# ManuelZ/image-search-engine

Hardware: AMD Instinct MI355X
Metric: queries/sec, exact brute-force L2 kNN (recall@10 vs exact CPU), 1Mx512 fp32 index, k=10 (higher is better)
Workload: dtype f32; 1 GPU; 1000000x512 fp32 uniform[0,1) index (default_rng 1234), L2, k=10, nq=16 queries per step, index resident in HBM, steps issued round-robin on 16 HIP streams; 400 untimed steps ahead of the warm-up bring the GPU out of its idle power state; n=1000000, d=512, k=10, nq=16

## Files before the change

### image-search-engine_amd/csrc/ise_knn.hip

```cpp

#include "ise_common.hpp"
#include "ise_scan_params.hpp"
#include "ise_assign.hpp"
#include "ise_exact.hpp"
#include "ise_merge.hpp"
#include "ise_exact_scan.hpp"
#include "ise_gemm_scan.hpp"
#include "ise_gemm_bf16.hpp"
#include "ise_rows.hpp"
#include "ise_short_scan.hpp"
#include "ise_range.hpp"
#include "ise_sel_scan.hpp"
#include "ise_stage.hpp"
#include "ise_remove.hpp"

static thread_local std::string g_err;
static int fail(int code, const std::string& msg) {
    g_err = msg;
    return code;
}
int ise_fail_(int code, const std::string& msg) { return fail(code, msg); }
#define HIP_TRY(expr)                                                                      \
    do {                                                                                   \
        hipError_t e_ = (expr);                                                            \
        if (e_ != hipSuccess)                                                              \
            return fail(e_ == hipErrorOutOfMemory ? ISE_E_NOMEM : ISE_E_HIP,               \
                        std::string(#expr) + ": " + hipGetErrorString(e_));                \
    } while (0)

struct ise_index {
    int d = 0, dp = 0, metric = ISE_METRIC_L2, device = 0;
    int storage = ISE_STORE_F32;
    long long n = 0, cap = 0;
    void* xb = nullptr;
    float* norms = nullptr;
    float* mu = nullptr;
    bool shift_pinned = false;
    long long mu_rows = 0;
    long long norms_rows = 0;
    void* xh = nullptr;
    float* hmeta = nullptr;
    int dph = 0;
    bool shadow_off = false;
    void* xq8 = nullptr;
    uint32_t* bmeta = nullptr;
    int dpb = 0;
    bool byte_off = false;
    double byte_rel = 0.0;
    double byte_rho = 1.0;
    unsigned long long half_batches = 0;
    unsigned long long byte_batches = 0;
    unsigned long long* stats_dev = nullptr;
    unsigned long long mu_updates = 0;
    unsigned long long gemm_chunks = 0;
    struct WorkSlot {
        u64* part = nullptr;
        size_t part_elems = 0;
        u64* keys_tmp = nullptr;
        size_t keys_tmp_elems = 0;
        u64* xchg = nullptr;
        size_t xchg_elems = 0;
        uint32_t xchg_seq = 0;
        char* gemm = nullptr;
        size_t gemm_bytes = 0;
        u64* fl_state = nullptr;
        int* fl_list = nullptr;
        size_t fl_elems = 0;
        uint32_t fl_seq = 0;
        hipEvent_t done = nullptr;
        bool used = false;
        hipStream_t last_stream = nullptr;
    };
    static constexpr int NWS = 6;
    WorkSlot ws[NWS];
    unsigned ws_next = 0;
    hipStream_t stream = nullptr;
    struct HostCtx {
        hipStream_t stream = nullptr;
        float* q_dev = nullptr;  size_t q_elems = 0;
        float* D_dev = nullptr;  long long* I_dev = nullptr;  size_t out_elems = 0;
        float* q_pin = nullptr;  size_t q_pin_elems = 0;
        float* D_pin = nullptr;  long long* I_pin = nullptr;  size_t out_pin_elems = 0;
        float* D_pin_dev = nullptr;  long long* I_pin_dev = nullptr;
        bool busy = false;
    };
    static constexpr int NHC = 4;
    HostCtx hc[NHC];
    std::mutex hc_mu;
    std::condition_variable hc_cv;
    struct HostReq {
        const float* q; long long nq; int k; float* D; long long* I;
        int rc = 0; std::string err; bool done = false;
        std::condition_variable cv;
    };
    static constexpr int CQ_LEADERS = 2;
    std::mutex cq_mu;
    std::deque<HostReq*> cq;
    int cq_leaders = 0;
    unsigned long long cq_batches = 0, cq_requests = 0;
    unsigned long long direct_queries = 0;
    unsigned long long short_batches = 0;
    int num_cu = 256;
    std::mutex mu_;
    template <class T>
    struct Buf {
        T* p = nullptr;
        size_t n = 0;
    };
    struct RangeWs {
        Buf<float> q;
        Buf<unsigned> cnt;
        Buf<long long> segoff;
        Buf<float> sD;
        Buf<uint32_t> sI;
        Buf<long long> tot, lims;
        Buf<unsigned> flag;
        Buf<float> D;
        Buf<long long> I;
        Buf<float> q_pin;
        Buf<long long> lims_pin;
        Buf<float> D_pin;
        Buf<long long> I_pin;
    };
    RangeWs rg;
    std::mutex rg_mu;
    unsigned long long range_batches = 0, range_overflows = 0;
    unsigned long long remove_calls = 0, remove_rows = 0, remove_moved = 0;
    float remove_last_ms = 0.f;
    unsigned long long remove_last_bytes = 0;
    unsigned long long row_epoch = 0;
    struct SelSlot {
        Buf<float> q;
        Buf<u64> part;
        Buf<u64> keys;
        hipEvent_t done = nullptr;
        bool used = false;
        hipStream_t last_stream = nullptr;
    };
    static constexpr int NSS = 4;
    SelSlot ss[NSS];
    unsigned ss_next = 0;
    unsigned long long sel_batches = 0, sel_passes = 0;
    unsigned long long sel_range_batches = 0;
};

static int elem_size(int storage) { return storage == ISE_STORE_BF16 ? 2 : 4; }
static int pad_dim(int d, int storage) {
    const int per_step = 64 / elem_size(storage);
    const int steps = (d + per_step - 1) / per_step;
    return (steps > 4 ? (steps + 3) / 4 * 4 : steps) * per_step;
}
static int pad_bytes(int d) {
    const int steps = (d + 63) / 64;
    return (steps > 4 ? (steps + 3) / 4 * 4 : steps) * 64;
}
static size_t row_bytes(const ise_index* h) { return (size_t)h->dp * elem_size(h->storage); }
static size_t shadow_row_bytes(const ise_index* h) { return (size_t)h->dph * 2; }
static size_t byte_row_bytes(const ise_index* h) { return (size_t)h->dpb; }
static int chunk_steps_rb(size_t rb) {
    const int steps = (int)(rb / 64);
    for (int ch = 8; ch > 1; ch >>= 1)
        if (steps % ch == 0) return ch;
    return 1;
}
static int chunk_steps(const ise_index* h) { return chunk_steps_rb(row_bytes(h)); }
static int qs_stride_units(int units) {
    const int pad = ((2 - (units / 4)) % 16 + 16) % 16 * 4;
    return units + pad;
}
static int qs_stride_for(const ise_index* h) { return qs_stride_units((int)(row_bytes(h) / 4)); }
static int qs_stride_half(const ise_index* h) { return qs_stride_units(h->dph); }
static int qs_stride_byte(const ise_index* h) { return qs_stride_units(h->dpb / 2); }
#define KPASS_MAX 36
#define XPASS_MAX 32
static size_t scan_lds_bytes(const ise_index* h, int waves, int T, int kb) {
    return scan_lds_layout(qs_stride_for(h), waves, T, kb);
}

extern "C" int ise_version(void) { return 100; }
extern "C" const char* ise_last_error(void) { return g_err.c_str(); }

extern "C" int ise_device_count(int* count) {
    if (!count) return fail(ISE_E_INVALID, "count is NULL");
    int n = 0;
    hipError_t e = hipGetDeviceCount(&n);
    if (e != hipSuccess) {
        *count = 0;
        return fail(ISE_E_NODEVICE, std::string("hipGetDeviceCount: ") + hipGetErrorString(e));
    }
    *count = n;
    return ISE_OK;
}

extern "C" int ise_device_arch(int device, char* buf, int buflen) {
    if (!buf || buflen <= 0) return fail(ISE_E_INVALID, "buf is NULL");
    hipDeviceProp_t prop;
    HIP_TRY(hipGetDeviceProperties(&prop, device));
    snprintf(buf, (size_t)buflen, "%s", prop.gcnArchName);
    return ISE_OK;
}

extern "C" int ise_index_create(ise_index_t** out, int d, int metric, int device) {
    return ise_index_create_ex(out, d, metric, device, ISE_STORE_F32);
}

extern "C" int ise_index_create_ex(ise_index_t** out, int d, int metric, int device, int storage) {
    if (!out) return fail(ISE_E_INVALID, "out is NULL");
    *out = nullptr;
    if (d <= 0) return fail(ISE_E_INVALID, "d must be positive");
    if (storage != ISE_STORE_F32 && storage != ISE_STORE_BF16)
        return fail(ISE_E_INVALID, "storage must be ISE_STORE_F32 or ISE_STORE_BF16");
    if (metric != ISE_METRIC_L2 && metric != ISE_METRIC_INNER_PRODUCT)
        return fail(ISE_E_INVALID, "metric must be ISE_METRIC_L2 or ISE_METRIC_INNER_PRODUCT");
    int ndev = 0;
    if (hipGetDeviceCount(&ndev) != hipSuccess || ndev <= 0)
        return fail(ISE_E_NODEVICE, "no HIP device visible: the kNN path needs an MI355X (gfx950) GPU");
    if (device < 0 || device >= ndev) return fail(ISE_E_INVALID, "device out of range");
    hipDeviceProp_t prop;
    HIP_TRY(hipGetDeviceProperties(&prop, device));
    if (strncmp(prop.gcnArchName, "gfx950", 6) != 0)
        return fail(ISE_E_NODEVICE, std::string("device is ") + prop.gcnArchName +
                                        ", this library is built for gfx950 only");
    ise_index* h = new (std::nothrow) ise_index();
    if (!h) return fail(ISE_E_NOMEM, "host allocation failed");
    h->d = d;
    h->storage = storage;
    h->dp = pad_dim(d, storage);
    h->dph = pad_dim(d, ISE_STORE_BF16);
    h->dpb = pad_bytes(d);
    h->metric = metric;
    h->device = device;
    h->num_cu = prop.multiProcessorCount > 0 ? prop.multiProcessorCount : 256;
    DeviceGuard gd(device);
    hipError_t e = hipStreamCreateWithFlags(&h->stream, hipStreamNonBlocking);
    if (e == hipSuccess) e = hipMalloc(&h->mu, (size_t)h->dp * sizeof(float));
    if (e == hipSuccess) e = hipMemset(h->mu, 0, (size_t)h->dp * sizeof(float));
    if (e == hipSuccess) e = hipMalloc(&h->stats_dev, 32 * sizeof(unsigned long long));
    if (e == hipSuccess) e = hipMemset(h->stats_dev, 0, 32 * sizeof(unsigned long long));
    if (e != hipSuccess) {
        if (h->stream) (void)hipStreamDestroy(h->stream);
        if (h->mu) (void)hipFree(h->mu);
        if (h->stats_dev) (void)hipFree(h->stats_dev);
        delete h;
        return fail(ISE_E_HIP, std::string("index setup: ") + hipGetErrorString(e));
    }
    *out = h;
    return ISE_OK;
}

static void free_byte_shadow(ise_index* h) {
    if (h->xq8) (void)hipFree(h->xq8);
    if (h->bmeta) (void)hipFree(h->bmeta);
    h->xq8 = nullptr;
    h->bmeta = nullptr;
}
static void free_shadow(ise_index* h) {
    if (h->xh) (void)hipFree(h->xh);
    if (h->hmeta) (void)hipFree(h->hmeta);
    h->xh = nullptr;
    h->hmeta = nullptr;
    free_byte_shadow(h);
}

static void free_all(ise_index* h) {
    if (h->xb) (void)hipFree(h->xb);
    if (h->norms) (void)hipFree(h->norms);
    free_shadow(h);
    for (auto& w : h->ws) {
        if (w.part) (void)hipFree(w.part);
        if (w.keys_tmp) (void)hipFree(w.keys_tmp);
        if (w.xchg) (void)hipFree(w.xchg);
        if (w.gemm) (void)hipFree(w.gemm);
        if (w.fl_state) (void)hipFree(w.fl_state);
        if (w.fl_list) (void)hipFree(w.fl_list);
        if (w.done) (void)hipEventDestroy(w.done);
        w = ise_index::WorkSlot();
    }
    for (auto& c : h->hc) {
        if (c.q_dev) (void)hipFree(c.q_dev);
        if (c.D_dev) (void)hipFree(c.D_dev);
        if (c.I_dev) (void)hipFree(c.I_dev);
        if (c.q_pin) (void)hipHostFree(c.q_pin);
        if (c.D_pin) (void)hipHostFree(c.D_pin);
        if (c.I_pin) (void)hipHostFree(c.I_pin);
        if (c.stream) (void)hipStreamDestroy(c.stream);
        c = ise_index::HostCtx();
    }
    {
        auto& r = h->rg;
        for (void* p : {(void*)r.q.p, (void*)r.cnt.p, (void*)r.segoff.p, (void*)r.sD.p, (void*)r.sI.p, (void*)r.tot.p,
                        (void*)r.lims.p, (void*)r.flag.p, (void*)r.D.p, (void*)r.I.p})
            if (p) (void)hipFree(p);
        for (void* p : {(void*)r.q_pin.p, (void*)r.lims_pin.p, (void*)r.D_pin.p, (void*)r.I_pin.p})
            if (p) (void)hipHostFree(p);
        r = ise_index::RangeWs();
    }
    for (auto& sl : h->ss) {
        for (void* p : {(void*)sl.q.p, (void*)sl.part.p, (void*)sl.keys.p})
            if (p) (void)hipFree(p);
        if (sl.done) (void)hipEventDestroy(sl.done);
        sl = ise_index::SelSlot();
    }
    h->xb = h->norms = nullptr;
    h->n = h->cap = 0;
}

extern "C" int ise_index_destroy(ise_index_t* h) {
    if (!h) return ISE_OK;
    {
        DeviceGuard gd(h->device);
        (void)hipDeviceSynchronize();
        free_all(h);
        if (h->mu) (void)hipFree(h->mu);
        if (h->stats_dev) (void)hipFree(h->stats_dev);
        if (h->stream) (void)hipStreamDestroy(h->stream);
    }
    delete h;
    return ISE_OK;
}

extern "C" int ise_index_reset(ise_index_t* h) {
    if (!h) return fail(ISE_E_INVALID, "handle is NULL");
    std::lock_guard<std::mutex> lk(h->mu_);
    DeviceGuard gd(h->device);
    HIP_TRY(hipDeviceSynchronize());
    if (h->xb) (void)hipFree(h->xb);
    if (h->norms) (void)hipFree(h->norms);
    free_shadow(h);
    h->shadow_off = false;
    h->byte_off = false;
    if (h->n > 0) h->row_epoch++;
    h->xb = h->norms = nullptr;
    h->n = h->cap = 0;
    h->shift_pinned = false;
    h->mu_rows = h->norms_rows = 0;
    HIP_TRY(hipMemset(h->mu, 0, (size_t)h->dp * sizeof(float)));
    return ISE_OK;
}

extern "C" int ise_index_info(const ise_index_t* h, int* d, int* metric, int64_t* ntotal, int* device) {
    if (!h) return fail(ISE_E_INVALID, "handle is NULL");
    if (d) *d = h->d;
    if (metric) *metric = h->metric;
    if (ntotal) *ntotal = h->n;
    if (device) *device = h->device;
    return ISE_OK;
}

static int reserve_rows(ise_index* h, long long need, hipStream_t st) {
    if (need <= h->cap) return ISE_OK;
    long long cap = h->cap ? h->cap : 0;
    long long want = need;
    if (cap > 0 && want < cap + cap / 2) want = cap + cap / 2;
    want = (want + 15) / 16 * 16;
    const size_t rb = row_bytes(h);
    char* nx = nullptr;
    float* nn = nullptr;
    HIP_TRY(hipMalloc(&nx, (size_t)want * rb));
    hipError_t e = hipMalloc(&nn, (size_t)want * sizeof(float));
    if (e != hipSuccess) {
        (void)hipFree(nx);
        return fail(ISE_E_NOMEM, std::string("hipMalloc(norms): ") + hipGetErrorString(e));
    }
    if (h->n > 0) {
        HIP_TRY(hipMemcpyAsync(nx, h->xb, (size_t)h->n * rb, hipMemcpyDeviceToDevice, st));
        HIP_TRY(hipMemcpyAsync(nn, h->norms, (size_t)h->n * sizeof(float), hipMemcpyDeviceToDevice, st));
    }
    HIP_TRY(hipMemsetAsync(nx + (size_t)h->n * rb, 0, (size_t)(want - h->n) * rb, st));
    HIP_TRY(hipMemsetAsync(nn + h->n, 0, (size_t)(want - h->n) * sizeof(float), st));
    char* nxh = nullptr;
    float* nmeta = nullptr;
    if (h->xh) {
        const size_t hb = shadow_row_bytes(h);
        if (hipMalloc(&nxh, (size_t)want * hb) != hipSuccess || hipMalloc(&nmeta, (size_t)want * 3 * sizeof(float)) != hipSuccess) {
            (void)hipGetLastError();
            if (nxh) (void)hipFree(nxh);
            nxh = nullptr;
        } else {
            HIP_TRY(hipMemcpyAsync(nxh, h->xh, (size_t)h->n * hb, hipMemcpyDeviceToDevice, st));
            HIP_TRY(hipMemsetAsync(nxh + (size_t)h->n * hb, 0, (size_t)(want - h->n) * hb, st));
            HIP_TRY(hipMemsetAsync(nmeta, 0, (size_t)want * 3 * sizeof(float), st));
            for (int i = 0; i < 3; i++)
                HIP_TRY(hipMemcpyAsync(nmeta + (size_t)i * want, h->hmeta + (size_t)i * h->cap, (size_t)h->n * sizeof(float),
                                       hipMemcpyDeviceToDevice, st));
        }
    }
    char* nxq = nullptr;
    uint32_t* nbm = nullptr;
    if (h->xq8 && nxh) {
        const size_t qb = byte_row_bytes(h);
        if (hipMalloc(&nxq, (size_t)want * qb) != hipSuccess || hipMalloc(&nbm, (size_t)want * sizeof(uint32_t)) != hipSuccess) {
            (void)hipGetLastError();
            if (nxq) (void)hipFree(nxq);
            nxq = nullptr;
        } else {
            HIP_TRY(hipMemcpyAsync(nxq, h->xq8, (size_t)h->n * qb, hipMemcpyDeviceToDevice, st));
            HIP_TRY(hipMemsetAsync(nxq + (size_t)h->n * qb, 0, (size_t)(want - h->n) * qb, st));
            HIP_TRY(hipMemsetAsync(nbm, 0, (size_t)want * sizeof(uint32_t), st));
            HIP_TRY(hipMemcpyAsync(nbm, h->bmeta, (size_t)h->n * sizeof(uint32_t), hipMemcpyDeviceToDevice, st));
        }
    }
    HIP_TRY(hipStreamSynchronize(st));
    if (h->xb) HIP_TRY(hipDeviceSynchronize());
    if (h->xb) (void)hipFree(h->xb);
    if (h->norms) (void)hipFree(h->norms);
    if (h->xh) {
        const bool had_byte = h->xq8 != nullptr;
        free_shadow(h);
        h->shadow_off = nxh == nullptr;
        h->byte_off = h->byte_off || (had_byte && nxh && !nxq);
        h->xh = nxh;
        h->hmeta = nmeta;
        h->xq8 = nxq;
        h->bmeta = nbm;
    }
    h->xb = nx;
    h->norms = nn;
    h->cap = want;
    return ISE_OK;
}

static bool rows_copy_verbatim(const ise_index* h) { return h->storage == ISE_STORE_F32 && h->dp == h->d; }

static bool uses_shift(const ise_index* h) { return h->storage == ISE_STORE_F32 && h->metric == ISE_METRIC_L2; }

static int prepare_shift_locked(ise_index* h, hipStream_t st);

static void launch_shadow(ise_index* h, long long row0, long long n, hipStream_t st) {
    const long long nblk = (n + 3) / 4;
    if (nblk > 0)
        hipLaunchKernelGGL(shadow_rows_kernel, dim3((unsigned)nblk), dim3(256), 0, st, (const float*)h->xb, row0, n, h->d,
                           h->dp, (const float*)h->mu, (_Float16*)h->xh, h->dph, h->hmeta, h->hmeta + h->cap,
                           h->hmeta + 2 * h->cap);
    if (nblk > 0 && h->xq8)
        hipLaunchKernelGGL(byte_rows_kernel, dim3((unsigned)nblk), dim3(256), 0, st, (const float*)h->xb, row0, n, h->d,
                           h->dp, (const float*)h->mu, (int8_t*)h->xq8, h->dpb, h->bmeta);
}

static void launch_norms(ise_index* h, long long row0, long long n, hipStream_t st) {
    const long long nblk = (n + 3) / 4;
    if (h->storage == ISE_STORE_BF16)
        hipLaunchKernelGGL(norms_bf16_kernel, dim3((unsigned)nblk), dim3(256), 0, st, (const __bf16*)h->xb, row0, n,
                           h->dp, h->norms);
    else
        hipLaunchKernelGGL(norms_kernel, dim3((unsigned)nblk), dim3(256), 0, st, (const float*)h->xb, row0, n, h->dp,
                           uses_shift(h) ? h->mu : (const float*)nullptr, h->norms);
    if (h->xh) launch_shadow(h, row0, n, st);
}

#define SHADOW_MIN_ROWS 262144
#define SHADOW_MAX_ROW_BYTES 2048
#define SHADOW_MAX_KC 16
#define BYTE_MAX_K 10
#define BYTE_MAX_NQ 16
#define BYTE_KC 32
#define BYTE_MAX_REL_ERR 0.005
#define BYTE_MIN_RHO 0.5
#define BYTE_SAMPLE 512
static bool byte_rel_ok(const ise_index* h) { return h->byte_rel <= BYTE_MAX_REL_ERR && h->byte_rho >= BYTE_MIN_RHO; }
static int measure_byte_rel(ise_index* h, hipStream_t st) {
    const int m = (int)std::min<long long>(BYTE_SAMPLE, h->n);
    double* dv = nullptr;
    float* dist = nullptr;
    HIP_TRY(hipMalloc(&dv, 2 * sizeof(double)));
    hipError_t e = hipMalloc(&dist, (size_t)m * m * sizeof(float));
    if (e == hipSuccess) {
        hipLaunchKernelGGL(byte_rel_kernel, dim3(1), dim3(1024), 0, st, (const float*)h->norms, (const uint32_t*)h->bmeta,
                           h->n, dv);
        hipLaunchKernelGGL(sample_dist_kernel, dim3((unsigned)(((long long)m * m + 255) / 256)), dim3(256), 0, st,
                           (const float*)h->xb, h->dp, h->d, h->n / m, m, dist);
        hipLaunchKernelGGL(rho_kernel, dim3(1), dim3(1024), 0, st, (const float*)dist, m, dv + 1);
        e = hipGetLastError();
    }
    double v[2] = {INFINITY, 0.0};
    if (e == hipSuccess) e = hipMemcpyAsync(v, dv, 2 * sizeof(double), hipMemcpyDeviceToHost, st);
    if (e == hipSuccess) e = hipStreamSynchronize(st);
    (void)hipFree(dv);
    if (dist) (void)hipFree(dist);
    if (e != hipSuccess) return fail(ISE_E_HIP, std::string("byte shadow statistics: ") + hipGetErrorString(e));
    h->byte_rel = v[0];
    h->byte_rho = v[1];
    return ISE_OK;
}
static bool shadow_wanted(const ise_index* h) {
    return uses_shift(h) && !h->xh && !h->shadow_off && h->n > SHADOW_MIN_ROWS &&
           shadow_row_bytes(h) <= SHADOW_MAX_ROW_BYTES;
}
static bool byte_alloc_refused();
static int alloc_shadow(ise_index* h) {
    hipError_t e = hipMalloc(&h->xh, (size_t)h->cap * shadow_row_bytes(h));
    if (e == hipSuccess) e = hipMalloc(&h->hmeta, (size_t)h->cap * 3 * sizeof(float));
    if (e == hipSuccess) e = hipMemset(h->xh, 0, (size_t)h->cap * shadow_row_bytes(h));
    if (e == hipSuccess) e = hipMemset(h->hmeta, 0, (size_t)h->cap * 3 * sizeof(float));
    if (e != hipSuccess) {
        (void)hipGetLastError();
        free_shadow(h);
        if (e != hipErrorOutOfMemory) return fail(ISE_E_HIP, std::string("shadow rows: ") + hipGetErrorString(e));
        h->shadow_off = true;
        return ISE_OK;
    }
    if (h->byte_off) return ISE_OK;
    e = byte_alloc_refused() ? hipErrorOutOfMemory : hipMalloc(&h->xq8, (size_t)h->cap * byte_row_bytes(h));
    if (e == hipSuccess) e = hipMalloc(&h->bmeta, (size_t)h->cap * sizeof(uint32_t));
    if (e == hipSuccess) e = hipMemset(h->xq8, 0, (size_t)h->cap * byte_row_bytes(h));
    if (e == hipSuccess) e = hipMemset(h->bmeta, 0, (size_t)h->cap * sizeof(uint32_t));
    if (e == hipSuccess) return ISE_OK;
    (void)hipGetLastError();
    if (e != hipErrorOutOfMemory) {
        free_shadow(h);
        return fail(ISE_E_HIP, std::string("byte shadow rows: ") + hipGetErrorString(e));
    }
    free_byte_shadow(h);
    h->byte_off = true;
    return ISE_OK;
}

static int prepare_shift_locked(ise_index* h, hipStream_t st) {
    if (!uses_shift(h) || h->n == 0) return ISE_OK;
    const bool need_mu = !h->shift_pinned && (h->mu_rows == 0 || h->n >= h->mu_rows + h->mu_rows / 4 + 1);
    const bool need_shadow = shadow_wanted(h);
    if (!need_mu && h->norms_rows == h->n && !need_shadow) return ISE_OK;
    HIP_TRY(hipDeviceSynchronize());
    if (need_mu) {
        const int groups = (int)std::max<long long>(1, std::min<long long>(COLMEAN_GROUPS_MAX, h->n / 64));
        float* partial = nullptr;
        HIP_TRY(hipMalloc(&partial, (size_t)groups * h->dp * sizeof(float)));
        hipLaunchKernelGGL(col_sum_kernel, dim3((h->dp + 255) / 256, groups), dim3(256), 0, st, (const float*)h->xb,
                           h->n, h->d, h->dp, groups, partial);
        hipLaunchKernelGGL(col_mean_kernel, dim3((h->dp + 255) / 256), dim3(256), 0, st, partial, h->n, h->d, h->dp,
                           groups, h->mu);
        hipError_t e = hipGetLastError();
        if (e == hipSuccess) e = hipStreamSynchronize(st);
        (void)hipFree(partial);
        if (e != hipSuccess) return fail(ISE_E_HIP, std::string("shift vector: ") + hipGetErrorString(e));
        h->mu_rows = h->n;
        h->norms_rows = 0;
        h->mu_updates++;
    }
    if (need_shadow) {
        int rc = alloc_shadow(h);
        if (rc) return rc;
        if (h->xh) launch_shadow(h, 0, h->norms_rows, st);
    }
    const bool full = h->norms_rows == 0 || need_shadow;
    if (h->n > h->norms_rows) launch_norms(h, h->norms_rows, h->n - h->norms_rows, st);
    HIP_TRY(hipGetLastError());
    HIP_TRY(hipStreamSynchronize(st));
    h->norms_rows = h->n;
    if (full && h->xq8) return measure_byte_rel(h, st);
    return ISE_OK;
}

static void norms_after_add(ise_index* h, long long n, hipStream_t st) {
    if (uses_shift(h) && !h->shift_pinned && h->mu_rows == 0) return;
    if (h->norms_rows != h->n) return;
    launch_norms(h, h->n, n, st);
    h->norms_rows = h->n + n;
}

static int add_device_locked(ise_index* h, const float* x_dev, long long n, hipStream_t st) {
    if (n == 0) return ISE_OK;
    if (h->n + n >= (1ll << 32)) return fail(ISE_E_INVALID, "index would exceed 2^32 - 1 rows");
    int rc = reserve_rows(h, h->n + n, st);
    if (rc) return rc;
    char* dst = static_cast<char*>(h->xb) + (size_t)h->n * row_bytes(h);
    if (rows_copy_verbatim(h)) {
        HIP_TRY(hipMemcpyAsync(dst, x_dev, (size_t)n * h->d * sizeof(float), hipMemcpyDeviceToDevice, st));
    } else {
        const long long total = n * h->dp;
        const int blocks = (int)std::min<long long>((total + 255) / 256, 8192);
        if (h->storage == ISE_STORE_BF16)
            hipLaunchKernelGGL(pad_rows_bf16_kernel, dim3(blocks), dim3(256), 0, st, x_dev, n, h->d, (__bf16*)dst, h->dp);
        else
            hipLaunchKernelGGL(pad_rows_kernel, dim3(blocks), dim3(256), 0, st, x_dev, n, h->d, (float*)dst, h->dp);
        HIP_TRY(hipGetLastError());
    }
    norms_after_add(h, n, st);
    HIP_TRY(hipGetLastError());
    h->n += n;
    return ISE_OK;
}

extern "C" int ise_index_set_shift(ise_index_t* h, const float* mu_host) {
    if (!h || !mu_host) return fail(ISE_E_INVALID, "NULL argument");
    std::lock_guard<std::mutex> lk(h->mu_);
    if (!uses_shift(h)) return ISE_OK;
    DeviceGuard gd(h->device);
    HIP_TRY(hipDeviceSynchronize());
    HIP_TRY(hipMemset(h->mu, 0, (size_t)h->dp * sizeof(float)));
    HIP_TRY(hipMemcpy(h->mu, mu_host, (size_t)h->d * sizeof(float), hipMemcpyHostToDevice));
    h->shift_pinned = true;
    h->norms_rows = 0;
    return ISE_OK;
}

extern "C" int ise_index_get_shift(ise_index_t* h, float* mu_host) {
    if (!h || !mu_host) return fail(ISE_E_INVALID, "NULL argument");
    std::lock_guard<std::mutex> lk(h->mu_);
    DeviceGuard gd(h->device);
    int rc = prepare_shift_locked(h, h->stream);
    if (rc) return rc;
    HIP_TRY(hipDeviceSynchronize());
    HIP_TRY(hipMemcpy(mu_host, h->mu, (size_t)h->d * sizeof(float), hipMemcpyDeviceToHost));
    return ISE_OK;
}

extern "C" int ise_index_add_device(ise_index_t* h, const float* x_dev, int64_t n, void* stream) {
    if (!h) return fail(ISE_E_INVALID, "handle is NULL");
    if (n < 0 || (n > 0 && !x_dev)) return fail(ISE_E_INVALID, "bad rows argument");
    std::lock_guard<std::mutex> lk(h->mu_);
    DeviceGuard gd(h->device);
    return add_device_locked(h, x_dev, n, (hipStream_t)stream);
}

extern "C" int ise_index_add_host(ise_index_t* h, const float* x, int64_t n) {
    if (!h) return fail(ISE_E_INVALID, "handle is NULL");
    if (n < 0 || (n > 0 && !x)) return fail(ISE_E_INVALID, "bad rows argument");
    if (n == 0) return ISE_OK;
    std::lock_guard<std::mutex> lk(h->mu_);
    DeviceGuard gd(h->device);
    if (h->n + n >= (1ll << 32)) return fail(ISE_E_INVALID, "index would exceed 2^32 - 1 rows");
    int rc = reserve_rows(h, h->n + n, h->stream);
    if (rc) return rc;
    const long long slab = std::max<long long>(1, (256ll << 20) / ((long long)h->d * 4));
    float* tmp = nullptr;
    if (!rows_copy_verbatim(h)) HIP_TRY(hipMalloc(&tmp, (size_t)std::min<long long>(slab, n) * h->d * sizeof(float)));
    for (long long i0 = 0; i0 < n; i0 += slab) {
        const long long m = std::min<long long>(slab, n - i0);
        if (rows_copy_verbatim(h)) {
            char* dst = static_cast<char*>(h->xb) + (size_t)h->n * row_bytes(h);
            hipError_t e = hipMemcpyAsync(dst, x + (size_t)i0 * h->d, (size_t)m * h->d * sizeof(float),
                                          hipMemcpyHostToDevice, h->stream);
            if (e != hipSuccess) return fail(ISE_E_HIP, std::string("H2D: ") + hipGetErrorString(e));
            norms_after_add(h, m, h->stream);
            h->n += m;
        } else {
            hipError_t e = hipMemcpyAsync(tmp, x + (size_t)i0 * h->d, (size_t)m * h->d * sizeof(float),
                                          hipMemcpyHostToDevice, h->stream);
            if (e != hipSuccess) {
                (void)hipFree(tmp);
                return fail(ISE_E_HIP, std::string("H2D: ") + hipGetErrorString(e));
            }
            rc = add_device_locked(h, tmp, m, h->stream);
            if (rc) {
                (void)hipFree(tmp);
                return rc;
            }
        }
        hipError_t e = hipStreamSynchronize(h->stream);
        if (e != hipSuccess) {
            if (tmp) (void)hipFree(tmp);
            return fail(ISE_E_HIP, std::string("add sync: ") + hipGetErrorString(e));
        }
    }
    if (tmp) (void)hipFree(tmp);
    return ISE_OK;
}

extern "C" int ise_index_reconstruct_host(ise_index_t* h, int64_t i0, int64_t n, float* out) {
    if (!h) return fail(ISE_E_INVALID, "handle is NULL");
    std::lock_guard<std::mutex> lk(h->mu_);
    if (i0 < 0 || n < 0 || i0 + n > h->n || (n > 0 && !out)) return fail(ISE_E_INVALID, "row range out of bounds");
    if (n == 0) return ISE_OK;
    DeviceGuard gd(h->device);
    const char* src = static_cast<const char*>(h->xb) + (size_t)i0 * row_bytes(h);
    if (h->storage == ISE_STORE_F32) {
        HIP_TRY(hipMemcpy2DAsync(out, (size_t)h->d * 4, src, row_bytes(h), (size_t)h->d * 4, (size_t)n,
                                 hipMemcpyDeviceToHost, h->stream));
        HIP_TRY(hipStreamSynchronize(h->stream));
        return ISE_OK;
    }
    const long long slab = std::max<long long>(1, (64ll << 20) / ((long long)h->d * 4));
    float* tmp = nullptr;
    HIP_TRY(hipMalloc(&tmp, (size_t)std::min<long long>(slab, n) * h->d * sizeof(float)));
    int rc = ISE_OK;
    for (long long r0 = 0; r0 < n && rc == ISE_OK; r0 += slab) {
        const long long m = std::min<long long>(slab, n - r0);
        const long long total = m * h->d;
        hipLaunchKernelGGL(unpack_rows_bf16_kernel, dim3((unsigned)std::min<long long>((total + 255) / 256, 8192)),
                           dim3(256), 0, h->stream, (const __bf16*)(src + (size_t)r0 * row_bytes(h)), m, h->d, h->dp, tmp);
        hipError_t e = hipMemcpyAsync(out + (size_t)r0 * h->d, tmp, (size_t)total * sizeof(float), hipMemcpyDeviceToHost,
                                      h->stream);
        if (e == hipSuccess) e = hipStreamSynchronize(h->stream);
        if (e != hipSuccess) rc = fail(ISE_E_HIP, std::string("reconstruct: ") + hipGetErrorString(e));
    }
    (void)hipFree(tmp);
    return rc;
}


static void launch_short(const ise_index* h, int ch, int waves, int bpc, int grid, size_t lds, hipStream_t st,
                         const ScanParams& sp, const ShortParams& tp) {
    if (h->storage == ISE_STORE_BF16) ise_launch_short_bf16(ch, waves, bpc, grid, lds, st, sp, tp);
    else if (uses_shift(h)) ise_launch_short_f32_shift(ch, waves, bpc, grid, lds, st, sp, tp);
    else ise_launch_short_f32_plain(ch, waves, bpc, grid, lds, st, sp, tp);
}

struct ScanPlan {
    int nblocks, tiles_total, tiles_per_block, nqt, ch, kpass, kb, waves, T;
    size_t lds;
    bool exact;
    int kc;
    bool gemm;
    size_t gemm_bytes;
    bool half;
    bool byte;
    bool short_;
    int short_bpc;
};

static void launch_scan(const ise_index* h, const ScanPlan& pl, dim3 grid, hipStream_t st, const ScanParams& sp) {
    const int ch = pl.ch, waves = pl.waves, T = pl.T;
    const size_t lds = pl.lds;
    if (pl.byte) ise_launch_scan_i8_shadow(ch, waves, T, grid, lds, st, sp);
    else if (pl.half) ise_launch_scan_f16_shadow(ch, waves, T, grid, lds, st, sp);
    else if (h->storage == ISE_STORE_BF16) ise_launch_scan_bf16(ch, waves, T, grid, lds, st, sp);
    else if (uses_shift(h)) ise_launch_scan_f32_shift(ch, waves, T, grid, lds, st, sp);
    else ise_launch_scan_f32_plain(ch, waves, T, grid, lds, st, sp);
}

static int exact_extra(int k) {
    static const int forced = [] { const char* e = getenv("ISE_EXACT_EXTRA"); return e ? atoi(e) : 0; }();
    (void)k;
    return forced > 0 && forced <= 16 ? forced : 4;
}
static float exact_beta(const ise_index* h) { return (0.5625f * h->dp + 256.f) * 5.9604645e-8f * 1.02f; }
static float half_beta(const ise_index* h) { return (5.f * h->dph + 128.f) * 5.9604645e-8f * 1.02f; }
static float half_lo_shrink(const ise_index* h) { return 1.f - ((float)h->dp / 16.f + 96.f) * 5.9604645e-8f; }
static float byte_beta(const ise_index* h) { return ((float)h->dp / 8.f + 64.f) * 5.9604645e-8f * 1.02f; }
struct EnvKnobs {
    std::atomic<int> force_exact{0};
    std::atomic<int> no_direct{0};
    std::atomic<int> no_short{0};
    std::atomic<int> short_tpb_max{0};
    std::atomic<int> direct_short_max_tiles{0};
    std::atomic<int> range_stage_cap{0};
    std::atomic<int> no_half{0};
    std::atomic<int> no_byte{0};
    std::atomic<int> fail_byte_alloc{0};
    std::atomic<int> remove_slab_rows{0};
    void refresh() {
        auto flag = [](const char* name) { const char* e = getenv(name); return (e && e[0] == '1') ? 1 : 0; };
        auto num = [](const char* name) { const char* e = getenv(name); return e ? atoi(e) : 0; };
        force_exact.store(flag("ISE_FORCE_EXACT"));
        no_direct.store(flag("ISE_NO_DIRECT"));
        no_short.store(flag("ISE_NO_SHORT"));
        short_tpb_max.store(num("ISE_SHORT_TPB_MAX"));
        direct_short_max_tiles.store(num("ISE_DIRECT_SHORT_MAX_TILES"));
        range_stage_cap.store(num("ISE_RANGE_STAGE_CAP"));
        no_half.store(flag("ISE_NO_HALF_FILTER"));
        no_byte.store(flag("ISE_NO_BYTE_FILTER"));
        fail_byte_alloc.store(flag("ISE_FAIL_BYTE_ALLOC"));
        remove_slab_rows.store(num("ISE_REMOVE_SLAB_ROWS"));
    }
};
static EnvKnobs& knobs() {
    static EnvKnobs k;
    static std::once_flag once;
    std::call_once(once, [] { k.refresh(); });
    return k;
}
extern "C" int ise_refresh_env_knobs(void) {
    knobs().refresh();
    return ISE_OK;
}
static bool force_exact() { return knobs().force_exact.load(std::memory_order_relaxed) != 0; }
static bool byte_alloc_refused() { return knobs().fail_byte_alloc.load(std::memory_order_relaxed) != 0; }

static bool xchg_enabled() {
    static const bool on = [] { const char* e = getenv("ISE_NO_XCHG"); return !(e && e[0] == '1'); }();
    return on;
}

static int make_plan(const ise_index* h, long long nq, int k, ScanPlan* pl, bool allow_short = true,
                     bool allow_half = true) {
    pl->exact = uses_shift(h);
    const bool shadow_ok = allow_half && pl->exact && h->xh != nullptr && !knobs().no_half.load(std::memory_order_relaxed);
    pl->byte = shadow_ok && h->xq8 != nullptr && byte_rel_ok(h) && !knobs().no_byte.load(std::memory_order_relaxed) &&
               k <= BYTE_MAX_K && nq <= BYTE_MAX_NQ;
    pl->kc = pl->exact ? (pl->byte ? BYTE_KC : k + exact_extra(k)) : k;
    pl->kpass = pl->kc < KPASS_MAX ? pl->kc : KPASS_MAX;
    pl->kb = pl->kpass <= 16 ? 16 : (pl->kpass <= 32 ? 32 : KB_MAX);
    pl->half = shadow_ok && (pl->byte || pl->kc <= SHADOW_MAX_KC);
    const size_t rb = pl->byte ? byte_row_bytes(h) : (pl->half ? shadow_row_bytes(h) : row_bytes(h));
    auto lds_bytes = [&](int waves, int T) {
        if (pl->byte) return scan_lds_layout(qs_stride_byte(h), waves, T, pl->kb, true);
        return pl->half ? scan_lds_layout(qs_stride_half(h), waves, T, pl->kb, true) : scan_lds_bytes(h, waves, T, pl->kb);
    };
    pl->ch = chunk_steps_rb(rb);
#ifdef ISE_ABLATE
    if (const char* e = getenv("ISE_CH")) {
        const int ch = atoi(e);
        if ((ch == 1 || ch == 2 || ch == 4 || ch == 8) && (int)(rb / 64) % ch == 0) pl->ch = ch;
    }
#endif
    static const double pass_cost_f32[5] = {0.0, 1.0, 1.11, 1.45, 0.0};
    static const double pass_cost_bf16[5] = {0.0, 1.0, 1.07, 1.16, 1.25};
    const bool bf16 = h->storage == ISE_STORE_BF16;
    const double* pass_cost = (bf16 || pl->half) ? pass_cost_bf16 : pass_cost_f32;
    int tmax = bf16 ? 4 : 3;
#ifdef ISE_ABLATE
    if (const char* e = getenv("ISE_TMAX")) tmax = std::min(tmax, std::max(1, atoi(e)));
#endif
    pl->T = 0;
    double best = 0;
    for (int t = 1; t <= tmax; t++) {
        int wv = 0;
        size_t lds = 0;
        const bool xchg_pays = !bf16 && xchg_enabled() && (h->n + 15) / 16 >= 6ll * 8 * h->num_cu;
        if (t == 2 && !xchg_pays && lds_bytes(16, 2) <= LDS_LIMIT) {
            wv = 16;
            lds = lds_bytes(16, 2);
        }
        for (int cand_w = 8; cand_w >= (t == 1 ? 4 : 8) && !wv; cand_w -= 4) {
            lds = lds_bytes(cand_w, t);
            if (lds <= LDS_LIMIT) wv = cand_w;
        }
        if (!wv) break;
        const double cost = (double)((nq + 16 * t - 1) / (16 * t)) * pass_cost[t];
        if (!pl->T || cost < best - 1e-9) {
            pl->T = t;
            pl->waves = wv;
            pl->lds = lds;
            best = cost;
        }
    }
    if (!pl->T) return fail(ISE_E_INVALID, "d too large: a 16-query tile must fit the 160 KiB LDS "
                                              "(float32 rows: d <= 2240, bf16 rows: d <= 4480)");
    if ((pl->T == 1 || pl->waves == 16) && pl->ch > 4) pl->ch = 4;
    pl->tiles_total = (int)((h->n + 15) / 16);
    int blocks_per_cu = (pl->T == 1 && pl->waves <= 8 && pl->lds <= LDS_LIMIT / 2) ? 2 : 1;
#ifdef ISE_ABLATE
    if (const char* e = getenv("ISE_PLAN")) {
        int wv = 8, bpc = 2;
        if (pl->T == 1 && sscanf(e, "%d,%d", &wv, &bpc) == 2 && (wv == 4 || wv == 8) && bpc >= 1) {
            pl->waves = wv;
            pl->lds = lds_bytes(wv, 1);
            blocks_per_cu = bpc;
        }
    }
#endif
    const bool long_rows = rb > 2048;
    const int nqt_plan = (int)((nq + 16 * pl->T - 1) / (16 * pl->T));
    const int min_tiles = (int)std::max<size_t>(1, 65536 / (16 * rb));
    const int slots = h->num_cu * blocks_per_cu;
    const int nb_packed = std::min(slots, (pl->tiles_total + pl->waves - 1) / pl->waves);
    const int nb_spread = std::min(std::max(1, slots / nqt_plan), (pl->tiles_total + min_tiles - 1) / min_tiles);
    int nb = std::max(nb_packed, nb_spread);
    if (nb < 1) nb = 1;
    if (nb > MERGE_LISTS_MAX) nb = MERGE_LISTS_MAX;
    pl->tiles_per_block = (pl->tiles_total + nb - 1) / nb;
    if (pl->tiles_per_block < 1) pl->tiles_per_block = 1;
    pl->nblocks = (pl->tiles_total + pl->tiles_per_block - 1) / pl->tiles_per_block;
    if (pl->nblocks < 1) pl->nblocks = 1;
    if (long_rows && pl->T == 1 && pl->waves <= 8 && pl->tiles_per_block <= pl->waves && chunk_steps_rb(rb) == 8) pl->ch = 8;
    pl->nqt = (int)((nq + 16 * pl->T - 1) / (16 * pl->T));
    pl->gemm = false;
    pl->gemm_bytes = 0;
    pl->short_ = false;
    pl->short_bpc = 0;
    static const bool short_t2 = [] { const char* e = getenv("ISE_SHORT_T2"); return !(e && e[0] == '0'); }();
    const int short_T = nq <= 16 ? 1 : 2;
    if (allow_short && !pl->byte && (nq <= 16 || (short_t2 && nq <= 64)) && pl->kc <= pl->kpass && h->n > 0 &&
        !knobs().no_short.load(std::memory_order_relaxed)) {
        int tpb_max = knobs().short_tpb_max.load(std::memory_order_relaxed);
        if (tpb_max <= 0 || tpb_max > SHORT_TPB_MAX) tpb_max = SHORT_TPB_MAX;
        const int S = qs_stride_for(h);
        static const int shapes[2][3] = {{16, 1, 1}, {8, 2, 1}};
        int first = row_bytes(h) <= 2048 ? 0 : 2;
#ifdef ISE_ABLATE
        if (const char* e = getenv("ISE_SHORT_SHAPE")) first = std::max(first, std::min(1, atoi(e)));
#endif
        for (int si = first; si < 2 && !pl->short_; si++) {
            const int wv = shapes[si][0], bpc = shapes[si][1];
            const int short_nqt = (int)((nq + 16 * short_T - 1) / (16 * short_T));
            const int packed = (pl->tiles_total + wv - 1) / wv;
            const int spread = std::min(std::max(1, h->num_cu * bpc / short_nqt), (pl->tiles_total + min_tiles - 1) / min_tiles);
            int nbs = std::max(1, std::min(h->num_cu * bpc * shapes[si][2], std::max(packed, spread)));
            nbs = std::min(nbs, MERGE_LISTS_MAX);
            const int tpb = (pl->tiles_total + nbs - 1) / nbs;
            const size_t lds = short_lds_layout(S, tpb, wv, short_T);
            if (tpb <= tpb_max && lds <= (size_t)LDS_LIMIT / bpc) {
                pl->short_ = true;
                pl->nblocks = nbs;
                pl->tiles_per_block = tpb;
                pl->lds = lds;
                pl->waves = wv;
                pl->short_bpc = bpc;
                pl->T = short_T;
                pl->nqt = short_nqt;
                pl->ch = std::min(chunk_steps(h), 4);
                pl->half = false;
                pl->byte = false;
            }
        }
    }
    return ISE_OK;
}

static int ensure_workspace(ise_index::WorkSlot* w, const ScanPlan& pl, long long nq, bool* changed) {
    if (!w->done) HIP_TRY(hipEventCreateWithFlags(&w->done, hipEventDisableTiming));
    const size_t need = std::max<size_t>((size_t)pl.nqt * pl.nblocks * (16 * pl.T) * pl.kpass, (size_t)MERGE_LISTS_MAX * XPASS_MAX);
    if (need > w->part_elems) {
        if (w->part) (void)hipFree(w->part);
        w->part = nullptr;
        w->part_elems = 0;
        HIP_TRY(hipMalloc(&w->part, need * sizeof(u64)));
        w->part_elems = need;
        *changed = true;
    }
    const size_t needx = (size_t)pl.nqt * (16 * pl.T) * pl.nblocks;
    if (needx > w->xchg_elems) {
        if (w->xchg) (void)hipFree(w->xchg);
        w->xchg = nullptr;
        w->xchg_elems = 0;
        HIP_TRY(hipMalloc(&w->xchg, needx * sizeof(u64)));
        HIP_TRY(hipMemset(w->xchg, 0xFF, needx * sizeof(u64)));
        w->xchg_elems = needx;
        w->xchg_seq = 0;
        if (const char* e = getenv("ISE_XCHG_SEQ_START"))
            w->xchg_seq = (uint32_t)strtoul(e, nullptr, 0);
        *changed = true;
    }
    if (pl.kc > pl.kpass) {
        const size_t need2 = (size_t)nq * ((size_t)pl.kc + 2 + pl.kpass + XPASS_MAX);
        if (need2 > w->keys_tmp_elems) {
            if (w->keys_tmp) (void)hipFree(w->keys_tmp);
            w->keys_tmp = nullptr;
            w->keys_tmp_elems = 0;
            HIP_TRY(hipMalloc(&w->keys_tmp, need2 * sizeof(u64)));
            w->keys_tmp_elems = need2;
            *changed = true;
        }
    }
    if (pl.gemm) {
        const size_t needg = pl.gemm_bytes;
        if (needg > w->gemm_bytes) {
            if (w->gemm) (void)hipFree(w->gemm);
            w->gemm = nullptr;
            w->gemm_bytes = 0;
            HIP_TRY(hipMalloc(&w->gemm, needg));
            w->gemm_bytes = needg;
            *changed = true;
        }
    }
    if (pl.exact) {
        if (!w->fl_state) {
            HIP_TRY(hipMalloc(&w->fl_state, 2 * sizeof(u64)));
            HIP_TRY(hipMemset(w->fl_state, 0, 2 * sizeof(u64)));
            w->fl_seq = 0;
            if (const char* e = getenv("ISE_XCHG_SEQ_START")) w->fl_seq = (uint32_t)strtoul(e, nullptr, 0);
            *changed = true;
        }
        if ((size_t)nq > w->fl_elems) {
            if (w->fl_list) (void)hipFree(w->fl_list);
            w->fl_list = nullptr;
            w->fl_elems = 0;
            HIP_TRY(hipMalloc(&w->fl_list, (size_t)nq * sizeof(int)));
            w->fl_elems = (size_t)nq;
            *changed = true;
        }
    }
    return ISE_OK;
}

static int ensure_workspaces(ise_index* h, const ScanPlan& pl, long long nq) {
    bool changed = false;
    for (auto& w : h->ws) {
        int rc = ensure_workspace(&w, pl, nq, &changed);
        if (rc) return rc;
    }
    if (changed) HIP_TRY(hipDeviceSynchronize());
    return ISE_OK;
}

__global__ void floor_from_keys_kernel(const u64* pass_keys, int nq, int kp, u64* floor_out) {
    const int q = blockIdx.x * blockDim.x + threadIdx.x;
    if (q < nq) floor_out[q] = pass_keys[(size_t)q * kp + kp - 1];
}
__global__ void scatter_pass_kernel(const u64* pass_keys, int nq, int kp, u64* keys_all, int k, int off) {
    const int i = blockIdx.x * blockDim.x + threadIdx.x;
    if (i < nq * kp) {
        const int q = i / kp, r = i - q * kp;
        if (off + r < k) keys_all[(size_t)q * k + off + r] = pass_keys[i];
    }
}
__global__ void decode_keys_kernel(const u64* keys, long long total, int metric, float* D, long long* I) {
    const long long i = (long long)blockIdx.x * blockDim.x + threadIdx.x;
    if (i < total) {
        const u64 key = keys[i];
        const bool pad = key == KEY_PAD;
        const float sc = unord_f32((uint32_t)(key >> 32));
        D[i] = pad ? (metric == ISE_METRIC_L2 ? FLT_MAX : -FLT_MAX) : (metric == ISE_METRIC_L2 ? sc : -sc);
        I[i] = pad ? -1ll : (long long)(uint32_t)key;
    }
}

struct TimedOut {
    hipEvent_t e0, e1, e2;
    bool on = false;
};

static int next_xchg_seq(ise_index::WorkSlot* w, hipStream_t st, uint32_t* seq) {
    if (w->xchg_seq >= 0xFFFFFFF0u) {
        HIP_TRY(hipMemsetAsync(w->xchg, 0xFF, w->xchg_elems * sizeof(u64), st));
        w->xchg_seq = 0;
    }
    *seq = ++w->xchg_seq;
    return ISE_OK;
}
static int next_fl_seq(ise_index::WorkSlot* w, hipStream_t st, uint32_t* seq) {
    if (w->fl_seq >= 0xFFFFFFF0u) {
        HIP_TRY(hipMemsetAsync(w->fl_state, 0, sizeof(u64), st));
        w->fl_seq = 0;
    }
    *seq = ++w->fl_seq;
    return ISE_OK;
}

template <bool RERANK>
static void launch_merge(unsigned grid, size_t lds, hipStream_t st, const MergeParams& mp, const ExactParams& xp) {
    hipLaunchKernelGGL((merge_kernel<RERANK>), dim3(grid), dim3(MERGE_THREADS), lds, st, mp, xp);
}

static int enqueue_exact_fallback(ise_index* h, ise_index::WorkSlot* w, const ScanPlan& pl, const ExactParams& xp,
                                  long long nq, hipStream_t st) {
    ExactScanParams xs;
    xs.xb = (const float*)h->xb; xs.q = xp.q; xs.n = h->n; xs.d = h->d; xs.dp = h->dp;
    xs.id_base = xp.id_base; xs.fl_state = w->fl_state; xs.fl_list = w->fl_list; xs.seq = xp.seq;
    xs.part = w->part;
    xs.rows_per_block = (long long)pl.tiles_per_block * 16;
    xs.arrive = reinterpret_cast<unsigned int*>(w->fl_state + 1);
    xs.direct_n = 0;
    const size_t lds = (size_t)XQ * h->dp * 4 + (size_t)XQ * 4 * 32 * 8;
    MergeParams mp;
    mp.lists = w->part; mp.qt = 1; mp.n_lists = pl.nblocks; mp.nq = (int)nq; mp.metric = h->metric;
    mp.fl_state = w->fl_state; mp.fl_list = w->fl_list; mp.seq = xp.seq; mp.dbg = nullptr; mp.gate = nullptr;
    const int k = xp.k;
    if (k <= XPASS_MAX) {
        xs.kpass = k; xs.floor_keys = nullptr;
        mp.k = k; mp.stride_list = k; mp.stride_qtile = (long long)pl.nblocks * k;
        mp.D = xp.D; mp.I = xp.I; mp.keys_out = xp.keys_out; mp.out_by_pos = 0;
        hipLaunchKernelGGL(exact_scan_kernel<XQ>, dim3((unsigned)pl.nblocks), dim3(256), lds, st, xs, mp);
        HIP_TRY(hipGetLastError());
        return ISE_OK;
    }
    u64* fb_floor = w->keys_tmp + (size_t)nq * ((size_t)pl.kc + 1 + pl.kpass);
    u64* fb_pass = fb_floor + nq;
    const int kp = XPASS_MAX;
    for (int off = 0; off < k; off += kp) {
        xs.kpass = kp; xs.floor_keys = off ? fb_floor : nullptr;
        mp.k = kp; mp.stride_list = kp; mp.stride_qtile = (long long)pl.nblocks * kp;
        mp.D = nullptr; mp.I = nullptr; mp.keys_out = fb_pass; mp.out_by_pos = 1;
        hipLaunchKernelGGL(exact_scan_kernel<XQ>, dim3((unsigned)pl.nblocks), dim3(256), lds, st, xs, mp);
        const long long tot = nq * kp;
        hipLaunchKernelGGL(exact_scatter_kernel, dim3((unsigned)((tot + 255) / 256)), dim3(256), 0, st, xp,
                           (const u64*)fb_pass, kp, off, fb_floor);
        HIP_TRY(hipGetLastError());
    }
    return ISE_OK;
}

static bool no_direct() { return knobs().no_direct.load(std::memory_order_relaxed) != 0; }
static bool direct_applies(const ise_index* h, const ise_index::WorkSlot* w, const ScanPlan& pl, long long nq, int k,
                           int* blocks_out) {
    if (!pl.exact || nq != 1 || k > XPASS_MAX || h->n <= 0 || !w->fl_state || no_direct() || force_exact()) return false;
    int max_tiles = knobs().direct_short_max_tiles.load(std::memory_order_relaxed);
    if (max_tiles <= 0) max_tiles = 128;
    if (pl.short_ && pl.tiles_total > max_tiles) return false;
    long long min_rows = std::max<long long>(16, std::min<long long>(64, (32 * 1024) / ((long long)h->dp * 4)));
    if (h->n < min_rows * 64) min_rows = std::max<long long>(16, h->n / 64);
    long long blocks = std::min<long long>(MERGE_LISTS_MAX, (h->n + min_rows - 1) / min_rows);
    static const long long per_cu = [] { const char* e = getenv("ISE_DIRECT_BLOCKS_PER_CU"); const int v = e ? atoi(e) : 0; return (long long)(v > 0 ? v : 2); }();
    blocks = std::min<long long>(blocks, (long long)h->num_cu * per_cu);
    if ((size_t)nq * blocks * k > w->part_elems) return false;
    *blocks_out = (int)blocks;
    return true;
}
static int direct_small_enqueue(ise_index* h, ise_index::WorkSlot* w, int blocks, const float* q_dev, long long nq, int k,
                                uint32_t id_base, float* D_dev, long long* I_dev, u64* keys_out, hipStream_t st,
                                TimedOut* tm) {
    ExactScanParams xs;
    xs.xb = (const float*)h->xb; xs.q = q_dev; xs.n = h->n; xs.d = h->d; xs.dp = h->dp;
    xs.kpass = k; xs.id_base = id_base; xs.fl_state = w->fl_state; xs.fl_list = w->fl_list; xs.seq = 0;
    xs.floor_keys = nullptr; xs.part = w->part;
    xs.rows_per_block = (h->n + blocks - 1) / blocks;
    xs.arrive = reinterpret_cast<unsigned int*>(w->fl_state + 1);
    xs.direct_n = (int)nq;
    MergeParams mp;
    mp.lists = w->part; mp.qt = 1; mp.n_lists = blocks; mp.nq = (int)nq; mp.metric = h->metric;
    mp.fl_state = w->fl_state; mp.fl_list = w->fl_list; mp.seq = 0; mp.dbg = nullptr; mp.gate = nullptr;
    mp.k = k; mp.stride_list = k; mp.stride_qtile = (long long)blocks * k;
    mp.D = D_dev; mp.I = I_dev; mp.keys_out = keys_out; mp.out_by_pos = 0;
    if (tm && tm->on) HIP_TRY(hipEventRecord(tm->e0, st));
    const int qn = 1;
    const size_t lds = (size_t)qn * h->dp * 4 + (size_t)qn * 4 * 32 * 8;
    hipLaunchKernelGGL((exact_scan_kernel<1, true>), dim3((unsigned)blocks), dim3(256), lds, st, xs, mp);
    HIP_TRY(hipGetLastError());
    if (tm && tm->on) {
        HIP_TRY(hipEventRecord(tm->e1, st));
        HIP_TRY(hipEventRecord(tm->e2, st));
    }
    h->direct_queries += (unsigned long long)nq;
    return ISE_OK;
}

#define GEMM_MIN_NQ 256
#define GEMM_CAPQ 4096
#define GEMM_SAMPLE_SLABS 128
static bool gemm_applies(const ise_index* h, long long nq, int k) {
    static const bool off = [] { const char* e = getenv("ISE_NO_GEMM"); return e && e[0] == '1'; }();
    static const long long min_nq = [] { const char* e = getenv("ISE_GEMM_MIN_NQ"); const int v = e ? atoi(e) : 0; return (long long)(v >= 17 ? v : GEMM_MIN_NQ); }();
    const long long need = h->storage == ISE_STORE_BF16 ? std::min<long long>(min_nq, 128) : min_nq;
    if (off || nq < need || h->n < 128ll * 1024) return false;
    if (h->dp > 512 || h->dp % 128 != 0) return false;
    if (h->storage == ISE_STORE_BF16) return k <= XPASS_MAX;
    if (!uses_shift(h)) return k <= XPASS_MAX;
    return k + exact_extra(k) <= XPASS_MAX;
}
#define GEMM_CAPW 2048
struct GemmLayout {
    size_t qprep, xn, tau, ccnt, dump, cand, wbuf, wcnt, total;
};
static GemmLayout gemm_layout(const ise_index* h) {
    GemmLayout g;
    size_t o = 0;
    auto take = [&](size_t bytes) { const size_t at = o; o += (bytes + 255) / 256 * 256; return at; };
    g.qprep = take((size_t)GEMM_NQ_MAX * qs_stride_for(h) * 4);
    g.xn = take((size_t)GEMM_NQ_MAX * 4);
    g.tau = take((size_t)GEMM_NQ_MAX * 4);
    g.ccnt = take((size_t)(GEMM_NQ_MAX * GEMM_SUBS + 64) * 4);
    g.dump = take((size_t)GEMM_NQ_MAX * GEMM_SAMPLE_SLABS * 128 * 4);
    g.cand = take((size_t)GEMM_NQ_MAX * GEMM_CAPQ * 8);
    g.wbuf = take((size_t)h->num_cu * 8 * GEMM_CAPW * 16);
    g.wcnt = take((size_t)h->num_cu * 8 * 4);
    g.total = o;
    return g;
}

static int plan_for_batch(const ise_index* h, long long nq, int k, ScanPlan* pl) {
    const bool big = gemm_applies(h, nq, k);
    int rc = make_plan(h, big ? std::min<long long>(nq, GEMM_NQ_MAX) : nq, k, pl);
    if (rc) return rc;
    pl->gemm = big;
    pl->gemm_bytes = big ? gemm_layout(h).total : 0;
    return ISE_OK;
}

template <int NS, bool DUMP, bool IPM>
static void launch_gemm_metric(int grid, size_t lds, hipStream_t st, const GemmScanParams& gp) {
    static LdsAttrOnce attr;
    attr.ensure(reinterpret_cast<const void*>(&gemm_scan_kernel<NS, DUMP, IPM>), LDS_LIMIT);
    hipLaunchKernelGGL((gemm_scan_kernel<NS, DUMP, IPM>), dim3(grid), dim3(512), lds, st, gp);
}
template <int NS, bool DUMP>
static void launch_gemm_one(int grid, size_t lds, hipStream_t st, const GemmScanParams& gp) {
    if (gp.metric == ISE_METRIC_INNER_PRODUCT) launch_gemm_metric<NS, DUMP, true>(grid, lds, st, gp);
    else launch_gemm_metric<NS, DUMP, false>(grid, lds, st, gp);
}
template <bool DUMP>
static int launch_gemm(int ns, int grid, size_t lds, hipStream_t st, const GemmScanParams& gp) {
    switch (ns) {
        case 8: launch_gemm_one<8, DUMP>(grid, lds, st, gp); break;
        case 16: launch_gemm_one<16, DUMP>(grid, lds, st, gp); break;
        case 24: launch_gemm_one<24, DUMP>(grid, lds, st, gp); break;
        case 32: launch_gemm_one<32, DUMP>(grid, lds, st, gp); break;
        default: return fail(ISE_E_INVALID, "large-batch path: unsupported padded dimension");
    }
    return ISE_OK;
}

static int search_large_chunk(ise_index* h, ise_index::WorkSlot* w, const float* q_dev, long long nq, int k,
                              uint32_t id_base, float* D_dev, long long* I_dev, u64* keys_out, hipStream_t st,
                              TimedOut* tm) {
    const int kc = k + exact_extra(k);
    const int S = qs_stride_for(h);
    const GemmLayout gl = gemm_layout(h);
    h->gemm_chunks++;
    float* qprep = reinterpret_cast<float*>(w->gemm + gl.qprep);
    float* xn = reinterpret_cast<float*>(w->gemm + gl.xn);
    float* tau = reinterpret_cast<float*>(w->gemm + gl.tau);
    unsigned int* ccnt = reinterpret_cast<unsigned int*>(w->gemm + gl.ccnt);
    float* dump = reinterpret_cast<float*>(w->gemm + gl.dump);
    u64* cand = reinterpret_cast<u64*>(w->gemm + gl.cand);
    const int nq_pad = (int)((nq + GQ - 1) / GQ * GQ);
    int rc;

    if (tm && tm->on) HIP_TRY(hipEventRecord(tm->e0, st));
    hipLaunchKernelGGL(qprep_kernel, dim3((unsigned)((nq_pad + 3) / 4)), dim3(256), 0, st, q_dev, (int)nq, nq_pad, h->d, S,
                       (const float*)h->mu, qprep, xn);
    HIP_TRY(hipGetLastError());

    GemmScanParams gp;
    gp.xb = (const float*)h->xb; gp.norms = h->norms; gp.mu = h->mu; gp.n = h->n; gp.rows16 = (h->n + 15) / 16 * 16;
    gp.dp = h->dp; gp.S = S; gp.qprep = qprep; gp.xn = xn; gp.tau = tau; gp.nq = (int)nq; gp.nq_pad = nq_pad;
    gp.beta = exact_beta(h); gp.id_base = id_base; gp.metric = ISE_METRIC_L2;
    gp.wbuf = reinterpret_cast<u32x4*>(w->gemm + gl.wbuf); gp.wcnt = reinterpret_cast<unsigned int*>(w->gemm + gl.wcnt);
    gp.capw = GEMM_CAPW;
    gp.ablate = 0;
    const int slabs_all = (int)((h->n + 127) / 128);
    const size_t lds = gemm_lds_bytes(S);
    const int ns = h->dp / 16;

    gp.slabs = std::min(slabs_all, GEMM_SAMPLE_SLABS);
    gp.slab_stride = slabs_all / gp.slabs;
    const int nstages = nq_pad / GQ;
    gp.qparts = std::max(1, std::min(nstages, (2 * h->num_cu) / gp.slabs));
    gp.dump = dump;
    if ((rc = launch_gemm<true>(ns, gp.slabs * gp.qparts, lds, st, gp))) return rc;
    hipLaunchKernelGGL(kth_select_kernel, dim3((unsigned)nq_pad), dim3(256), 0, st, (const float*)dump, gp.slabs * 128, kc,
                       (int)nq, tau);
    HIP_TRY(hipGetLastError());
    HIP_TRY(hipMemsetAsync(ccnt, 0, (size_t)(GEMM_NQ_MAX * GEMM_SUBS + 64) * 4, st));

    gp.slabs = slabs_all; gp.slab_stride = 1; gp.qparts = 1; gp.dump = nullptr;
    const int grid = std::min(slabs_all, h->num_cu);
    if ((rc = launch_gemm<false>(ns, grid, lds, st, gp))) return rc;
    unsigned int* overflow = ccnt + GEMM_NQ_MAX * GEMM_SUBS;
    hipLaunchKernelGGL(regroup_kernel, dim3((unsigned)grid * 8), dim3(256), 0, st, (const u32x4*)gp.wbuf,
                       (const unsigned int*)gp.wcnt, GEMM_CAPW, cand, ccnt, GEMM_CAPQ, overflow);
    HIP_TRY(hipGetLastError());
    if (tm && tm->on) HIP_TRY(hipEventRecord(tm->e1, st));

    ScanPlan pl;
    rc = make_plan(h, nq, k, &pl);
    if (rc) return rc;
    ExactParams xp;
    xp.xb = (const float*)h->xb; xp.q = q_dev; xp.n = h->n; xp.d = h->d; xp.dp = h->dp; xp.nq = (int)nq;
    xp.k = k; xp.kc = kc; xp.id_base = id_base; xp.D = D_dev; xp.I = I_dev; xp.keys_out = keys_out;
    xp.fl_state = w->fl_state; xp.fl_list = w->fl_list; xp.seq = 0; xp.stats = h->stats_dev;
    xp.force_fail = force_exact() ? 1 : 0;
    xp.tau_bound = tau;
    if ((rc = next_fl_seq(w, st, &xp.seq))) return rc;
    hipLaunchKernelGGL(gemm_select_kernel, dim3((unsigned)nq), dim3(256),
                       rerank_lds_bytes(h->dp, kc) + (size_t)(GEMM_CAPQ + 256) * 8, st, xp, (const u64*)cand,
                       (const unsigned int*)ccnt, GEMM_CAPQ, (const unsigned int*)overflow);
    HIP_TRY(hipGetLastError());
    if ((rc = enqueue_exact_fallback(h, w, pl, xp, nq, st))) return rc;
    if (tm && tm->on) HIP_TRY(hipEventRecord(tm->e2, st));
    return ISE_OK;
}

static int scan_path_enqueue(ise_index* h, ise_index::WorkSlot* w, const ScanPlan& pl, const float* q_dev, long long nq,
                             int k, uint32_t id_base, float* D_dev, long long* I_dev, u64* keys_out, hipStream_t st,
                             TimedOut* tm, const unsigned int* gate) {
    int rc;
    ScanParams sp;
    sp.xb = h->xb; sp.norms = h->norms; sp.q = q_dev; sp.mu = h->mu; sp.floor_keys = nullptr; sp.part = w->part;
    sp.n = h->n; sp.d = h->d; sp.dp = h->dp; sp.qs_stride = qs_stride_for(h);
    sp.row_slots = (int)(row_bytes(h) / 16);
    sp.nq = (int)nq; sp.k = pl.kpass; sp.kb = pl.kb; sp.metric = h->metric; sp.id_base = id_base;
    sp.beta = pl.exact ? exact_beta(h) : 0.f;
    if (pl.byte) {
        sp.xb = h->xq8; sp.bmeta = h->bmeta;
        sp.qs_stride = qs_stride_byte(h); sp.row_slots = (int)(byte_row_bytes(h) / 16);
        sp.beta = byte_beta(h); sp.lo_shrink = half_lo_shrink(h);
        h->half_batches++;
        h->byte_batches++;
    } else if (pl.half) {
        sp.xb = h->xh; sp.norms = h->hmeta; sp.herr = h->hmeta + h->cap; sp.hexp = h->hmeta + 2 * h->cap;
        sp.qs_stride = qs_stride_half(h); sp.row_slots = (int)(shadow_row_bytes(h) / 16);
        sp.beta = half_beta(h); sp.lo_shrink = half_lo_shrink(h);
        h->half_batches++;
    }
    sp.tiles_total = pl.tiles_total; sp.tiles_per_block = pl.tiles_per_block;
    sp.xchg = xchg_enabled() ? w->xchg : nullptr;
    sp.xchg_seq = 0;
    sp.gate = gate;
    sp.ablate = 0;
    sp.stamps = nullptr;
#ifdef ISE_ABLATE
    if (const char* e = getenv("ISE_ABLATE")) sp.ablate = atoi(e);
    if (const char* e = getenv("ISE_STAMPS")) sp.stamps = (unsigned long long*)strtoull(e, nullptr, 0);
#endif

    MergeParams mp;
    const int NQ = 16 * pl.T;
    mp.lists = w->part; mp.stride_list = (long long)NQ * pl.kpass;
    mp.stride_qtile = (long long)pl.nblocks * NQ * pl.kpass; mp.qt = NQ;
    mp.n_lists = pl.nblocks; mp.nq = (int)nq; mp.k = pl.kpass; mp.metric = h->metric;
    mp.fl_state = nullptr; mp.fl_list = nullptr; mp.seq = 0; mp.out_by_pos = 0;
    mp.dbg = h->stats_dev + 8;
    mp.gate = gate;

    ExactParams xp;
    xp.xb = (const float*)h->xb; xp.q = q_dev; xp.n = h->n; xp.d = h->d; xp.dp = h->dp; xp.nq = (int)nq;
    xp.k = k; xp.kc = pl.kc; xp.id_base = id_base; xp.D = D_dev; xp.I = I_dev; xp.keys_out = keys_out;
    xp.fl_state = w->fl_state; xp.fl_list = w->fl_list; xp.seq = 0; xp.stats = h->stats_dev;
    xp.force_fail = force_exact() ? 1 : 0;
    xp.tau_bound = nullptr;

    if (pl.short_) {
        if (gate) return fail(ISE_E_INVALID, "internal: a gated rerun was planned for the short-index kernel");
        ShortParams shp;
        shp.even_split = 1;
        shp.T = pl.T;
        shp.nqt = pl.nqt;
        h->short_batches++;
        if (tm && tm->on) HIP_TRY(hipEventRecord(tm->e0, st));
        launch_short(h, pl.ch, pl.waves, pl.short_bpc, pl.nblocks, pl.lds, st, sp, shp);
        HIP_TRY(hipGetLastError());
        if (tm && tm->on) HIP_TRY(hipEventRecord(tm->e1, st));
        if (pl.exact) {
            if ((rc = next_fl_seq(w, st, &xp.seq))) return rc;
            mp.D = nullptr; mp.I = nullptr; mp.keys_out = nullptr;
            launch_merge<true>((unsigned)nq, rerank_lds_bytes(h->dp, pl.kc), st, mp, xp);
            HIP_TRY(hipGetLastError());
            if ((rc = enqueue_exact_fallback(h, w, pl, xp, nq, st))) return rc;
        } else {
            mp.D = D_dev; mp.I = I_dev; mp.keys_out = keys_out;
            launch_merge<false>((unsigned)nq, 0, st, mp, xp);
            HIP_TRY(hipGetLastError());
        }
        if (tm && tm->on) HIP_TRY(hipEventRecord(tm->e2, st));
        return ISE_OK;
    }
    const dim3 grid((unsigned)pl.nblocks, (unsigned)pl.nqt);
    if (pl.kc <= pl.kpass) {
        if ((rc = next_xchg_seq(w, st, &sp.xchg_seq))) return rc;
        if (tm && tm->on) HIP_TRY(hipEventRecord(tm->e0, st));
        launch_scan(h, pl, grid, st, sp);
        HIP_TRY(hipGetLastError());
        if (tm && tm->on) HIP_TRY(hipEventRecord(tm->e1, st));
        if (pl.exact) {
            if ((rc = next_fl_seq(w, st, &xp.seq))) return rc;
            mp.D = nullptr; mp.I = nullptr; mp.keys_out = nullptr;
            launch_merge<true>((unsigned)nq, rerank_lds_bytes(h->dp, pl.kc), st, mp, xp);
            HIP_TRY(hipGetLastError());
            if ((rc = enqueue_exact_fallback(h, w, pl, xp, nq, st))) return rc;
        } else {
            mp.D = D_dev; mp.I = I_dev; mp.keys_out = keys_out;
            launch_merge<false>((unsigned)nq, 0, st, mp, xp);
            HIP_TRY(hipGetLastError());
        }
        if (tm && tm->on) HIP_TRY(hipEventRecord(tm->e2, st));
        return ISE_OK;
    }
    const int kc = pl.kc;
    u64* keys_all = (!pl.exact && keys_out) ? keys_out : w->keys_tmp;
    u64* floor_dev = w->keys_tmp + (size_t)nq * kc;
    u64* pass_keys = floor_dev + nq;
    if (tm && tm->on) HIP_TRY(hipEventRecord(tm->e0, st));
    for (int off = 0; off < kc; off += pl.kpass) {
        sp.floor_keys = off ? floor_dev : nullptr;
        mp.D = nullptr; mp.I = nullptr; mp.keys_out = pass_keys;
        if ((rc = next_xchg_seq(w, st, &sp.xchg_seq))) return rc;
        launch_scan(h, pl, grid, st, sp);
        HIP_TRY(hipGetLastError());
        launch_merge<false>((unsigned)nq, 0, st, mp, xp);
        HIP_TRY(hipGetLastError());
        const int tot = (int)nq * pl.kpass;
        hipLaunchKernelGGL(scatter_pass_kernel, dim3((tot + 255) / 256), dim3(256), 0, st, pass_keys, (int)nq,
                           pl.kpass, keys_all, kc, off);
        hipLaunchKernelGGL(floor_from_keys_kernel, dim3(((int)nq + 255) / 256), dim3(256), 0, st, pass_keys, (int)nq,
                           pl.kpass, floor_dev);
        HIP_TRY(hipGetLastError());
    }
    if (tm && tm->on) HIP_TRY(hipEventRecord(tm->e1, st));
    if (pl.exact) {
        if ((rc = next_fl_seq(w, st, &xp.seq))) return rc;
        hipLaunchKernelGGL(rerank_kernel, dim3((unsigned)nq), dim3(256), rerank_lds_bytes(h->dp, kc), st, xp,
                           (const u64*)keys_all);
        HIP_TRY(hipGetLastError());
        if ((rc = enqueue_exact_fallback(h, w, pl, xp, nq, st))) return rc;
    } else if (D_dev) {
        const long long total = nq * k;
        hipLaunchKernelGGL(decode_keys_kernel, dim3((unsigned)((total + 255) / 256)), dim3(256), 0, st, keys_all, total,
                           h->metric, D_dev, I_dev);
        HIP_TRY(hipGetLastError());
    }
    if (tm && tm->on) HIP_TRY(hipEventRecord(tm->e2, st));
    return ISE_OK;
}


template <int NS, bool DUMP, bool L2>
static void launch_gemm_bf16_metric(int grid, size_t lds, hipStream_t st, const GemmScanParams& gp) {
    static LdsAttrOnce attr;
    attr.ensure(reinterpret_cast<const void*>(&gemm_scan_bf16_kernel<NS, DUMP, L2>), LDS_LIMIT);
    hipLaunchKernelGGL((gemm_scan_bf16_kernel<NS, DUMP, L2>), dim3(grid), dim3(512), lds, st, gp);
}
template <int NS, bool DUMP>
static void launch_gemm_bf16_one(int grid, size_t lds, hipStream_t st, const GemmScanParams& gp) {
    if (gp.metric == ISE_METRIC_L2) launch_gemm_bf16_metric<NS, DUMP, true>(grid, lds, st, gp);
    else launch_gemm_bf16_metric<NS, DUMP, false>(grid, lds, st, gp);
}
template <bool DUMP>
static int launch_gemm_bf16(int ns, int grid, size_t lds, hipStream_t st, const GemmScanParams& gp) {
    switch (ns) {
        case 4: launch_gemm_bf16_one<4, DUMP>(grid, lds, st, gp); break;
        case 8: launch_gemm_bf16_one<8, DUMP>(grid, lds, st, gp); break;
        case 12: launch_gemm_bf16_one<12, DUMP>(grid, lds, st, gp); break;
        case 16: launch_gemm_bf16_one<16, DUMP>(grid, lds, st, gp); break;
        default: return fail(ISE_E_INVALID, "large-batch path: unsupported padded dimension");
    }
    return ISE_OK;
}

static int search_large_chunk_bf16(ise_index* h, ise_index::WorkSlot* w, const float* q_dev, long long nq, int k,
                                   uint32_t id_base, float* D_dev, long long* I_dev, u64* keys_out, hipStream_t st,
                                   TimedOut* tm) {
    const int S = qs_stride_for(h);
    const GemmLayout gl = gemm_layout(h);
    h->gemm_chunks++;
    uint32_t* qprep = reinterpret_cast<uint32_t*>(w->gemm + gl.qprep);
    float* xn = reinterpret_cast<float*>(w->gemm + gl.xn);
    float* tau = reinterpret_cast<float*>(w->gemm + gl.tau);
    unsigned int* ccnt = reinterpret_cast<unsigned int*>(w->gemm + gl.ccnt);
    float* dump = reinterpret_cast<float*>(w->gemm + gl.dump);
    u64* cand = reinterpret_cast<u64*>(w->gemm + gl.cand);
    const int nq_pad = (int)((nq + GB_GQ - 1) / GB_GQ * GB_GQ);
    int rc;

    if (tm && tm->on) HIP_TRY(hipEventRecord(tm->e0, st));
    hipLaunchKernelGGL(qprep_bf16_kernel, dim3((unsigned)((nq_pad + 3) / 4)), dim3(256), 0, st, q_dev, (int)nq, nq_pad, h->d, S,
                       qprep, xn);
    HIP_TRY(hipGetLastError());

    constexpr int ROWS = 8 * GB_XT * 16;
    GemmScanParams gp;
    gp.xb = (const float*)h->xb; gp.norms = h->norms; gp.mu = nullptr; gp.n = h->n; gp.rows16 = (h->n + 15) / 16 * 16;
    gp.dp = h->dp; gp.S = S; gp.qprep = reinterpret_cast<const float*>(qprep); gp.xn = xn; gp.tau = tau; gp.nq = (int)nq;
    gp.nq_pad = nq_pad; gp.beta = 0.f; gp.metric = h->metric; gp.id_base = id_base;
    gp.wbuf = reinterpret_cast<u32x4*>(w->gemm + gl.wbuf); gp.wcnt = reinterpret_cast<unsigned int*>(w->gemm + gl.wcnt);
    gp.capw = GEMM_CAPW;
    gp.ablate = 0;
#ifdef ISE_ABLATE
    if (const char* e = getenv("ISE_GEMM_ABLATE")) gp.ablate = atoi(e);
#endif
    const int slabs_all = (int)((h->n + ROWS - 1) / ROWS);
    const size_t lds = (size_t)2 * GB_GQ * S * 4 + (size_t)2 * GEMM_NQ_MAX * 4;
    const int ns = h->dp / 32;

    gp.slabs = std::min(slabs_all, GEMM_SAMPLE_SLABS * 128 / ROWS);
    gp.slab_stride = slabs_all / gp.slabs;
    const int nstages = nq_pad / GB_GQ;
    gp.qparts = std::max(1, std::min(nstages, (2 * h->num_cu) / gp.slabs));
    gp.dump = dump;
    if ((rc = launch_gemm_bf16<true>(ns, gp.slabs * gp.qparts, lds, st, gp))) return rc;
    hipLaunchKernelGGL(kth_select_kernel, dim3((unsigned)nq_pad), dim3(256), 0, st, (const float*)dump, gp.slabs * ROWS, k,
                       (int)nq, tau);
    HIP_TRY(hipGetLastError());
    HIP_TRY(hipMemsetAsync(ccnt, 0, (size_t)(GEMM_NQ_MAX * GEMM_SUBS + 64) * 4, st));

    gp.slabs = slabs_all; gp.slab_stride = 1; gp.qparts = 1; gp.dump = nullptr;
    const int grid = std::min(slabs_all, h->num_cu);
    if ((rc = launch_gemm_bf16<false>(ns, grid, lds, st, gp))) return rc;
    unsigned int* overflow = ccnt + GEMM_NQ_MAX * GEMM_SUBS;
    unsigned int* rerun = overflow + 1;
    hipLaunchKernelGGL(regroup_kernel, dim3((unsigned)grid * 8), dim3(256), 0, st, (const u32x4*)gp.wbuf,
                       (const unsigned int*)gp.wcnt, GEMM_CAPW, cand, ccnt, GEMM_CAPQ, overflow);
    HIP_TRY(hipGetLastError());
    if (tm && tm->on) HIP_TRY(hipEventRecord(tm->e1, st));
    hipLaunchKernelGGL(gemm_select_plain_kernel, dim3((unsigned)nq), dim3(256), (size_t)(GEMM_CAPQ + 320) * 8, st, (const u64*)cand,
                       (const unsigned int*)ccnt, GEMM_CAPQ, (const unsigned int*)overflow, rerun, k, h->metric, D_dev, I_dev,
                       keys_out);
    HIP_TRY(hipGetLastError());
    ScanPlan pl;
    rc = make_plan(h, nq, k, &pl, false);
    if (rc) return rc;
    rc = scan_path_enqueue(h, w, pl, q_dev, nq, k, id_base, D_dev, I_dev, keys_out, st, nullptr, rerun);
    if (rc) return rc;
    if (tm && tm->on) HIP_TRY(hipEventRecord(tm->e2, st));
    return ISE_OK;
}

static int search_large_chunk_ip(ise_index* h, ise_index::WorkSlot* w, const float* q_dev, long long nq, int k,
                                 uint32_t id_base, float* D_dev, long long* I_dev, u64* keys_out, hipStream_t st,
                                 TimedOut* tm) {
    const int S = qs_stride_for(h);
    const GemmLayout gl = gemm_layout(h);
    h->gemm_chunks++;
    float* qprep = reinterpret_cast<float*>(w->gemm + gl.qprep);
    float* xn = reinterpret_cast<float*>(w->gemm + gl.xn);
    float* tau = reinterpret_cast<float*>(w->gemm + gl.tau);
    unsigned int* ccnt = reinterpret_cast<unsigned int*>(w->gemm + gl.ccnt);
    float* dump = reinterpret_cast<float*>(w->gemm + gl.dump);
    u64* cand = reinterpret_cast<u64*>(w->gemm + gl.cand);
    const int nq_pad = (int)((nq + GQ - 1) / GQ * GQ);
    int rc;

    if (tm && tm->on) HIP_TRY(hipEventRecord(tm->e0, st));
    hipLaunchKernelGGL(qprep_kernel, dim3((unsigned)((nq_pad + 3) / 4)), dim3(256), 0, st, q_dev, (int)nq, nq_pad, h->d, S,
                       (const float*)nullptr, qprep, xn);
    HIP_TRY(hipGetLastError());

    GemmScanParams gp;
    gp.xb = (const float*)h->xb; gp.norms = h->norms; gp.mu = nullptr; gp.n = h->n; gp.rows16 = (h->n + 15) / 16 * 16;
    gp.dp = h->dp; gp.S = S; gp.qprep = qprep; gp.xn = xn; gp.tau = tau; gp.nq = (int)nq; gp.nq_pad = nq_pad;
    gp.beta = 0.f; gp.id_base = id_base; gp.metric = ISE_METRIC_INNER_PRODUCT;
    gp.wbuf = reinterpret_cast<u32x4*>(w->gemm + gl.wbuf); gp.wcnt = reinterpret_cast<unsigned int*>(w->gemm + gl.wcnt);
    gp.capw = GEMM_CAPW;
    gp.ablate = 0;
    const int slabs_all = (int)((h->n + 127) / 128);
    const size_t lds = gemm_lds_bytes(S);
    const int ns = h->dp / 16;

    gp.slabs = std::min(slabs_all, GEMM_SAMPLE_SLABS);
    gp.slab_stride = slabs_all / gp.slabs;
    const int nstages = nq_pad / GQ;
    gp.qparts = std::max(1, std::min(nstages, (2 * h->num_cu) / gp.slabs));
    gp.dump = dump;
    if ((rc = launch_gemm<true>(ns, gp.slabs * gp.qparts, lds, st, gp))) return rc;
    hipLaunchKernelGGL(kth_select_kernel, dim3((unsigned)nq_pad), dim3(256), 0, st, (const float*)dump, gp.slabs * 128, k,
                       (int)nq, tau);
    HIP_TRY(hipGetLastError());
    HIP_TRY(hipMemsetAsync(ccnt, 0, (size_t)(GEMM_NQ_MAX * GEMM_SUBS + 64) * 4, st));

    gp.slabs = slabs_all; gp.slab_stride = 1; gp.qparts = 1; gp.dump = nullptr;
    const int grid = std::min(slabs_all, h->num_cu);
    if ((rc = launch_gemm<false>(ns, grid, lds, st, gp))) return rc;
    unsigned int* overflow = ccnt + GEMM_NQ_MAX * GEMM_SUBS;
    unsigned int* rerun = overflow + 1;
    hipLaunchKernelGGL(regroup_kernel, dim3((unsigned)grid * 8), dim3(256), 0, st, (const u32x4*)gp.wbuf,
                       (const unsigned int*)gp.wcnt, GEMM_CAPW, cand, ccnt, GEMM_CAPQ, overflow);
    HIP_TRY(hipGetLastError());
    if (tm && tm->on) HIP_TRY(hipEventRecord(tm->e1, st));
    hipLaunchKernelGGL(gemm_select_plain_kernel, dim3((unsigned)nq), dim3(256), (size_t)(GEMM_CAPQ + 320) * 8, st, (const u64*)cand,
                       (const unsigned int*)ccnt, GEMM_CAPQ, (const unsigned int*)overflow, rerun, k, h->metric, D_dev, I_dev,
                       keys_out);
    HIP_TRY(hipGetLastError());
    ScanPlan pl;
    rc = make_plan(h, nq, k, &pl, false);
    if (rc) return rc;
    rc = scan_path_enqueue(h, w, pl, q_dev, nq, k, id_base, D_dev, I_dev, keys_out, st, nullptr, rerun);
    if (rc) return rc;
    if (tm && tm->on) HIP_TRY(hipEventRecord(tm->e2, st));
    return ISE_OK;
}

static int search_enqueue(ise_index* h, const float* q_dev, long long nq, int k, uint32_t id_base, float* D_dev,
                          long long* I_dev, u64* keys_out, hipStream_t st, TimedOut* tm) {
    int rc = prepare_shift_locked(h, st);
    if (rc) return rc;
    ScanPlan pl;
    rc = plan_for_batch(h, nq, k, &pl);
    if (rc) return rc;
    rc = ensure_workspaces(h, pl, pl.gemm ? std::min<long long>(nq, GEMM_NQ_MAX) : nq);
    if (rc) return rc;
    ise_index::WorkSlot* w = nullptr;
    bool same_stream = false;
    for (auto& s : h->ws)
        if (s.used && s.last_stream == st) { w = &s; same_stream = true; break; }
    if (!w)
        for (auto& s : h->ws)
            if (!s.used) { w = &s; break; }
    if (!w) w = &h->ws[h->ws_next++ % ise_index::NWS];
    if (w->used && !same_stream) HIP_TRY(hipStreamWaitEvent(st, w->done, 0));
    struct Release {
        ise_index::WorkSlot* w;
        hipStream_t st;
        ~Release() {
            if (hipEventRecord(w->done, st) == hipSuccess) { w->used = true; w->last_stream = st; }
        }
    } release{w, st};

    if (pl.gemm) {
        for (long long q0 = 0; q0 < nq; q0 += GEMM_NQ_MAX) {
            const long long m = std::min<long long>(GEMM_NQ_MAX, nq - q0);
            rc = (h->storage == ISE_STORE_BF16 ? search_large_chunk_bf16
                  : uses_shift(h)               ? search_large_chunk
                                                : search_large_chunk_ip)(
                h, w, q_dev + (size_t)q0 * h->d, m, k, id_base, D_dev ? D_dev + (size_t)q0 * k : nullptr,
                I_dev ? I_dev + (size_t)q0 * k : nullptr, keys_out ? keys_out + (size_t)q0 * k : nullptr, st, tm);
            if (rc) return rc;
        }
        return ISE_OK;
    }

    int dblocks = 0;
    if (direct_applies(h, w, pl, nq, k, &dblocks))
        return direct_small_enqueue(h, w, dblocks, q_dev, nq, k, id_base, D_dev, I_dev, keys_out, st, tm);
    return scan_path_enqueue(h, w, pl, q_dev, nq, k, id_base, D_dev, I_dev, keys_out, st, tm, nullptr);
}

static int check_search_args(const ise_index* h, const void* q, long long nq, int k) {
    if (!h) return fail(ISE_E_INVALID, "handle is NULL");
    if (nq < 0 || (nq > 0 && !q)) return fail(ISE_E_INVALID, "bad query argument");
    if (k <= 0 || k > ISE_MAX_K) return fail(ISE_E_INVALID, "k must be in [1, 2048]");
    if (nq > (1ll << 20)) return fail(ISE_E_INVALID, "at most 2^20 queries per call");
    return ISE_OK;
}

extern "C" int ise_index_search_device(ise_index_t* h, const float* q_dev, int64_t nq, int k, float* D_dev,
                                       int64_t* I_dev, void* stream) {
    int rc = check_search_args(h, q_dev, nq, k);
    if (rc) return rc;
    if (nq == 0) return ISE_OK;
    if (!D_dev || !I_dev) return fail(ISE_E_INVALID, "output pointer is NULL");
    std::lock_guard<std::mutex> lk(h->mu_);
    DeviceGuard gd(h->device);
    return search_enqueue(h, q_dev, nq, k, 0u, D_dev, (long long*)I_dev, nullptr, (hipStream_t)stream, nullptr);
}

extern "C" int ise_index_search_keys_device(ise_index_t* h, const float* q_dev, int64_t nq, int k, uint32_t id_base,
                                            uint64_t* keys_dev, void* stream) {
    int rc = check_search_args(h, q_dev, nq, k);
    if (rc) return rc;
    if (nq == 0) return ISE_OK;
    if (!keys_dev) return fail(ISE_E_INVALID, "output pointer is NULL");
    if ((long long)id_base + h->n > (1ll << 32)) return fail(ISE_E_INVALID, "id_base + ntotal exceeds 2^32");
    std::lock_guard<std::mutex> lk(h->mu_);
    DeviceGuard gd(h->device);
    return search_enqueue(h, q_dev, nq, k, id_base, nullptr, nullptr, (u64*)keys_dev, (hipStream_t)stream, nullptr);
}

extern "C" int ise_index_search_timed_device(ise_index_t* h, const float* q_dev, int64_t nq, int k, float* D_dev,
                                             int64_t* I_dev, void* stream, int iters, float* scan_ms_avg,
                                             float* merge_ms_avg) {
    int rc = check_search_args(h, q_dev, nq, k);
    if (rc) return rc;
    if (nq == 0 || iters <= 0) return fail(ISE_E_INVALID, "timed search needs nq > 0, iters > 0");
    if (!D_dev || !I_dev) return fail(ISE_E_INVALID, "output pointer is NULL");
    std::lock_guard<std::mutex> lk(h->mu_);
    DeviceGuard gd(h->device);
    hipStream_t st = (hipStream_t)stream;
    TimedOut tm;
    tm.on = true;
    HIP_TRY(hipEventCreate(&tm.e0));
    HIP_TRY(hipEventCreate(&tm.e1));
    HIP_TRY(hipEventCreate(&tm.e2));
    double s_scan = 0, s_merge = 0;
    for (int it = 0; it < iters; it++) {
// ... 694 lines not shown
    struct Release {
        ise_index::SelSlot* sl;
        hipStream_t st;
        ~Release() {
            if (hipEventRecord(sl->done, st) == hipSuccess) { sl->used = true; sl->last_stream = st; }
        }
    } release{sl, st};
    for (long long i0 = 0; i0 < nq; i0 += SEL_NQ_CHUNK) {
        const long long m = std::min<long long>(SEL_NQ_CHUNK, nq - i0);
        rc = sel_chunk_enqueue(h, sl, sel, q_dev + (size_t)i0 * h->d, m, k, D_dev + (size_t)i0 * k, I_dev + (size_t)i0 * k, st);
        if (rc) return rc;
    }
    return ISE_OK;
}

extern "C" int ise_index_search_sel_device(ise_index_t* h, const float* q_dev, int64_t nq, int k, const ise_selector_t* sel,
                                           float* D_dev, int64_t* I_dev, void* stream) {
    int rc = check_search_args(h, q_dev, nq, k);
    if (rc) return rc;
    if (!sel) return fail(ISE_E_INVALID, "selector is NULL");
    if (nq > 0 && (!D_dev || !I_dev)) return fail(ISE_E_INVALID, "output pointer is NULL");
    std::lock_guard<std::mutex> lk(h->mu_);
    if (nq == 0) return selector_check_locked(h, sel);
    DeviceGuard gd(h->device);
    return search_sel_enqueue(h, sel, q_dev, nq, k, D_dev, (long long*)I_dev, (hipStream_t)stream);
}

extern "C" int ise_index_search_sel_host(ise_index_t* h, const float* q, int64_t nq, int k, const ise_selector_t* sel,
                                         float* D, int64_t* I) {
    int rc = check_search_args(h, q, nq, k);
    if (rc) return rc;
    if (!sel) return fail(ISE_E_INVALID, "selector is NULL");
    if (nq > 0 && (!D || !I)) return fail(ISE_E_INVALID, "output pointer is NULL");
    if (nq == 0) {
        std::lock_guard<std::mutex> lk(h->mu_);
        return selector_check_locked(h, sel);
    }
    DeviceGuard gd(h->device);
    ise_index::HostCtx* c = acquire_ctx(h);
    struct Rel { ise_index* h; ise_index::HostCtx* c; ~Rel() { release_ctx(h, c); } } rel{h, c};
    if (!c->stream) HIP_TRY(hipStreamCreateWithFlags(&c->stream, hipStreamNonBlocking));
    const long long batch = 1024;
    const size_t qe = (size_t)std::min<long long>(nq, batch) * h->d;
    const size_t oe = (size_t)std::min<long long>(nq, batch) * k;
    if (qe > c->q_elems) {
        if (c->q_dev) (void)hipFree(c->q_dev);
        c->q_dev = nullptr; c->q_elems = 0;
        HIP_TRY(hipMalloc(&c->q_dev, qe * sizeof(float)));
        c->q_elems = qe;
    }
    if (oe > c->out_elems) {
        if (c->D_dev) (void)hipFree(c->D_dev);
        if (c->I_dev) (void)hipFree(c->I_dev);
        c->D_dev = nullptr; c->I_dev = nullptr; c->out_elems = 0;
        HIP_TRY(hipMalloc(&c->D_dev, oe * sizeof(float)));
        HIP_TRY(hipMalloc(&c->I_dev, oe * sizeof(long long)));
        c->out_elems = oe;
    }
    for (long long i0 = 0; i0 < nq; i0 += batch) {
        const long long m = std::min<long long>(batch, nq - i0);
        HIP_TRY(hipMemcpyAsync(c->q_dev, q + (size_t)i0 * h->d, (size_t)m * h->d * sizeof(float), hipMemcpyHostToDevice,
                               c->stream));
        {
            std::lock_guard<std::mutex> lk(h->mu_);
            rc = search_sel_enqueue(h, sel, c->q_dev, m, k, c->D_dev, c->I_dev, c->stream);
        }
        if (rc) return rc;
        HIP_TRY(hipMemcpyAsync(D + (size_t)i0 * k, c->D_dev, (size_t)m * k * sizeof(float), hipMemcpyDeviceToHost, c->stream));
        HIP_TRY(hipMemcpyAsync(I + (size_t)i0 * k, c->I_dev, (size_t)m * k * sizeof(long long), hipMemcpyDeviceToHost,
                               c->stream));
        HIP_TRY(hipStreamSynchronize(c->stream));
    }
    return ISE_OK;
}

extern "C" int ise_index_sel_stats(ise_index_t* h, uint64_t* out3) {
    if (!h || !out3) return fail(ISE_E_INVALID, "NULL argument");
    {
        std::lock_guard<std::mutex> lk(h->mu_);
        out3[0] = h->sel_batches;
        out3[1] = h->sel_passes;
    }
    std::lock_guard<std::mutex> lk(h->rg_mu);
    out3[2] = h->sel_range_batches;
    return ISE_OK;
}

struct RemoveRun {
    long long start, len;
};

struct RemoveScratch {
    uint32_t* g = nullptr;
    uint32_t* cend = nullptr;
    uint32_t* src_idx = nullptr;
    char* bounce = nullptr;
    hipEvent_t ev0 = nullptr, ev1 = nullptr;
    ~RemoveScratch() {
        for (void* p : {(void*)g, (void*)cend, (void*)src_idx, (void*)bounce})
            if (p) (void)hipFree(p);
        if (ev0) (void)hipEventDestroy(ev0);
        if (ev1) (void)hipEventDestroy(ev1);
    }
};

static void remove_move_rows(const ise_index* h, void* base, size_t stride, long long a, long long m, const RemoveScratch& sc,
                             hipStream_t st) {
    const uint32_t upr = (uint32_t)(stride / 16);
    const uint32_t total = (uint32_t)(m * upr);
    const uint32_t pieces = (total + 64 * REMOVE_UNROLL - 1) / (64 * REMOVE_UNROLL);
    const unsigned grid = std::max(1u, std::min((pieces + 3) / 4, (unsigned)h->num_cu * 4u));
    hipLaunchKernelGGL(remove_rows_kernel<true>, dim3(grid), dim3(256), 0, st, (const u32x4*)base,
                       (const uint32_t*)sc.src_idx, (u32x4*)sc.bounce, total, upr);
    hipLaunchKernelGGL(remove_rows_kernel<false>, dim3(grid), dim3(256), 0, st, (const u32x4*)sc.bounce,
                       (const uint32_t*)nullptr, (u32x4*)(static_cast<char*>(base) + (size_t)a * stride), total, upr);
}

static int remove_runs_locked(ise_index* h, const std::vector<RemoveRun>& runs, long long removed) {
    const long long n_old = h->n, n_new = n_old - removed, first = runs[0].start;
    const long long moved = n_new - first;
    hipStream_t st = h->stream;
    HIP_TRY(hipDeviceSynchronize());
    if (n_new <= SHADOW_MIN_ROWS) free_shadow(h);
    const bool meta = h->norms_rows == n_old;
    const size_t rb = row_bytes(h), hb = shadow_row_bytes(h), qb = byte_row_bytes(h);
    const bool mv_h = meta && h->xh, mv_q = meta && h->xq8;
    RemoveScratch sc;
    if (moved > 0) {
        const long long T = (long long)runs.size();
        std::vector<uint32_t> g((size_t)T), cend((size_t)T);
        long long c = 0;
        for (long long t = 0; t < T; t++) {
            g[(size_t)t] = (uint32_t)(runs[(size_t)t].start - c);
            c += runs[(size_t)t].len;
            cend[(size_t)t] = (uint32_t)c;
        }
        long long slab = knobs().remove_slab_rows.load(std::memory_order_relaxed);
        if (slab <= 0) slab = std::max<long long>(1, (256ll << 20) / (long long)rb);
        slab = std::min(slab, std::max<long long>(1, (1ll << 31) / (long long)(rb / 16)));
        slab = std::min(slab, moved);
        HIP_TRY(hipMalloc(&sc.g, (size_t)T * sizeof(uint32_t)));
        HIP_TRY(hipMalloc(&sc.cend, (size_t)T * sizeof(uint32_t)));
        HIP_TRY(hipMalloc(&sc.src_idx, (size_t)slab * sizeof(uint32_t)));
        HIP_TRY(hipMalloc(&sc.bounce, (size_t)slab * rb));
        HIP_TRY(hipEventCreate(&sc.ev0));
        HIP_TRY(hipEventCreate(&sc.ev1));
        HIP_TRY(hipMemcpyAsync(sc.g, g.data(), (size_t)T * sizeof(uint32_t), hipMemcpyHostToDevice, st));
        HIP_TRY(hipMemcpyAsync(sc.cend, cend.data(), (size_t)T * sizeof(uint32_t), hipMemcpyHostToDevice, st));
        HIP_TRY(hipStreamSynchronize(st));
        HIP_TRY(hipEventRecord(sc.ev0, st));
        for (long long a = first; a < n_new; a += slab) {
            const long long m = std::min(slab, n_new - a);
            const unsigned gw = (unsigned)std::min<long long>((m + 255) / 256, (long long)h->num_cu * 8);
            hipLaunchKernelGGL(remove_src_kernel, dim3(gw), dim3(256), 0, st, (const uint32_t*)sc.g,
                               (const uint32_t*)sc.cend, (int)T, (uint32_t)a, (uint32_t)m, sc.src_idx);
            remove_move_rows(h, h->xb, rb, a, m, sc, st);
            if (mv_h) remove_move_rows(h, h->xh, hb, a, m, sc, st);
            if (mv_q) remove_move_rows(h, h->xq8, qb, a, m, sc, st);
            if (meta) {
                RemovePlanes gp{}, cp{};
                int np = 0;
                auto plane = [&](void* arr) {
                    uint32_t* w = static_cast<uint32_t*>(arr);
                    uint32_t* b = reinterpret_cast<uint32_t*>(sc.bounce) + (size_t)np * m;
                    gp.src[np] = w;
                    gp.dst[np] = b;
                    cp.src[np] = b;
                    cp.dst[np] = w + a;
                    np++;
                };
                plane(h->norms);
                if (mv_h)
                    for (int i = 0; i < 3; i++) plane(h->hmeta + (size_t)i * h->cap);
                if (mv_q) plane(h->bmeta);
                hipLaunchKernelGGL(remove_words_kernel<true>, dim3(gw, np), dim3(256), 0, st, gp,
                                   (const uint32_t*)sc.src_idx, (uint32_t)m);
                hipLaunchKernelGGL(remove_words_kernel<false>, dim3(gw, np), dim3(256), 0, st, cp,
                                   (const uint32_t*)nullptr, (uint32_t)m);
            }
            HIP_TRY(hipGetLastError());
        }
        HIP_TRY(hipEventRecord(sc.ev1, st));
    }
    HIP_TRY(hipMemsetAsync(static_cast<char*>(h->xb) + (size_t)n_new * rb, 0, (size_t)removed * rb, st));
    HIP_TRY(hipMemsetAsync(h->norms + n_new, 0, (size_t)removed * sizeof(float), st));
    if (h->xh) {
        HIP_TRY(hipMemsetAsync(static_cast<char*>(h->xh) + (size_t)n_new * hb, 0, (size_t)removed * hb, st));
        for (int i = 0; i < 3; i++)
            HIP_TRY(hipMemsetAsync(h->hmeta + (size_t)i * h->cap + n_new, 0, (size_t)removed * sizeof(float), st));
    }
    if (h->xq8) {
        HIP_TRY(hipMemsetAsync(static_cast<char*>(h->xq8) + (size_t)n_new * qb, 0, (size_t)removed * qb, st));
        HIP_TRY(hipMemsetAsync(h->bmeta + n_new, 0, (size_t)removed * sizeof(uint32_t), st));
    }
    h->n = n_new;
    h->row_epoch++;
    h->norms_rows = meta ? n_new : 0;
    const long long mu_rows_old = h->mu_rows;
    h->mu_rows = std::min(h->mu_rows, n_new);
    if (uses_shift(h) && !h->shift_pinned && n_new * 4 < mu_rows_old * 3) h->mu_rows = 0;
    HIP_TRY(hipGetLastError());
    HIP_TRY(hipStreamSynchronize(st));
    h->remove_last_ms = 0.f;
    h->remove_last_bytes = 0;
    if (moved > 0) {
        (void)hipEventElapsedTime(&h->remove_last_ms, sc.ev0, sc.ev1);
        const size_t per_row = rb + (mv_h ? hb + 12 : 0) + (mv_q ? qb + 4 : 0) + (meta ? 4 : 0);
        h->remove_last_bytes = (unsigned long long)moved * per_row;
    }
    h->remove_calls++;
    h->remove_rows += (unsigned long long)removed;
    h->remove_moved += (unsigned long long)moved;
    return ISE_OK;
}

extern "C" int ise_index_remove_range(ise_index_t* h, int64_t i0, int64_t i1, int64_t* n_removed) {
    if (!h) return fail(ISE_E_INVALID, "handle is NULL");
    if (n_removed) *n_removed = 0;
    std::lock_guard<std::mutex> lr(h->rg_mu);
    std::lock_guard<std::mutex> lk(h->mu_);
    const long long a = std::max<long long>(i0, 0), b = std::min<long long>(i1, h->n);
    if (a >= b) return ISE_OK;
    DeviceGuard gd(h->device);
    const int rc = remove_runs_locked(h, {RemoveRun{a, b - a}}, b - a);
    if (rc == ISE_OK && n_removed) *n_removed = b - a;
    return rc;
}

extern "C" int ise_index_remove_ids_host(ise_index_t* h, const int64_t* ids, int64_t n_ids, int64_t* n_removed) {
    if (!h) return fail(ISE_E_INVALID, "handle is NULL");
    if (n_removed) *n_removed = 0;
    if (n_ids < 0 || (n_ids > 0 && !ids)) return fail(ISE_E_INVALID, "ids is NULL");
    if (n_ids == 0) return ISE_OK;
    std::vector<long long> v;
    std::vector<RemoveRun> runs;
    try {
        v.reserve((size_t)n_ids);
        for (int64_t i = 0; i < n_ids; i++)
            if (ids[i] >= 0) v.push_back(ids[i]);
        std::sort(v.begin(), v.end());
        v.erase(std::unique(v.begin(), v.end()), v.end());
    } catch (const std::bad_alloc&) {
        return fail(ISE_E_NOMEM, "remove_ids: host allocation failed");
    }
    std::lock_guard<std::mutex> lr(h->rg_mu);
    std::lock_guard<std::mutex> lk(h->mu_);
    long long removed = 0;
    try {
        for (long long id : v) {
            if (id >= h->n) break;
            if (!runs.empty() && runs.back().start + runs.back().len == id) runs.back().len++;
            else runs.push_back(RemoveRun{id, 1});
            removed++;
        }
    } catch (const std::bad_alloc&) {
        return fail(ISE_E_NOMEM, "remove_ids: host allocation failed");
    }
    if (removed == 0) return ISE_OK;
    DeviceGuard gd(h->device);
    const int rc = remove_runs_locked(h, runs, removed);
    if (rc == ISE_OK && n_removed) *n_removed = removed;
    return rc;
}

extern "C" int ise_index_remove_stats(ise_index_t* h, uint64_t* out3) {
    if (!h || !out3) return fail(ISE_E_INVALID, "NULL argument");
    std::lock_guard<std::mutex> lk(h->mu_);
    out3[0] = h->remove_calls;
    out3[1] = h->remove_rows;
    out3[2] = h->remove_moved;
    return ISE_OK;
}

extern "C" int ise_index_remove_last_timing(ise_index_t* h, float* ms, uint64_t* bytes) {
    if (!h || !ms || !bytes) return fail(ISE_E_INVALID, "NULL argument");
    std::lock_guard<std::mutex> lk(h->mu_);
    *ms = h->remove_last_ms;
    *bytes = h->remove_last_bytes;
    return ISE_OK;
}

extern "C" int ise_index_range_stats(ise_index_t* h, uint64_t* out2) {
    if (!h || !out2) return fail(ISE_E_INVALID, "NULL argument");
    std::lock_guard<std::mutex> lk(h->rg_mu);
    out2[0] = h->range_batches;
    out2[1] = h->range_overflows;
    return ISE_OK;
}

extern "C" int ise_index_short_stats(ise_index_t* h, uint64_t* out1) {
    if (!h || !out1) return fail(ISE_E_INVALID, "NULL argument");
    std::lock_guard<std::mutex> lk(h->mu_);
    out1[0] = h->short_batches;
    return ISE_OK;
}

extern "C" int ise_index_half_stats(ise_index_t* h, uint64_t* out1) {
    if (!h || !out1) return fail(ISE_E_INVALID, "NULL argument");
    std::lock_guard<std::mutex> lk(h->mu_);
    out1[0] = h->half_batches;
    return ISE_OK;
}

extern "C" int ise_index_byte_stats(ise_index_t* h, uint64_t* out2) {
    if (!h || !out2) return fail(ISE_E_INVALID, "NULL argument");
    std::lock_guard<std::mutex> lk(h->mu_);
    out2[0] = h->byte_batches;
    out2[1] = (h->xq8 && byte_rel_ok(h)) ? 1 : 0;
    return ISE_OK;
}

extern "C" int ise_index_byte_row(ise_index_t* h, int64_t i, float* out2) {
    if (!h || !out2) return fail(ISE_E_INVALID, "NULL argument");
    std::lock_guard<std::mutex> lk(h->mu_);
    if (i < 0 || i >= h->n) return fail(ISE_E_INVALID, "row out of range");
    DeviceGuard gd(h->device);
    int rc = prepare_shift_locked(h, h->stream);
    if (rc) return rc;
    if (!h->xq8) return fail(ISE_E_INVALID, "this index has no byte shadow rows");
    HIP_TRY(hipDeviceSynchronize());
    uint32_t m = 0;
    HIP_TRY(hipMemcpy(&m, h->bmeta + i, sizeof(uint32_t), hipMemcpyDeviceToHost));
    uint32_t cb = m << 16, eb = m >> 16;
    float cr;
    memcpy(&cr, &cb, sizeof(float));
    const _Float16 eh = __builtin_bit_cast(_Float16, (unsigned short)eb);
    out2[0] = cr;
    out2[1] = cr * (float)eh;
    return ISE_OK;
}

extern "C" int ise_index_shadow_row(ise_index_t* h, int64_t i, float* out3) {
    if (!h || !out3) return fail(ISE_E_INVALID, "NULL argument");
    std::lock_guard<std::mutex> lk(h->mu_);
    if (i < 0 || i >= h->n) return fail(ISE_E_INVALID, "row out of range");
    DeviceGuard gd(h->device);
    int rc = prepare_shift_locked(h, h->stream);
    if (rc) return rc;
    if (!h->xh) return fail(ISE_E_INVALID, "this index has no shadow rows");
    HIP_TRY(hipDeviceSynchronize());
    for (int j = 0; j < 3; j++)
        HIP_TRY(hipMemcpy(out3 + j, h->hmeta + (size_t)j * h->cap + i, sizeof(float), hipMemcpyDeviceToHost));
    return ISE_OK;
}

extern "C" int ise_index_stage_query_debug(ise_index_t* h, const void* q_dev, int route, void* limbs, int64_t limbs_bytes,
                                           float* out2, int32_t* info3) {
    if (!h || !q_dev || !limbs || !out2 || !info3) return fail(ISE_E_INVALID, "NULL argument");
    if (route != 0 && route != 1) return fail(ISE_E_INVALID, "route: 0 = fp16 shadow, 1 = byte shadow");
    std::lock_guard<std::mutex> lk(h->mu_);
    DeviceGuard gd(h->device);
    int rc = prepare_shift_locked(h, h->stream);
    if (rc) return rc;
    if (route == 1 ? !h->xq8 : !h->xh) return fail(ISE_E_INVALID, "this index has no such shadow rows");
    const int P = route == 1 ? h->dpb : h->dph, es = route == 1 ? 1 : 2;
    const size_t need = (size_t)2 * P * es;
    if (P > 1024 || limbs_bytes < (int64_t)need) return fail(ISE_E_INVALID, "limbs: room for hi and lo of the padded row needed");
    unsigned char* dev = nullptr;
    HIP_TRY(hipMalloc(&dev, need + 16));
    float* out_f = reinterpret_cast<float*>(dev + need);
    int* out_i = reinterpret_cast<int*>(dev + need + 8);
    if (route == 1)
        hipLaunchKernelGGL(stage_debug_kernel<true>, dim3(1), dim3(32), 0, h->stream, (const float*)q_dev, h->mu, h->d, P, dev, out_f, out_i);
    else
        hipLaunchKernelGGL(stage_debug_kernel<false>, dim3(1), dim3(32), 0, h->stream, (const float*)q_dev, h->mu, h->d, P, dev, out_f, out_i);
    hipError_t e = hipGetLastError();
    if (e == hipSuccess) e = hipStreamSynchronize(h->stream);
    std::vector<unsigned char> host(need + 16);
    if (e == hipSuccess) e = hipMemcpy(host.data(), dev, need + 16, hipMemcpyDeviceToHost);
    (void)hipFree(dev);
    HIP_TRY(e);
    memcpy(limbs, host.data(), need);
    memcpy(out2, host.data() + need, 8);
    memcpy(info3, host.data() + need + 8, 8);
    info3[2] = P;
    return ISE_OK;
}

extern "C" int ise_index_host_stats(ise_index_t* h, uint64_t* out3) {
    if (!h || !out3) return fail(ISE_E_INVALID, "NULL argument");
    {
        std::lock_guard<std::mutex> lk(h->cq_mu);
        out3[0] = h->cq_batches;
        out3[1] = h->cq_requests;
    }
    std::lock_guard<std::mutex> lk(h->mu_);
    out3[2] = h->direct_queries;
    return ISE_OK;
}

extern "C" int ise_index_reserve_workspaces(ise_index_t* h, int64_t nq, int k) {
    int rc = check_search_args(h, h, nq, k);
    if (rc) return rc;
    if (nq == 0) return ISE_OK;
    std::lock_guard<std::mutex> lk(h->mu_);
    DeviceGuard gd(h->device);
    rc = prepare_shift_locked(h, h->stream);
    if (rc) return rc;
    ScanPlan pl;
    rc = plan_for_batch(h, nq, k, &pl);
    if (rc) return rc;
    return ensure_workspaces(h, pl, pl.gemm ? std::min<long long>(nq, GEMM_NQ_MAX) : nq);
}

extern "C" int ise_index_stats(ise_index_t* h, uint64_t* out4) {
    if (!h || !out4) return fail(ISE_E_INVALID, "NULL argument");
    std::lock_guard<std::mutex> lk(h->mu_);
    DeviceGuard gd(h->device);
    HIP_TRY(hipDeviceSynchronize());
    unsigned long long tmp[4];
    HIP_TRY(hipMemcpy(tmp, h->stats_dev, sizeof(tmp), hipMemcpyDeviceToHost));
#ifdef ISE_ABLATE
    if (getenv("ISE_DEBUG_STAMPS")) {
        unsigned long long st[16];
        if (hipMemcpy(st, h->stats_dev + 8, sizeof(st), hipMemcpyDeviceToHost) == hipSuccess) {
            fprintf(stderr, "merge/rerank stamps (us since kernel entry):");
            for (int i = 1; i < 8; i++) fprintf(stderr, " [%d] %.2f", i, (double)(long long)(st[i] - st[0]) / 100.0);
            fprintf(stderr, "\n");
        }
    }
#endif
    out4[0] = tmp[0];
    out4[1] = tmp[1];
    out4[2] = h->mu_updates;
    out4[3] = h->gemm_chunks;
    return ISE_OK;
}

static int assign_stage_rows(const ise_index* h) {
    const size_t per = (size_t)(qs_stride_for(h) + 1) * 4;
    int cs = (int)std::min<size_t>(ASSIGN_CS_MAX, (150 * 1024) / per) / 16 * 16;
    return cs;
}
static size_t assign_lds_bytes(const ise_index* h) {
    return (size_t)assign_stage_rows(h) * (qs_stride_for(h) + 1) * 4;
}

template <int NS, int XT>
static void launch_assign(int grid, size_t lds, hipStream_t st, const AssignParams& ap) {
    static LdsAttrOnce attr;
    attr.ensure(reinterpret_cast<const void*>(&assign_kernel<NS, XT>), LDS_LIMIT);
    hipLaunchKernelGGL((assign_kernel<NS, XT>), dim3(grid), dim3(512), lds, st, ap);
}

static bool assign_supported(const ise_index* h) {
    return h->storage == ISE_STORE_F32 && h->dp <= 512 && h->n > 0 && assign_stage_rows(h) >= 16;
}

extern "C" int ise_index_assign_device(ise_index_t* h, const float* x_dev, int64_t n, float* D_dev, int64_t* I_dev,
                                       void* stream) {
    if (!h) return fail(ISE_E_INVALID, "handle is NULL");
    if (n < 0 || (n > 0 && (!x_dev || !I_dev))) return fail(ISE_E_INVALID, "bad argument");
    if (n == 0) return ISE_OK;
    std::lock_guard<std::mutex> lk(h->mu_);
    DeviceGuard gd(h->device);
    if (!assign_supported(h))
        return fail(ISE_E_INVALID, "assignment kernel needs a non-empty float32 index with d <= 512");
    {
        int rc = prepare_shift_locked(h, (hipStream_t)stream);
        if (rc) return rc;
    }
    AssignParams ap;
    ap.x = x_dev; ap.cb = (const float*)h->xb; ap.cnorm = h->norms; ap.mu = uses_shift(h) ? h->mu : nullptr; ap.n = n; ap.d = h->d; ap.dp = h->dp;
    ap.cs_stride = qs_stride_for(h); ap.K = (int)h->n; ap.metric = h->metric; ap.cs = assign_stage_rows(h);
    ap.I = (long long*)I_dev; ap.D = D_dev;
    const size_t lds = assign_lds_bytes(h);
    const int ns = h->dp / 16;
    const int xt = ns <= 8 ? 4 : (ns <= 16 ? 2 : 1);
    const long long rows_per_block = 8ll * xt * 16;
    const long long nslabs = (n + rows_per_block - 1) / rows_per_block;
    const int grid = (int)std::min<long long>(nslabs, (long long)h->num_cu);
    hipStream_t st = (hipStream_t)stream;
    switch (ns) {
        case 1: launch_assign<1, 4>(grid, lds, st, ap); break;
        case 2: launch_assign<2, 4>(grid, lds, st, ap); break;
        case 3: launch_assign<3, 4>(grid, lds, st, ap); break;
        case 4: launch_assign<4, 4>(grid, lds, st, ap); break;
        case 8: launch_assign<8, 4>(grid, lds, st, ap); break;
        case 12: launch_assign<12, 2>(grid, lds, st, ap); break;
        case 16: launch_assign<16, 2>(grid, lds, st, ap); break;
        case 20: launch_assign<20, 1>(grid, lds, st, ap); break;
        case 24: launch_assign<24, 1>(grid, lds, st, ap); break;
        case 28: launch_assign<28, 1>(grid, lds, st, ap); break;
        case 32: launch_assign<32, 1>(grid, lds, st, ap); break;
        default: return fail(ISE_E_INVALID, "unsupported padded dimension for the assignment kernel");
    }
    HIP_TRY(hipGetLastError());
    return ISE_OK;
}

extern "C" int ise_merge_keys_device(const uint64_t* keys_dev, int n_lists, int64_t nq, int k, int metric, float* D_dev,
                                     int64_t* I_dev, int device, void* stream) {
    if (!keys_dev || !D_dev || !I_dev) return fail(ISE_E_INVALID, "NULL pointer");
    if (n_lists <= 0 || n_lists > MERGE_LISTS_MAX) return fail(ISE_E_INVALID, "n_lists must be in [1, 1024]");
    if (k <= 0 || k > ISE_MAX_K || nq < 0 || nq > (1ll << 20)) return fail(ISE_E_INVALID, "bad nq / k");
    if (metric != ISE_METRIC_L2 && metric != ISE_METRIC_INNER_PRODUCT) return fail(ISE_E_INVALID, "bad metric");
    if (nq == 0) return ISE_OK;
    DeviceGuard gd(device);
    MergeParams mp;
    mp.lists = (const u64*)keys_dev;
    mp.stride_list = (long long)nq * k;
    mp.stride_qtile = (long long)k; mp.qt = 1;
    mp.n_lists = n_lists; mp.nq = (int)nq; mp.k = k; mp.metric = metric;
    mp.D = D_dev; mp.I = (long long*)I_dev; mp.keys_out = nullptr;
    mp.fl_state = nullptr; mp.fl_list = nullptr; mp.seq = 0; mp.out_by_pos = 0; mp.dbg = nullptr; mp.gate = nullptr;
    if (n_lists <= 64)
        hipLaunchKernelGGL(merge_small_kernel, dim3((unsigned)((nq + 3) / 4)), dim3(256), 0, (hipStream_t)stream, mp);
    else
        launch_merge<false>((unsigned)nq, 0, (hipStream_t)stream, mp, ExactParams());
    HIP_TRY(hipGetLastError());
    return ISE_OK;
}

extern "C" int ise_normalize_rows_device(float* x_dev, int64_t n, int d, int device, void* stream) {
    if (n < 0 || d <= 0 || (n > 0 && !x_dev)) return fail(ISE_E_INVALID, "bad argument");
    if (n == 0) return ISE_OK;
    if (n >= (1ll << 32)) return fail(ISE_E_INVALID, "too many rows");
    DeviceGuard gd(device);
    hipLaunchKernelGGL(normalize_kernel, dim3((unsigned)((n + 3) / 4)), dim3(256), 0, (hipStream_t)stream, x_dev,
                       (long long)n, d);
    HIP_TRY(hipGetLastError());
    return ISE_OK;
}

extern "C" int ise_bovw_histogram_device(const int64_t* labels_dev, const int64_t* offsets_dev, int64_t n_images, int K,
                                         double* out_dev, int device, void* stream) {
    if (n_images < 0 || K <= 0 || (n_images > 0 && (!offsets_dev || !out_dev)))
        return fail(ISE_E_INVALID, "bad argument");
    if (K > HIST_K_MAX) return fail(ISE_E_INVALID, "histogram: at most 16384 bins");
    if (n_images == 0) return ISE_OK;
    if (n_images >= (1ll << 31)) return fail(ISE_E_INVALID, "too many images");
    DeviceGuard gd(device);
    hipLaunchKernelGGL(bovw_histogram_kernel, dim3((unsigned)n_images), dim3(256), (size_t)K * sizeof(unsigned int),
                       (hipStream_t)stream, (const long long*)labels_dev, (const long long*)offsets_dev, K, out_dev);
    HIP_TRY(hipGetLastError());
    return ISE_OK;
}

extern "C" int ise_normalize_rows_host(float* x, int64_t n, int d, int device) {
    if (n < 0 || d <= 0 || (n > 0 && !x)) return fail(ISE_E_INVALID, "bad argument");
    if (n == 0) return ISE_OK;
    int ndev = 0;
    if (hipGetDeviceCount(&ndev) != hipSuccess || ndev <= 0)
        return fail(ISE_E_NODEVICE, "no HIP device visible: normalize_L2 runs on the GPU");
    DeviceGuard gd(device);
    const long long slab = std::max<long long>(1, (256ll << 20) / ((long long)d * 4));
    float* tmp = nullptr;
    HIP_TRY(hipMalloc(&tmp, (size_t)std::min<long long>(slab, n) * d * sizeof(float)));
    int rc = ISE_OK;
    for (long long i0 = 0; i0 < n && rc == ISE_OK; i0 += slab) {
        const long long m = std::min<long long>(slab, n - i0);
        hipError_t e = hipMemcpy(tmp, x + (size_t)i0 * d, (size_t)m * d * sizeof(float), hipMemcpyHostToDevice);
        if (e == hipSuccess) {
            hipLaunchKernelGGL(normalize_kernel, dim3((unsigned)((m + 3) / 4)), dim3(256), 0, 0, tmp, m, d);
            e = hipGetLastError();
        }
        if (e == hipSuccess)
            e = hipMemcpy(x + (size_t)i0 * d, tmp, (size_t)m * d * sizeof(float), hipMemcpyDeviceToHost);
        if (e != hipSuccess) rc = fail(ISE_E_HIP, std::string("normalize: ") + hipGetErrorString(e));
    }
    (void)hipFree(tmp);
    return rc;
}
```

### image-search-engine_amd/csrc/ise_scan.hpp

```cpp
#pragma once
#include "ise_common.hpp"
#include "ise_scan_params.hpp"
#include "ise_select.hpp"
#include "ise_stage.hpp"

#ifndef ISE_FINAL_FILTER
#define ISE_FINAL_FILTER 1
#endif

#ifdef ISE_ABLATE
#define ABL(bit) (p.ablate & (bit))
#define STAMP(i)                                                                                   \
    do {                                                                                           \
        if (p.stamps && lane == 0)                                                                 \
            p.stamps[((size_t)blockIdx.x * W + w) * 16 + (i)] = __builtin_amdgcn_s_memrealtime();  \
    } while (0)
#define CSTAMP(i)                                                                                  \
    do {                                                                                           \
        if (p.stamps && lane == 0)                                                                 \
            p.stamps[((size_t)blockIdx.x * W + w) * 16 + (i)] = __builtin_amdgcn_s_memtime();      \
    } while (0)
#else
#define ABL(bit) 0
#define STAMP(i) do {} while (0)
#define CSTAMP(i) do {} while (0)
#endif

template <int CH, int W, int T, bool BF16, bool SHIFT, int RM = ROWS_OWN>
__global__ __launch_bounds__(W * 64, T == 1 ? W / 2 : (W / 4 > 0 ? W / 4 : 1)) void scan_kernel(const ScanParams p) {
    constexpr bool HALF = RM == ROWS_F16, BYTE = RM == ROWS_I8, SHADOW = HALF || BYTE;
    static_assert(!(BF16 && SHIFT), "the shift is applied to fp32 rows only");
    static_assert(!SHADOW || SHIFT, "shadow rows belong to float32 L2 indexes");
    constexpr bool F32S = SHIFT && !SHADOW;
    if (p.gate && *p.gate == 0u) return;
    constexpr int BLOCK_THREADS = W * 64;
    constexpr bool XCHG = T >= 3 || (T == 2 && W == 8) || (RM == ROWS_I8 && T == 1 && W == 8);
    constexpr bool FFILT = XCHG && ISE_FINAL_FILTER;
    constexpr int NQ = 16 * T;
    constexpr int TPR = W >= 16 ? 32 : BLOCK_THREADS / 16;
    constexpr int KPLB = (W * 16 + 63) / 64;
    constexpr int KPLF = (KB_MAX + W * CAP + 63) / 64;
    static_assert(KB_MAX + CAP <= 64 && MERGE_TRIG + 4 <= CAP, "list sizes");
    extern __shared__ __align__(16) unsigned char smem[];
    const int S = p.qs_stride;
    const int kb = p.kb;
    float* mus = reinterpret_cast<float*>(smem);
    float* qs = mus + S;
    float* xn = qs + NQ * S;
    float* xe = xn + NQ;
    int* xsh = reinterpret_cast<int*>(xe + NQ);
    u64* tauS = reinterpret_cast<u64*>(xn + (SHADOW ? 3 : 1) * NQ);
    int* bwc = reinterpret_cast<int*>(tauS + NQ);
    int* lockS = bwc + NQ;
    int* cntS = lockS + NQ;
    u64* bootw = reinterpret_cast<u64*>(cntS + W * NQ);
    u64* cand = bootw + NQ * kb;
    u64* boot = cand;

    const int tid = threadIdx.x, lane = tid & 63, w = __builtin_amdgcn_readfirstlane(tid >> 6);
    const int c = lane & 15, g = lane >> 4;
    const int q0 = blockIdx.y * NQ;
    const int nqt = min(NQ, p.nq - q0);
    const int k = p.k;
    const int nsteps = p.row_slots >> 2;
    const int t0 = blockIdx.x * p.tiles_per_block;
    const int t1 = min(t0 + p.tiles_per_block, p.tiles_total);
    const bool l2 = p.metric == ISE_METRIC_L2;
    STAMP(0);

    auto load_chunk = [&](f32x4(&a)[CH], int tile, int s0) {
        const char* base = static_cast<const char*>(p.xb) +
                           ((((size_t)tile * 16 + c) * p.row_slots + 4 * s0 + g) << 4);
        if (ABL(32)) base = static_cast<const char*>(p.xb) + (((size_t)c * p.row_slots + g) << 4);
        if (ABL(128)) return;
#pragma unroll
        for (int s = 0; s < CH; s++) a[s] = *reinterpret_cast<const f32x4*>(base + 64 * s);
    };
    auto load_norms = [&](int tile) -> f32x4 {
        return *reinterpret_cast<const f32x4*>(p.norms + (size_t)tile * 16 + 4 * g);
    };
    auto load_meta = [&](const void* m, int tile) -> f32x4 {
        if constexpr (!SHADOW) return (f32x4){0.f, 0.f, 0.f, 0.f};
        return *reinterpret_cast<const f32x4*>(static_cast<const float*>(m) + (size_t)tile * 16 + 4 * g);
    };

    constexpr int FPS = BF16 ? 2 : 1;
    constexpr int QV = 8;
    constexpr int QVS = QV / FPS;
    const int S4 = S >> 2;
    const int dslots = BF16 ? (p.d >> 3) : (p.d >> 2);
    const bool vec_q = !SHADOW && (p.d & (BF16 ? 7 : 3)) == 0 && ((reinterpret_cast<uintptr_t>(p.q) & 15) == 0) &&
                       S4 <= TPR * QVS;
    f32x4 qv[T][QV];
    f32x4 muv[F32S ? QVS : 1];
    const bool stager = tid < 16 * TPR;
    if (F32S && vec_q && stager) {
#pragma unroll
        for (int i = 0; i < QVS; i++) {
            const int j4 = tid % TPR + i * TPR;
            muv[i] = (f32x4){0.f, 0.f, 0.f, 0.f};
            if (j4 < dslots) muv[i] = *reinterpret_cast<const f32x4*>(p.mu + 4 * j4);
        }
    }
    if (vec_q && stager) {
#pragma unroll
        for (int tq = 0; tq < T; tq++) {
            const int cc = tq * 16 + tid / TPR, t = tid % TPR;
            const bool rowok = cc < nqt && !ABL(1);
            const float* src = p.q + (size_t)(q0 + (rowok ? cc : 0)) * p.d;
#pragma unroll
            for (int i = 0; i < QVS; i++) {
                const int j4 = t + i * TPR;
#pragma unroll
                for (int f = 0; f < FPS; f++) {
                    qv[tq][i * FPS + f] = (f32x4){0.f, 0.f, 0.f, 0.f};
                    if (rowok && j4 < dslots)
                        qv[tq][i * FPS + f] = *reinterpret_cast<const f32x4*>(src + 4 * (j4 * FPS + f));
                }
            }
        }
    }
    const int PS = p.row_slots * (BYTE ? 16 : 8);
    const bool vec_s = SHADOW && W < 16 && shadow_vec_ok(p.d, PS, p.q, TPR);
    f32x4 sqv[SHADOW ? T : 1][SHADOW_QV], smuv[SHADOW_QV];
    auto shadow_src = [&](int tq) -> const float* {
        const int cc = tq * 16 + tid / TPR;
        return p.q + (size_t)(q0 + ((cc < nqt && !ABL(1)) ? cc : 0)) * p.d;
    };
    if constexpr (SHADOW) {
        if (vec_s && stager) {
            stage_request_row(smuv, p.mu, tid % TPR, TPR, p.d >> 2);
#pragma unroll
            for (int tq = 0; tq < T; tq++) stage_request_row(sqv[tq], shadow_src(tq), tid % TPR, TPR, p.d >> 2);
        }
    }
    __builtin_amdgcn_sched_barrier(0);

    constexpr int R = (T == 1 || W >= 16) ? 2 : (T == 2 ? 4 : (T == 3 ? 3 : 2));
    const bool has_work = (t0 + w) < t1 && !ABL(16);
    f32x4 A[R][CH];
    int ltile = t0 + w, ls0 = 0;
    auto advance_load = [&]() {
        int ns = ls0 + CH, nt = ltile;
        if (ns >= nsteps) { ns = 0; nt = ltile + W; }
        if (nt < t1) { ltile = nt; ls0 = ns; }
    };
    if (has_work) {
#pragma unroll
        for (int j = 0; j < R - 1; j++) {
            load_chunk(A[j], ltile, ls0);
            advance_load();
        }
    }
    __builtin_amdgcn_sched_barrier(0);

    auto to_bf16_pair = [](float lo, float hi) -> uint32_t {
        const __bf16 a = (__bf16)lo, b = (__bf16)hi;
        return (uint32_t)__builtin_bit_cast(unsigned short, a) | ((uint32_t)__builtin_bit_cast(unsigned short, b) << 16);
    };
    auto bf16_round = [](float v) -> float { return (float)(__bf16)v; };
#pragma unroll
    for (int tq = 0; tq < T; tq++) {
        if (!stager) continue;
        const int cc = tq * 16 + tid / TPR, t = tid % TPR;
        float sn = 0.f;
        if (vec_q) {
#pragma unroll
            for (int i = 0; i < QVS; i++) {
                const int j4 = t + i * TPR;
                if (j4 < S4) {
                    if (BF16) {
                        const f32x4 v0 = qv[tq][i * FPS], v1 = qv[tq][i * FPS + FPS - 1];
                        u32x4 o;
                        o[0] = to_bf16_pair(v0[0], v0[1]);
                        o[1] = to_bf16_pair(v0[2], v0[3]);
                        o[2] = to_bf16_pair(v1[0], v1[1]);
                        o[3] = to_bf16_pair(v1[2], v1[3]);
                        *reinterpret_cast<u32x4*>(qs + cc * S + 4 * j4) = o;
#pragma unroll
                        for (int e = 0; e < 4; e++) {
                            const float r0 = bf16_round(v0[e]), r1 = bf16_round(v1[e]);
                            sn = fmaf(r0, r0, sn);
                            sn = fmaf(r1, r1, sn);
                        }
                    } else {
                        f32x4 v = qv[tq][i];
                        if (F32S) {
                            if (cc < nqt) v = v - muv[i];
                            if (cc == 0) *reinterpret_cast<f32x4*>(mus + 4 * j4) = muv[i];
                        }
                        *reinterpret_cast<f32x4*>(qs + cc * S + 4 * j4) = v;
                        sn = fmaf(v[0], v[0], sn);
                        sn = fmaf(v[1], v[1], sn);
                        sn = fmaf(v[2], v[2], sn);
                        sn = fmaf(v[3], v[3], sn);
                        if (F32S) sn += nonfinite_mark(qv[tq][i]);
                    }
                }
            }
        } else if (SHADOW) {
            if constexpr (SHADOW) {
                const bool rowok = cc < nqt && !ABL(1);
                unsigned char* hi = reinterpret_cast<unsigned char*>(qs + cc * S);
                unsigned char* lo = hi + 16 * p.row_slots;
                if (vec_s) {
                    float amax, mark;
                    stage_shadow_vec_scale<TPR>(sqv[tq], smuv, shadow_src(tq), p.mu, p.d >> 2, rowok, t, PS >> 2, tq > 0,
                                                amax, mark);
                    stage_shadow_vec_limbs<BYTE, TPR>(sqv[tq], smuv, shadow_src(tq), p.mu, p.d >> 2, rowok, t, PS >> 2,
                                                      amax, mark, hi, lo, xn + cc, xe + cc, xsh + cc);
                } else {
                    stage_shadow_scalar<BYTE, TPR>(shadow_src(tq), p.mu, p.d, PS, rowok, t, hi, lo, xn + cc, xe + cc,
                                                   xsh + cc);
                }
            }
        } else {
            const bool rowok = cc < nqt && !ABL(1);
            const float* src = p.q + (size_t)(q0 + (rowok ? cc : 0)) * p.d;
            constexpr int SB = 8;
            for (int j0 = t; j0 < S; j0 += SB * TPR) {
                float lo[SB], hi[SB], m[SB];
#pragma unroll
                for (int b = 0; b < SB; b++) {
                    const int j = j0 + b * TPR;
                    lo[b] = hi[b] = m[b] = 0.f;
                    if (BF16) {
                        if (rowok && j < S && 2 * j < p.d) lo[b] = src[2 * j];
                        if (rowok && j < S && 2 * j + 1 < p.d) hi[b] = src[2 * j + 1];
                    } else {
                        if (SHIFT && j < S && j < p.d) m[b] = p.mu[j];
                        if (rowok && j < S && j < p.d) lo[b] = src[j];
                    }
                }
#pragma unroll
                for (int b = 0; b < SB; b++) {
                    const int j = j0 + b * TPR;
                    if (j < S) {
                        if (BF16) {
                            reinterpret_cast<uint32_t*>(qs)[cc * S + j] = to_bf16_pair(lo[b], hi[b]);
                            const float r0 = bf16_round(lo[b]), r1 = bf16_round(hi[b]);
                            sn = fmaf(r0, r0, sn);
                            sn = fmaf(r1, r1, sn);
                        } else {
                            const float v = (rowok && j < p.d) ? lo[b] - m[b] : 0.f;
                            qs[cc * S + j] = v;
                            if (SHIFT && cc == 0) mus[j] = m[b];
                            sn = fmaf(v, v, sn);
                            if (SHIFT) sn += nonfinite_mark(lo[b]);
                        }
                    }
                }
            }
        }
        if (!SHADOW) {
#pragma unroll
            for (int o = TPR / 2; o > 0; o >>= 1) sn += __shfl_xor(sn, o);
            if (t == 0) xn[cc] = sn;
        }
    }
    for (int i = tid; i < NQ; i += BLOCK_THREADS) {
        tauS[i] = TAU0;
        bwc[i] = 0;
        lockS[i] = 0;
    }
    __syncthreads();
    STAMP(1);
    CSTAMP(8);

    const float* qrow = qs + c * S + 4 * g;
    const bool use_floor = p.floor_keys != nullptr;

    float xq_n[T], xq_e[T], xq_r[T];
    int xq_sh[T];
    u64 tau[T];
    int cnt[T];
    f32x4 acc0[T], acc1[T];
#pragma unroll
    for (int t = 0; t < T; t++) {
        xq_n[t] = xn[t * 16 + c];
        xq_e[t] = SHADOW ? xe[t * 16 + c] : 0.f;
        xq_sh[t] = SHADOW ? xsh[t * 16 + c] : 0;
        xq_r[t] = BYTE ? sqrtf(xq_n[t]) + 0x1p-60f : 0.f;
        tau[t] = TAU0;
        cnt[t] = 0;
        acc0[t] = (f32x4){0.f, 0.f, 0.f, 0.f};
        acc1[t] = (f32x4){0.f, 0.f, 0.f, 0.f};
    }
    u64 xbound = KEY_PAD;
    bool booted = false;

    auto merge_out = [&](int t, int cq) {
        const int qq = t * 16 + cq;
        const int n_ = __builtin_amdgcn_readlane(cnt[t], cq);
        const u64* buf = cand + (size_t)(w * NQ + qq) * CAP;
        if (lane == 0)
            while (atomicCAS(&lockS[qq], 0, 1) != 0) __builtin_amdgcn_s_sleep(1);
        wave_lds_fence();
        const int nb = bwc[qq];
        u64 kk[1];
        kk[0] = lane < nb ? bootw[qq * kb + lane] : (lane - nb < n_ ? buf[lane - nb] : KEY_PAD);
        wave_lds_fence();
        u64 ktau = KEY_PAD;
        const int nw = wave_select<1>(kk, nb + n_, k, bootw + qq * kb, &ktau);
        if (lane == 0) {
            bwc[qq] = nw;
            if (nw == k) tauS[qq] = min_u64(tauS[qq], ktau);
        }
        wave_lds_fence();
        if (lane == 0) atomicExch(&lockS[qq], 0);
        if (c == cq) {
            cnt[t] = 0;
            if (nw == k) tau[t] = min_u64(tau[t], ktau);
        }
    };

    auto boot_phase = [&](const u64(&key)[T][4]) {
        STAMP(2);
#pragma unroll
        for (int t = 0; t < T; t++)
#pragma unroll
            for (int j = 0; j < 4; j++) boot[(size_t)(t * 16 + c) * (W * 16) + w * 16 + 4 * g + j] = key[t][j];
        __syncthreads();
        STAMP(7);
        for (int qq = w; qq < NQ; qq += W) {
            u64 kk[KPLB];
#pragma unroll
            for (int e = 0; e < KPLB; e++)
                kk[e] = (lane + 64 * e) < W * 16 ? boot[(size_t)qq * (W * 16) + lane + 64 * e] : KEY_PAD;
            u64 ktau = TAU0;
            const int nw = wave_cut<KPLB>(kk, W * 16, k, kb, bootw + qq * kb, &ktau);
            u64 best = kk[0];
#pragma unroll
            for (int e = 1; e < KPLB; e++) best = min_u64(best, kk[e]);
            best = wave_min_u64(best);
            if (lane == 0) {
                bwc[qq] = nw;
                tauS[qq] = ktau;
                if (XCHG && p.xchg)
                    __hip_atomic_store(p.xchg + ((size_t)blockIdx.y * NQ + qq) * gridDim.x + blockIdx.x,
                                       ((u64)p.xchg_seq << 32) | (best >> 32), __ATOMIC_RELAXED,
                                       __HIP_MEMORY_SCOPE_AGENT);
            }
        }
        __syncthreads();
#pragma unroll
        for (int t = 0; t < T; t++) tau[t] = tauS[t * 16 + c];
        booted = true;
        STAMP(3);
    };

    auto score = [&](int t, float dotj, float ynj, float yej, float ysj) -> float {
        if constexpr (HALF) return half_lower_bound(p.beta, p.lo_shrink, xq_n[t] + ynj,
                                                    ldexpf(dotj, -((int)ysj + xq_sh[t])), yej + xq_e[t]);
        if constexpr (BYTE) {
            const uint32_t m = __float_as_uint(yej);
            const float cr = __uint_as_float(m << 16);
            const float er = cr * (float)__builtin_bit_cast(_Float16, (unsigned short)(m >> 16));
            return byte_lower_bound(p.beta, p.lo_shrink, xq_n[t], ynj, ldexpf(dotj * cr, -xq_sh[t]), xq_r[t],
                                    sqrtf(ynj) + 0x1p-60f, er, xq_e[t]);
        }
        if (l2) {
            const float tt = xq_n[t] + ynj;
            const float sc = tt - 2.f * dotj;
            if (SHIFT) return l2_lower_bound(p.beta, tt, sc);
            return sc < 0.f ? 0.f : sc;
        }
        return -dotj;
    };
    auto make_keys = [&](int etile, const f32x4(&sc)[T], u64(&key)[T][4]) {
        const long long row0 = (long long)etile * 16 + 4 * g;
#pragma unroll
        for (int t = 0; t < T; t++)
#pragma unroll
            for (int j = 0; j < 4; j++) {
                bool ok = (row0 + j < p.n) && (sc[t][j] < FLT_MAX) && (t * 16 + c < nqt);
                const u64 kj = ((u64)ord_f32(sc[t][j]) << 32) | (uint32_t)((uint32_t)(row0 + j) + p.id_base);
                if (use_floor) ok = ok && (kj > p.floor_keys[q0 + min(t * 16 + c, nqt - 1)]);
                key[t][j] = ok ? kj : KEY_PAD;
            }
    };

    float tau_sc[T];
#pragma unroll
    for (int t = 0; t < T; t++) tau_sc[t] = FLT_MAX;

    auto epilogue = [&](int etile, f32x4 yn, f32x4 ye, f32x4 ys) {
        f32x4 sc[T];
#pragma unroll
        for (int t = 0; t < T; t++) {
            f32x4 dot = acc0[t] + acc1[t];
            if constexpr (BYTE) {
                const i32x4 ah = __builtin_bit_cast(i32x4, acc0[t]), al = __builtin_bit_cast(i32x4, acc1[t]);
#pragma unroll
                for (int j = 0; j < 4; j++) dot[j] = fmaf(256.f, (float)ah[j], (float)al[j]);
            }
            acc0[t] = (f32x4){0.f, 0.f, 0.f, 0.f};
            acc1[t] = (f32x4){0.f, 0.f, 0.f, 0.f};
#pragma unroll
            for (int j = 0; j < 4; j++) sc[t][j] = score(t, dot[j], yn[j], ye[j], ys[j]);
        }
        if (!booted) {
            u64 key[T][4];
            make_keys(etile, sc, key);
            boot_phase(key);
#pragma unroll
            for (int t = 0; t < T; t++) tau_sc[t] = unord_f32((uint32_t)(tau[t] >> 32));
            return;
        }
#pragma unroll
        for (int t = 0; t < T; t++) {
            tau[t] = min_u64(tau[t], tauS[t * 16 + c]);
            tau_sc[t] = unord_f32((uint32_t)(tau[t] >> 32));
        }
        u64 hit[T][4];
        u64 any_hit = 0;
#pragma unroll
        for (int t = 0; t < T; t++)
#pragma unroll
            for (int j = 0; j < 4; j++) {
                hit[t][j] = __ballot(sc[t][j] <= tau_sc[t]);
                any_hit |= hit[t][j];
            }
        if (any_hit && !ABL(2)) {
            const long long row0 = (long long)etile * 16 + 4 * g;
            const u64 qmask = 0x0001000100010001ull << c;
            const u64 lt_mask = (1ull << lane) - 1ull;
#pragma unroll
            for (int t = 0; t < T; t++) {
                u64* mybuf = cand + (size_t)(w * NQ + t * 16 + c) * CAP;
#pragma unroll
                for (int j = 0; j < 4; j++) {
                    if (hit[t][j]) {
                        const float s_ = sc[t][j];
                        bool ok = (row0 + j < p.n) && (s_ < FLT_MAX) && (t * 16 + c < nqt);
                        const u64 kj = ((u64)ord_f32(s_) << 32) | (uint32_t)((uint32_t)(row0 + j) + p.id_base);
                        if (use_floor) ok = ok && (kj > p.floor_keys[q0 + min(t * 16 + c, nqt - 1)]);
                        const bool v = ok && kj < tau[t];
                        const u64 m = __ballot(v);
                        if (m) {
                            const u64 mq = m & qmask;
                            if (v) mybuf[cnt[t] + __popcll(mq & lt_mask)] = kj;
                            cnt[t] += __popcll(mq);
                            u64 nm = __ballot(cnt[t] >= MERGE_TRIG) & 0xFFFFull;
                            while (nm) {
                                const int cq = __ffsll((long long)nm) - 1;
                                nm &= nm - 1;
                                merge_out(t, cq);
                            }
                        }
                    }
                }
                tau_sc[t] = unord_f32((uint32_t)(tau[t] >> 32));
            }
        }
    };

    auto exchange = [&]() {
        const int nb = (int)gridDim.x;
        const int G = (nb + 255) >> 8;
        for (int qq = w; qq < NQ; qq += W) {
            const u64* src = p.xchg + ((size_t)blockIdx.y * NQ + qq) * nb;
            auto slot_value = [&](int slot) -> uint32_t {
                uint32_t best = 0xFFFFFFFFu;
                for (int j = 0; j < G; j++) {
                    const int i = slot * G + j;
                    if (i < nb) {
                        const u64 v = __hip_atomic_load(src + i, __ATOMIC_RELAXED, __HIP_MEMORY_SCOPE_AGENT);
                        if ((uint32_t)(v >> 32) == p.xchg_seq) best = min(best, (uint32_t)v);
                    }
                }
                return best;
            };
            const uint32_t v0 = slot_value(lane), v1 = slot_value(lane + 64), v2 = slot_value(lane + 128),
                           v3 = slot_value(lane + 192);
            uint32_t prefix = 0;
            int rank = k;
            for (int b = 31; b >= 0; b--) {
                const uint32_t hm = b == 31 ? 0u : 0xFFFFFFFFu << (b + 1);
                auto zero_here = [&](uint32_t v) { return ((v ^ prefix) & hm) == 0u && ((v >> b) & 1u) == 0u; };
                const int c0 = __popcll(__ballot(zero_here(v0))) + __popcll(__ballot(zero_here(v1))) +
                               __popcll(__ballot(zero_here(v2))) + __popcll(__ballot(zero_here(v3)));
                if (rank > c0) {
                    rank -= c0;
                    prefix |= 1u << b;
                }
            }
            if (prefix != 0xFFFFFFFFu) {
                const u64 bound = ((u64)prefix << 32) | 0xFFFFFFFFull;
                if (FFILT && lane == (qq - w) / W) xbound = bound;
                if (lane == 0) {
                    while (atomicCAS(&lockS[qq], 0, 1) != 0) __builtin_amdgcn_s_sleep(1);
                }
                wave_lds_fence();
                if (lane == 0 && bound < tauS[qq]) tauS[qq] = bound;
                wave_lds_fence();
                if (lane == 0) atomicExch(&lockS[qq], 0);
            }
        }
    };

    f32x4 bcur[T], bcur_lo[SHADOW ? T : 1];
    auto load_b = [&](f32x4(&b)[T], f32x4(&blo)[SHADOW ? T : 1], int step) {
        if (ABL(512)) return;
#pragma unroll
        for (int t = 0; t < T; t++) {
            b[t] = *reinterpret_cast<const f32x4*>(qrow + (size_t)t * 16 * S + 16 * step);
            if constexpr (SHADOW) blo[t] = *reinterpret_cast<const f32x4*>(qrow + (size_t)t * 16 * S + 4 * p.row_slots + 16 * step);
        }
    };
    auto compute_chunk = [&](const f32x4(&a)[CH], int s0, int next_first_step) {
#pragma unroll
        for (int s = 0; s < CH; s++) {
            f32x4 bnext[T], bnext_lo[SHADOW ? T : 1];
            if (ABL(64)) {
#pragma unroll
                for (int t = 0; t < T; t++) acc0[t] += a[s];
                continue;
            }
            load_b(bnext, bnext_lo, s + 1 < CH ? s0 + s + 1 : next_first_step);
            f32x4 as = a[s];
            if (F32S && !ABL(1024)) as = as - *reinterpret_cast<const f32x4*>(mus + 4 * g + 16 * (s0 + s));
#pragma unroll
            for (int t = 0; t < T; t++) {
                if (BYTE) {
                    const i32x4 av = __builtin_bit_cast(i32x4, a[s]);
                    acc0[t] = __builtin_bit_cast(f32x4, __builtin_amdgcn_mfma_i32_16x16x64_i8(
                                                            av, __builtin_bit_cast(i32x4, bcur[t]),
                                                            __builtin_bit_cast(i32x4, acc0[t]), 0, 0, 0));
                    acc1[t] = __builtin_bit_cast(f32x4, __builtin_amdgcn_mfma_i32_16x16x64_i8(
                                                            av, __builtin_bit_cast(i32x4, bcur_lo[t]),
                                                            __builtin_bit_cast(i32x4, acc1[t]), 0, 0, 0));
                } else if (HALF) {
                    const f16x8 av = __builtin_bit_cast(f16x8, a[s]);
                    acc0[t] = __builtin_amdgcn_mfma_f32_16x16x32_f16(av, __builtin_bit_cast(f16x8, bcur[t]), acc0[t], 0, 0, 0);
                    acc1[t] = __builtin_amdgcn_mfma_f32_16x16x32_f16(av, __builtin_bit_cast(f16x8, bcur_lo[t]), acc1[t], 0, 0, 0);
                } else if (BF16) {
                    const bf16x8 av = __builtin_bit_cast(bf16x8, a[s]), bv = __builtin_bit_cast(bf16x8, bcur[t]);
                    if (s & 1) acc1[t] = __builtin_amdgcn_mfma_f32_16x16x32_bf16(av, bv, acc1[t], 0, 0, 0);
                    else acc0[t] = __builtin_amdgcn_mfma_f32_16x16x32_bf16(av, bv, acc0[t], 0, 0, 0);
                } else {
                    acc0[t] = __builtin_amdgcn_mfma_f32_16x16x4f32(as[0], bcur[t][0], acc0[t], 0, 0, 0);
                    acc1[t] = __builtin_amdgcn_mfma_f32_16x16x4f32(as[1], bcur[t][1], acc1[t], 0, 0, 0);
                    acc0[t] = __builtin_amdgcn_mfma_f32_16x16x4f32(as[2], bcur[t][2], acc0[t], 0, 0, 0);
                    acc1[t] = __builtin_amdgcn_mfma_f32_16x16x4f32(as[3], bcur[t][3], acc1[t], 0, 0, 0);
                }
            }
#pragma unroll
            for (int t = 0; t < T; t++) {
                bcur[t] = bnext[t];
                if constexpr (SHADOW) bcur_lo[t] = bnext_lo[t];
            }
        }
    };

    if (has_work) {
        int tile = t0 + w, s0 = 0;
        int tiles_done = 0;
        bool exchanged = !XCHG || p.xchg == nullptr || ABL(256);
        load_b(bcur, bcur_lo, 0);
        bool done = false;
        while (!done) {
#pragma unroll
            for (int j = 0; j < R; j++) {
                if (!done) {
                    const f32x4 yn = load_norms(tile);
                    const f32x4 ye = load_meta(BYTE ? (const void*)p.bmeta : p.herr, tile);
                    const f32x4 ys = HALF ? load_meta(p.hexp, tile) : (f32x4){0.f, 0.f, 0.f, 0.f};
                    load_chunk(A[(j + R - 1) % R], ltile, ls0);
                    advance_load();
                    __builtin_amdgcn_sched_barrier(0);
                    int ns0 = s0 + CH, ntile = tile;
                    if (ns0 >= nsteps) { ns0 = 0; ntile = tile + W; }
                    compute_chunk(A[j], s0, ns0);
                    if (ns0 == 0 && !ABL(8) && !(ABL(2048) && booted)) epilogue(tile, yn, ye, ys);
                    if (ns0 == 0) tiles_done++;
                    done = ntile >= t1;
                    tile = ntile; s0 = ns0;
                }
            }
            if constexpr (XCHG) {
                if (!exchanged && tiles_done >= 1) {
                    if (t1 - tile >= 4 * W) exchange();
                    exchanged = true;
                }
            }
        }
    }
    if (!booted) {
        u64 none[T][4];
#pragma unroll
        for (int t = 0; t < T; t++)
#pragma unroll
            for (int j = 0; j < 4; j++) none[t][j] = KEY_PAD;
        boot_phase(none);
    }

    STAMP(4);
    CSTAMP(9);
#pragma unroll
    for (int t = 0; t < T; t++)
        if (g == 0) cntS[w * NQ + t * 16 + c] = cnt[t];
    __syncthreads();
    STAMP(5);
    for (int qq = w; qq < NQ && !ABL(4); qq += W) {
        int P[W + 2];
        P[0] = 0;
        P[1] = bwc[qq];
#pragma unroll
        for (int i = 0; i < W; i++) P[i + 2] = P[i + 1] + cntS[i * NQ + qq];
        const int n = P[W + 1];
        u64 bnd = KEY_PAD;
        if constexpr (FFILT) {
            if (!use_floor && !ABL(8192)) bnd = readlane_u64(xbound, (qq - w) / W);
        }
        u64 kk[KPLF];
#pragma unroll
        for (int e = 0; e < KPLF; e++) {
            kk[e] = KEY_PAD;
            const int idx = lane + 64 * e;
            if (64 * e < n) {
                if (idx < P[1]) kk[e] = bootw[qq * kb + idx];
#pragma unroll
                for (int i = 0; i < W; i++)
                    if (idx >= P[i + 1] && idx < P[i + 2])
                        kk[e] = cand[(size_t)(i * NQ + qq) * CAP + idx - P[i + 1]];
                if (FFILT && kk[e] > bnd) kk[e] = KEY_PAD;
            }
        }
        u64* out = p.part + (((size_t)blockIdx.y * gridDim.x + blockIdx.x) * NQ + qq) * k;
        u64 kth_unused;
        const int nw = wave_select<KPLF>(kk, n, k, out, &kth_unused);
        if (lane >= nw && lane < k) out[lane] = KEY_PAD;
    }
    STAMP(6);
}
```

### image-search-engine_amd/csrc/ise_scan_params.hpp

```cpp
#pragma once
#include "ise_common.hpp"

enum RowMode : int { ROWS_OWN = 0, ROWS_F16 = 1, ROWS_I8 = 2 };

struct ScanParams {
    const void* xb;
    const float* norms;
    const float* herr = nullptr;
    const float* hexp = nullptr;
    const uint32_t* bmeta = nullptr;
    const float* q;
    const float* mu;
    const u64* floor_keys;
    u64* part;
    long long n;
    int d, dp, qs_stride;
    int row_slots;
    int nq, k, kb, metric;
    uint32_t id_base;
    float beta;
    float lo_shrink = 1.f;
    int tiles_total, tiles_per_block;
    unsigned long long* xchg;
    uint32_t xchg_seq;
    const unsigned int* gate;
    int ablate;
    unsigned long long* stamps;
};

#define CAP 16
#define MERGE_TRIG 12
#define KB_MAX 48

#define LDS_LIMIT (160 * 1024)

__host__ __device__ constexpr size_t scan_lds_layout(int S, int waves, int T, int kb, bool shadow = false) {
    return (size_t)S * 4  +
           (size_t)(16 * T) * ((size_t)S * 4 + 4  + (shadow ? 8 : 0)  + 8  + 8  +
                               (size_t)waves * 4  + (size_t)kb * 8  +
                               (size_t)waves * CAP * 8 );
}

void ise_launch_scan_f32_shift(int ch, int waves, int T, dim3 grid, size_t lds, hipStream_t st, const ScanParams& sp);
void ise_launch_scan_f32_plain(int ch, int waves, int T, dim3 grid, size_t lds, hipStream_t st, const ScanParams& sp);
void ise_launch_scan_bf16(int ch, int waves, int T, dim3 grid, size_t lds, hipStream_t st, const ScanParams& sp);
void ise_launch_scan_f16_shadow(int ch, int waves, int T, dim3 grid, size_t lds, hipStream_t st, const ScanParams& sp);
void ise_launch_scan_i8_shadow(int ch, int waves, int T, dim3 grid, size_t lds, hipStream_t st, const ScanParams& sp);
```

### image-search-engine_amd/csrc/ise_select.hpp

```cpp
#pragma once
#include "ise_common.hpp"


template <int KPL>
__device__ __forceinline__ int wave_select(const u64 (&kk)[KPL], int n, int k, u64* dst, u64* kth) {
    int nreal = 0;
#pragma unroll
    for (int e = 0; e < KPL; e++)
        if (64 * e < n) nreal += __popcll(__ballot(kk[e] != KEY_PAD));
    u64 kstar = KEY_PAD - 1;
    if (nreal > k && nreal > 40) {
        u64 L = 0, H = KEY_PAD;
        int t = k - 1;
        for (int round = 0;; round++) {
            u64 P = 0;
            bool found = false;
            const int rot = (round * 23 + 7) & 63;
#pragma unroll
            for (int e = 0; e < KPL; e++) {
                if (64 * e < n && !found) {
                    const u64 m = __ballot(kk[e] > L && kk[e] < H);
                    if (m) {
                        const u64 hi = (m >> rot) << rot;
                        P = readlane_u64(kk[e], __ffsll((long long)(hi ? hi : m)) - 1);
                        found = true;
                    }
                }
            }
            int c_lt = 0;
#pragma unroll
            for (int e = 0; e < KPL; e++)
                if (64 * e < n) c_lt += __popcll(__ballot(kk[e] > L && kk[e] < P));
            if (c_lt == t) {
                kstar = P;
                break;
            }
            if (c_lt > t) {
                H = P;
            } else {
                L = P;
                t -= c_lt + 1;
            }
        }
    }
    int rk[KPL];
#pragma unroll
    for (int e = 0; e < KPL; e++) rk[e] = 0;
#pragma unroll
    for (int es = 0; es < KPL; es++) {
        if (64 * es < n) {
            u64 m = __ballot(kk[es] <= kstar);
            while (m) {
                const int l = __ffsll((long long)m) - 1;
                m &= m - 1;
                const u64 ki = readlane_u64(kk[es], l);
#pragma unroll
                for (int e = 0; e < KPL; e++) rk[e] += (ki < kk[e]) ? 1 : 0;
            }
        }
    }
    u64 kth_key = 0;
#pragma unroll
    for (int e = 0; e < KPL; e++) {
        if (64 * e < n) {
            const bool win = kk[e] <= kstar && rk[e] < k;
            if (win) dst[rk[e]] = kk[e];
            const u64 hit = __ballot(win && rk[e] == k - 1);
            if (hit) kth_key = readlane_u64(kk[e], __ffsll((long long)hit) - 1);
        }
    }
    const int nw = min(nreal, k);
    if (nw == k) *kth = kth_key;
    return nw;
}

template <int KPL>
__device__ __forceinline__ int wave_cut(const u64 (&kk)[KPL], int n, int kmin, int kmax, u64* dst, u64* cut) {
    const int lane = threadIdx.x & 63;
    const u64 lt_mask = (1ull << lane) - 1ull;
    int nreal = 0;
    u64 mx = 0;
#pragma unroll
    for (int e = 0; e < KPL; e++)
        if (64 * e < n) nreal += __popcll(__ballot(kk[e] != KEY_PAD));
    u64 P = KEY_PAD - 1;
    int cnt = nreal;
    if (nreal > kmax) {
        u64 L = 0, H = KEY_PAD;
        int base = 0;
        for (int round = 0;; round++) {
            u64 piv = 0;
            bool found = false;
            const int rot = (round * 23 + 7) & 63;
#pragma unroll
            for (int e = 0; e < KPL; e++) {
                if (64 * e < n && !found) {
                    const u64 m = __ballot(kk[e] > L && kk[e] < H);
                    if (m) {
                        const u64 hi = (m >> rot) << rot;
                        piv = readlane_u64(kk[e], __ffsll((long long)(hi ? hi : m)) - 1);
                        found = true;
                    }
                }
            }
            int c = base;
#pragma unroll
            for (int e = 0; e < KPL; e++)
                if (64 * e < n) c += __popcll(__ballot(kk[e] > L && kk[e] <= piv));
            if (c < kmin) {
                L = piv;
                base = c;
            } else if (c > kmax) {
                H = piv;
            } else {
                P = piv;
                cnt = c;
                break;
            }
        }
    } else if (nreal >= kmin) {
#pragma unroll
        for (int e = 0; e < KPL; e++)
            if (64 * e < n) {
                const u64 v = kk[e] == KEY_PAD ? 0ull : kk[e];
                mx = mx > v ? mx : v;
            }
#pragma unroll
        for (int o = 32; o > 0; o >>= 1) {
            const u64 other = __shfl_xor(mx, o);
            mx = mx > other ? mx : other;
        }
        P = mx;
    }
    int off = 0;
#pragma unroll
    for (int e = 0; e < KPL; e++) {
        if (64 * e < n) {
            const bool keep = kk[e] <= P;
            const u64 m = __ballot(keep);
            if (keep) dst[off + __popcll(m & lt_mask)] = kk[e];
            off += __popcll(m);
        }
    }
    if (cnt >= kmin) *cut = P;
    return cnt;
}


template <int KPL>
__device__ __forceinline__ void block_topk_part(const u64* list, int n, int base, int per, int k, u64* dst) {
    const int lane = threadIdx.x & 63;
    u64 kk[KPL];
#pragma unroll
    for (int e = 0; e < KPL; e++) {
        const int idx = base + lane + 64 * e;
        kk[e] = (64 * e < per && idx < n) ? list[idx] : KEY_PAD;
    }
    u64 kth_unused = 0;
    const int nw = wave_select<KPL>(kk, per < 64 * KPL ? per : 64 * KPL, k, dst, &kth_unused);
    for (int i = nw + lane; i < k; i += 64) dst[i] = KEY_PAD;
}
__device__ __forceinline__ void block_topk_u64(const u64* list, int n, int k, u64* stage, u64* out) {
    const int lane = threadIdx.x & 63, w = __builtin_amdgcn_readfirstlane((int)threadIdx.x >> 6);
    const int per = (((n + 3) >> 2) + 63) & ~63;
    const int base = w * per;
    if (per <= 64) block_topk_part<1>(list, n, base, per, k, stage + w * k);
    else if (per <= 256) block_topk_part<4>(list, n, base, per, k, stage + w * k);
    else if (per <= 512) block_topk_part<8>(list, n, base, per, k, stage + w * k);
    else block_topk_part<16>(list, n, base, per, k, stage + w * k);
    __syncthreads();
    if (w == 0) {
        u64 kk[4];
#pragma unroll
        for (int e = 0; e < 4; e++) kk[e] = (lane + 64 * e) < 4 * k ? stage[lane + 64 * e] : KEY_PAD;
        u64 kth_unused = 0;
        const int nw = wave_select<4>(kk, 4 * k, k, out, &kth_unused);
        for (int i = nw + lane; i < k; i += 64) out[i] = KEY_PAD;
    }
    __syncthreads();
}
```

### image-search-engine_amd/faiss_compat.py

```python
from __future__ import annotations

import ctypes
import struct
import threading

import numpy as np

from . import _native as _n

METRIC_INNER_PRODUCT = _n.METRIC_INNER_PRODUCT
METRIC_L2 = _n.METRIC_L2

_FLT_MAX = float(np.finfo(np.float32).max)


def _as_rows(x, d=None) -> np.ndarray:
    x = np.ascontiguousarray(np.asarray(x), dtype=np.float32)
    assert x.ndim == 2, "expected a 2-D array"
    if d is not None:
        assert x.shape[1] == d, f"dimension mismatch: got {x.shape[1]}, index has d={d}"
    return x


def _default_device() -> int:
    import torch

    return torch.cuda.current_device() if torch.cuda.is_available() else 0


def _ids_array(ids) -> np.ndarray:
    return np.ascontiguousarray(np.asarray(ids).reshape(-1), dtype=np.int64)


def _runs_of_sorted(ids: np.ndarray) -> np.ndarray:
    if ids.size == 0:
        return np.zeros((0, 2), dtype=np.int64)
    brk = np.flatnonzero(np.diff(ids) != 1) + 1
    starts = np.concatenate(([0], brk))
    ends = np.concatenate((brk, [ids.size]))
    return np.stack([ids[starts], ends - starts], axis=1).astype(np.int64)


class IDSelector:

    def is_member(self, i: int) -> bool:
        raise NotImplementedError

    def runs(self, n: int) -> np.ndarray:
        raise NotImplementedError

    def members(self, ids) -> np.ndarray:
        return np.fromiter((self.is_member(int(i)) for i in _ids_array(ids)), dtype=bool, count=len(_ids_array(ids)))


class IDSelectorRange(IDSelector):

    def __init__(self, imin: int, imax: int):
        self.imin, self.imax = int(imin), int(imax)

    def is_member(self, i: int) -> bool:
        return self.imin <= int(i) < self.imax

    def runs(self, n: int) -> np.ndarray:
        a, b = max(self.imin, 0), min(self.imax, int(n))
        return np.array([[a, b - a]], dtype=np.int64) if a < b else np.zeros((0, 2), dtype=np.int64)

    def members(self, ids) -> np.ndarray:
        ids = _ids_array(ids)
        return (ids >= self.imin) & (ids < self.imax)


class IDSelectorBatch(IDSelector):

    def __init__(self, ids):
        self.ids = np.unique(_ids_array(ids))

    def is_member(self, i: int) -> bool:
        p = int(np.searchsorted(self.ids, int(i)))
        return p < self.ids.size and int(self.ids[p]) == int(i)

    def runs(self, n: int) -> np.ndarray:
        return _runs_of_sorted(self.ids[(self.ids >= 0) & (self.ids < int(n))])

    def members(self, ids) -> np.ndarray:
        return np.isin(_ids_array(ids), self.ids)


class IDSelectorArray(IDSelectorBatch):
    """Faiss's linear-scan form of IDSelectorBatch: the same members."""


class IDSelectorNot(IDSelector):

    def __init__(self, sel: IDSelector):
        self.sel = sel

    def is_member(self, i: int) -> bool:
        return not self.sel.is_member(i)

    def runs(self, n: int) -> np.ndarray:
        n = int(n)
        r = self.sel.runs(n)
        starts = np.concatenate(([0], r[:, 0] + r[:, 1]))
        ends = np.concatenate((r[:, 0], [n]))
        keep = ends > starts
        return np.stack([starts[keep], (ends - starts)[keep]], axis=1).astype(np.int64)

    def members(self, ids) -> np.ndarray:
        return ~self.sel.members(ids)


class SearchParameters:

    def __init__(self, sel=None):
        if sel is not None and not isinstance(sel, (IDSelector, DeviceSelector)):
            raise TypeError(f"SearchParameters.sel must be an IDSelector or a DeviceSelector, not {type(sel).__name__}")
        self.sel = sel


def _params_sel(params):
    if params is None:
        return None
    if not isinstance(params, SearchParameters):
        raise TypeError(f"params must be a SearchParameters, not {type(params).__name__}")
    return params.sel


def _bitmap_words(members: np.ndarray) -> np.ndarray:
    members = np.asarray(members, dtype=bool).reshape(-1)
    nw = (members.size + 31) // 32
    by = np.zeros(4 * nw, dtype=np.uint8)
    packed = np.packbits(members, bitorder="little")
    by[:packed.size] = packed
    return by.view("<u4")


def lower_selector(sel: IDSelector, ntotal: int):
    if isinstance(sel, IDSelectorRange):
        return ("range", sel.imin, sel.imax)
    if isinstance(sel, IDSelectorBatch):
        return ("ids", sel.ids, 0)
    if isinstance(sel, IDSelectorNot) and isinstance(sel.sel, IDSelectorBatch):
        return ("ids", sel.sel.ids, 1)
    if not isinstance(sel, IDSelector):
        raise TypeError(f"expected an IDSelector, not {type(sel).__name__}")
    return ("bitmap", _bitmap_words(sel.members(np.arange(int(ntotal), dtype=np.int64))))


class DeviceSelector:

    def __init__(self, index: "IndexFlat", lowered):
        self.index = index
        self._s = ctypes.c_void_p()
        kind = lowered[0]
        if kind == "range":
            _n.check(_n.lib.ise_selector_create_range(index._h, int(lowered[1]), int(lowered[2]), ctypes.byref(self._s)))
        elif kind == "ids":
            ids = _ids_array(lowered[1])
            _n.check(_n.lib.ise_selector_create_ids(index._h, ids.ctypes.data, ids.size, int(lowered[2]),
                                                    ctypes.byref(self._s)))
        else:
            words = np.ascontiguousarray(lowered[1], dtype="<u4")
            _n.check(_n.lib.ise_selector_create_bitmap(index._h, words.ctypes.data, words.size, ctypes.byref(self._s)))

    def close(self) -> None:
        s = getattr(self, "_s", None)
        if s is not None and s.value:
            try:
                _n.lib.ise_selector_destroy(s)
            except Exception:
                pass
            s.value = None

    __del__ = close

    def info(self) -> dict:
        out = (ctypes.c_int64 * 5)()
        _n.check(_n.lib.ise_selector_info(self._s, out))
        return {"ntotal": int(out[0]), "selected": int(out[1]), "window": (int(out[2]), int(out[3])),
                "tiles": int(out[4])}


def _runs_to_ids(runs: np.ndarray) -> np.ndarray:
    if len(runs) == 0:
        return np.zeros(0, dtype=np.int64)
    return np.concatenate([np.arange(a, a + m, dtype=np.int64) for a, m in runs])


class IndexFlat:

    def __init__(self, d: int, metric: int = METRIC_L2, device: int | None = None, storage: str = "f32"):
        self.d = int(d)
        self.metric_type = int(metric)
        self.is_trained = True
        self.storage = storage
        self.device = _default_device() if device is None else int(device)
        self._h = ctypes.c_void_p()
        self._lock = threading.Lock()
        store = {"f32": _n.STORE_F32, "bf16": _n.STORE_BF16}[storage]
        _n.check(_n.lib.ise_index_create_ex(ctypes.byref(self._h), self.d, self.metric_type, self.device, store))

    def __del__(self):
        h = getattr(self, "_h", None)
        if h is not None and h.value:
            try:
                _n.lib.ise_index_destroy(h)
            except Exception:
                pass
            h.value = None

    @property
    def ntotal(self) -> int:
        n = ctypes.c_int64(0)
        _n.check(_n.lib.ise_index_info(self._h, None, None, ctypes.byref(n), None))
        return int(n.value)

    def reset(self) -> None:
        _n.check(_n.lib.ise_index_reset(self._h))

    def exact_stats(self) -> dict:
        out = (ctypes.c_uint64 * 4)()
        _n.check(_n.lib.ise_index_stats(self._h, out))
        return {"reranked": int(out[0]), "exact_scan": int(out[1]), "shift_updates": int(out[2]),
                "gemm_chunks": int(out[3])}

    def host_stats(self) -> dict:
        out = (ctypes.c_uint64 * 3)()
        _n.check(_n.lib.ise_index_host_stats(self._h, out))
        return {"combined_batches": int(out[0]), "combined_calls": int(out[1]), "direct_queries": int(out[2])}

    def short_stats(self) -> dict:
        out = (ctypes.c_uint64 * 1)()
        _n.check(_n.lib.ise_index_short_stats(self._h, out))
        return {"short_batches": int(out[0])}

    def half_stats(self) -> dict:
        out = (ctypes.c_uint64 * 1)()
        _n.check(_n.lib.ise_index_half_stats(self._h, out))
        return {"half_batches": int(out[0])}

    def byte_stats(self) -> dict:
        out = (ctypes.c_uint64 * 2)()
        _n.check(_n.lib.ise_index_byte_stats(self._h, out))
        return {"byte_batches": int(out[0]), "byte_route": bool(out[1])}

    def byte_row(self, i: int) -> tuple:
        out = (ctypes.c_float * 2)()
        _n.check(_n.lib.ise_index_byte_row(self._h, int(i), out))
        return float(out[0]), float(out[1])

    def shadow_row(self, i: int) -> tuple:
        out = (ctypes.c_float * 3)()
        _n.check(_n.lib.ise_index_shadow_row(self._h, int(i), out))
        return float(out[0]), float(out[1]), int(out[2])

    def stage_query_debug(self, q: "torch.Tensor", route: str) -> dict:
        import torch
        assert q.is_cuda and q.dtype == torch.float32 and q.dim() == 1 and q.is_contiguous() and q.numel() == self.d
        es = {"half": 2, "byte": 1}[route]
        buf = np.zeros(2 * 1024 * es, dtype=np.uint8)
        out, info = (ctypes.c_float * 2)(), (ctypes.c_int32 * 3)()
        torch.cuda.synchronize()
        _n.check(_n.lib.ise_index_stage_query_debug(self._h, q.data_ptr(), es == 1, buf.ctypes.data, buf.nbytes, out, info))
        P = int(info[2])
        limbs = buf[: 2 * P * es].view(np.int8 if es == 1 else np.float16).reshape(2, P)
        return {"hi": limbs[0].copy(), "lo": limbs[1].copy(), "sh": int(info[0]), "vec": bool(info[1]),
                "vn2": float(out[0]), "eq": float(out[1])}

    def range_stats(self) -> dict:
        out = (ctypes.c_uint64 * 2)()
        _n.check(_n.lib.ise_index_range_stats(self._h, out))
        return {"range_batches": int(out[0]), "range_overflow_batches": int(out[1])}

    def reserve(self, nq: int, k: int) -> None:
        _n.check(_n.lib.ise_index_reserve_workspaces(self._h, int(nq), int(k)))

    def get_shift(self) -> np.ndarray:
        mu = np.zeros(self.d, dtype=np.float32)
        _n.check(_n.lib.ise_index_get_shift(self._h, mu.ctypes.data))
        return mu

    def set_shift(self, mu) -> None:
        mu = np.ascontiguousarray(mu, dtype=np.float32)
        assert mu.shape == (self.d,)
        _n.check(_n.lib.ise_index_set_shift(self._h, mu.ctypes.data))

    def add(self, x) -> None:
        x = _as_rows(x, self.d)
        _n.check(_n.lib.ise_index_add_host(self._h, x.ctypes.data, x.shape[0]))

    def add_torch(self, x) -> None:
        import torch

        assert x.is_cuda and x.dtype == torch.float32 and x.dim() == 2 and x.shape[1] == self.d
        x = x.contiguous()
        st = torch.cuda.current_stream(x.device).cuda_stream
        _n.check(_n.lib.ise_index_add_device(self._h, x.data_ptr(), x.shape[0], st))
        torch.cuda.current_stream(x.device).synchronize()

    def remove_ids(self, sel) -> int:
        out = ctypes.c_int64(0)
        if isinstance(sel, IDSelectorRange):
            _n.check(_n.lib.ise_index_remove_range(self._h, sel.imin, sel.imax, ctypes.byref(out)))
            return int(out.value)
        if isinstance(sel, IDSelectorBatch):
            ids = sel.ids
        elif isinstance(sel, IDSelector):
            ids = _runs_to_ids(sel.runs(self.ntotal))
        else:
            ids = _ids_array(sel)
        if ids.size:
            _n.check(_n.lib.ise_index_remove_ids_host(self._h, ids.ctypes.data, ids.size, ctypes.byref(out)))
        return int(out.value)

    def remove_stats(self) -> dict:
        out = (ctypes.c_uint64 * 3)()
        _n.check(_n.lib.ise_index_remove_stats(self._h, out))
        return {"remove_calls": int(out[0]), "rows_removed": int(out[1]), "rows_moved": int(out[2])}

    def remove_last_timing(self) -> tuple:
        ms, nb = ctypes.c_float(0), ctypes.c_uint64(0)
        _n.check(_n.lib.ise_index_remove_last_timing(self._h, ctypes.byref(ms), ctypes.byref(nb)))
        return float(ms.value), int(nb.value)

    def reconstruct_n(self, i0: int = 0, n: int | None = None) -> np.ndarray:
        n = self.ntotal - i0 if n is None else n
        out = np.empty((n, self.d), dtype=np.float32)
        _n.check(_n.lib.ise_index_reconstruct_host(self._h, i0, n, out.ctypes.data))
        return out

    ASSIGN_MIN_NQ = 2048

    def _assign_applies(self, nq: int, k: int) -> bool:
        return (k == 1 and nq >= self.ASSIGN_MIN_NQ and self.storage == "f32" and self.d <= 512
                and 0 < self.ntotal <= 65536)

    def assign_torch(self, x):
        import torch

        assert x.is_cuda and x.dtype == torch.float32 and x.dim() == 2 and x.shape[1] == self.d
        x = x.contiguous()
        n = x.shape[0]
        D = torch.empty((n, 1), dtype=torch.float32, device=x.device)
        I = torch.empty((n, 1), dtype=torch.int64, device=x.device)
        st = torch.cuda.current_stream(x.device).cuda_stream
        _n.check(_n.lib.ise_index_assign_device(self._h, x.data_ptr(), n, D.data_ptr(), I.data_ptr(), st))
        return D, I

    def make_selector(self, sel) -> DeviceSelector:
        return DeviceSelector(self, lower_selector(sel, self.ntotal))

    def _with_selector(self, sel, fn):
        if isinstance(sel, DeviceSelector):
            return fn(sel._s)
        ds = self.make_selector(sel)
        try:
            return fn(ds._s)
        finally:
            ds.close()

    def sel_stats(self) -> dict:
        out = (ctypes.c_uint64 * 3)()
        _n.check(_n.lib.ise_index_sel_stats(self._h, out))
        return {"sel_batches": int(out[0]), "sel_passes": int(out[1]), "sel_range_batches": int(out[2])}

    def search(self, x, k: int, params=None):
        x = _as_rows(x, self.d)
        k = int(k)
        assert k > 0
        nq = x.shape[0]
        sel = _params_sel(params)
        if sel is not None:
            D = np.empty((nq, k), dtype=np.float32)
            I = np.empty((nq, k), dtype=np.int64)
            self._with_selector(sel, lambda s: _n.check(_n.lib.ise_index_search_sel_host(
                self._h, x.ctypes.data, nq, k, s, D.ctypes.data, I.ctypes.data)))
            return D, I
        if self._assign_applies(nq, k):
            import torch

            D = np.empty((nq, 1), dtype=np.float32)
            I = np.empty((nq, 1), dtype=np.int64)
            dev = torch.device("cuda", self.device)
            step = max(1, (1 << 28) // (4 * self.d))
            for i0 in range(0, nq, step):
                d_, i_ = self.assign_torch(torch.from_numpy(x[i0:i0 + step]).to(dev))
                D[i0:i0 + step] = d_.cpu().numpy()
                I[i0:i0 + step] = i_.cpu().numpy()
            return D, I
        D = np.empty((nq, k), dtype=np.float32)
        I = np.empty((nq, k), dtype=np.int64)
        _n.check(_n.lib.ise_index_search_host(self._h, x.ctypes.data, nq, k, D.ctypes.data, I.ctypes.data))
        return D, I

    def range_search(self, x, radius: float, params=None):
        x = _as_rows(x, self.d)
        nq = x.shape[0]
        res = ctypes.c_void_p()
        sel = _params_sel(params)
        if sel is not None:
            self._with_selector(sel, lambda s: _n.check(_n.lib.ise_index_range_search_sel_host(
                self._h, x.ctypes.data, nq, ctypes.c_float(float(radius)), s, ctypes.byref(res))))
        else:
            _n.check(_n.lib.ise_index_range_search_host(self._h, x.ctypes.data, nq, ctypes.c_float(float(radius)),
                                                        ctypes.byref(res)))
        try:
            n = ctypes.c_int64()
            lp, dp_, ip = ctypes.c_void_p(), ctypes.c_void_p(), ctypes.c_void_p()
            _n.check(_n.lib.ise_range_result_get(res, ctypes.byref(n), ctypes.byref(lp), ctypes.byref(dp_),
                                                 ctypes.byref(ip)))
            lims = np.ctypeslib.as_array(ctypes.cast(lp, ctypes.POINTER(ctypes.c_int64)), (n.value + 1,))
            lims = lims.astype(np.uint64)
            total = int(lims[-1])
            D = np.empty(total, dtype=np.float32)
            I = np.empty(total, dtype=np.int64)
            if total:
                ctypes.memmove(D.ctypes.data, dp_.value, total * 4)
                ctypes.memmove(I.ctypes.data, ip.value, total * 8)
        finally:
            _n.lib.ise_range_result_destroy(res)
        return lims, D, I

    def search_torch(self, xq, k: int, params=None):
        import torch

        assert xq.is_cuda and xq.dtype == torch.float32 and xq.dim() == 2 and xq.shape[1] == self.d
        xq = xq.contiguous()
        nq = xq.shape[0]
        D = torch.empty((nq, k), dtype=torch.float32, device=xq.device)
        I = torch.empty((nq, k), dtype=torch.int64, device=xq.device)
        st = torch.cuda.current_stream(xq.device).cuda_stream
        sel = _params_sel(params)
        if sel is not None:
            def run(s):
                with self._lock:
                    _n.check(_n.lib.ise_index_search_sel_device(self._h, xq.data_ptr(), nq, int(k), s, D.data_ptr(),
                                                                I.data_ptr(), st))
            self._with_selector(sel, run)
            return D, I
        with self._lock:
            _n.check(_n.lib.ise_index_search_device(self._h, xq.data_ptr(), nq, int(k), D.data_ptr(),
                                                    I.data_ptr(), st))
        return D, I

    def search_into(self, xq, k: int, D, I, stream: int) -> None:
        with self._lock:
            _n.check(_n.lib.ise_index_search_device(self._h, xq.data_ptr(), xq.shape[0], int(k), D.data_ptr(),
                                                    I.data_ptr(), stream))

    def search_keys_into(self, xq, k: int, id_base: int, keys, stream: int) -> None:
        with self._lock:
            _n.check(_n.lib.ise_index_search_keys_device(self._h, xq.data_ptr(), xq.shape[0], int(k), int(id_base),
                                                         keys.data_ptr(), stream))

    def search_keys_torch(self, xq, k: int, id_base: int = 0):
        import torch

        assert xq.is_cuda and xq.dtype == torch.float32 and xq.dim() == 2 and xq.shape[1] == self.d
        xq = xq.contiguous()
        nq = xq.shape[0]
        keys = torch.empty((nq, k), dtype=torch.int64, device=xq.device)
        st = torch.cuda.current_stream(xq.device).cuda_stream
        with self._lock:
            _n.check(_n.lib.ise_index_search_keys_device(self._h, xq.data_ptr(), nq, int(k), int(id_base),
                                                         keys.data_ptr(), st))
        return keys

    def search_timed_torch(self, xq, k: int, iters: int):
        import torch

        xq = xq.contiguous()
        nq = xq.shape[0]
        D = torch.empty((nq, k), dtype=torch.float32, device=xq.device)
        I = torch.empty((nq, k), dtype=torch.int64, device=xq.device)
        st = torch.cuda.current_stream(xq.device).cuda_stream
        a, b = ctypes.c_float(0), ctypes.c_float(0)
        with self._lock:
            _n.check(_n.lib.ise_index_search_timed_device(self._h, xq.data_ptr(), nq, int(k), D.data_ptr(),
                                                          I.data_ptr(), st, int(iters), ctypes.byref(a),
                                                          ctypes.byref(b)))
        return D, I, float(a.value), float(b.value)


class IndexFlatL2(IndexFlat):
    def __init__(self, d: int, device: int | None = None, storage: str = "f32"):
        super().__init__(d, METRIC_L2, device, storage)


class IndexFlatIP(IndexFlat):
    def __init__(self, d: int, device: int | None = None, storage: str = "f32"):
        super().__init__(d, METRIC_INNER_PRODUCT, device, storage)


class _RowMask(IDSelector):

    def __init__(self, mask: np.ndarray):
        self.mask = np.asarray(mask, dtype=bool).reshape(-1)

    def is_member(self, i: int) -> bool:
        return 0 <= int(i) < self.mask.size and bool(self.mask[int(i)])

    def members(self, ids) -> np.ndarray:
        ids = _ids_array(ids)
        ok = (ids >= 0) & (ids < self.mask.size)
        out = np.zeros(ids.shape, dtype=bool)
        out[ok] = self.mask[ids[ok]]
        return out


class IndexIDMap:

    def __init__(self, index: IndexFlat):
        assert index.ntotal == 0, "IndexIDMap wraps an empty index (Faiss: index is empty on input)"
        self.index = index
        self.id_map = np.zeros(0, dtype=np.int64)

    d = property(lambda self: self.index.d)
    metric_type = property(lambda self: self.index.metric_type)
    is_trained = property(lambda self: self.index.is_trained)
    ntotal = property(lambda self: self.index.ntotal)

    def add(self, x) -> None:
        raise RuntimeError("add does not work with IndexIDMap, call add_with_ids")

    def add_with_ids(self, x, ids) -> None:
        x = _as_rows(x, self.index.d)
        ids = _ids_array(ids)
        assert ids.shape[0] == x.shape[0], "one id per row"
        self.index.add(x)
        self.id_map = np.concatenate((self.id_map, ids))

    def _map(self, I: np.ndarray) -> np.ndarray:
        out = np.full(I.shape, -1, dtype=np.int64)
        ok = I >= 0
        out[ok] = self.id_map[I[ok]]
        return out

    def _row_params(self, params):
        sel = _params_sel(params)
        if sel is None:
            return None
        if isinstance(sel, DeviceSelector):
            raise TypeError("IndexIDMap takes an IDSelector over external ids, not a DeviceSelector over rows")
        return SearchParameters(sel=_RowMask(sel.members(self.id_map)))

    def search(self, x, k: int, params=None):
        D, I = self.index.search(x, k, params=self._row_params(params))
# ... 376 lines not shown
```

### include/ise_knn.h

```cpp
#ifndef ISE_KNN_H
#define ISE_KNN_H

#include <stdint.h>

#ifdef __cplusplus
extern "C" {
#endif

#define ISE_METRIC_INNER_PRODUCT 0
#define ISE_METRIC_L2 1

#define ISE_STORE_F32 0
#define ISE_STORE_BF16 1

#define ISE_OK 0
#define ISE_E_INVALID -1
#define ISE_E_HIP -2
#define ISE_E_NOMEM -3
#define ISE_E_NODEVICE -4

#define ISE_MAX_K 2048

typedef struct ise_index ise_index_t;

int ise_version(void);
const char* ise_last_error(void);
int ise_device_count(int* count);
int ise_device_arch(int device, char* buf, int buflen);

int ise_index_create(ise_index_t** out, int d, int metric, int device);
int ise_index_create_ex(ise_index_t** out, int d, int metric, int device, int storage);
int ise_index_destroy(ise_index_t* h);
int ise_index_reset(ise_index_t* h);
int ise_index_info(const ise_index_t* h, int* d, int* metric, int64_t* ntotal, int* device);

int ise_index_add_host(ise_index_t* h, const float* x, int64_t n);
int ise_index_add_device(ise_index_t* h, const float* x_dev, int64_t n, void* stream);

int ise_index_set_shift(ise_index_t* h, const float* mu_host);
int ise_index_get_shift(ise_index_t* h, float* mu_host);

int ise_index_stats(ise_index_t* h, uint64_t* out4);

int ise_index_short_stats(ise_index_t* h, uint64_t* out1);

int ise_index_half_stats(ise_index_t* h, uint64_t* out1);
int ise_index_byte_stats(ise_index_t* h, uint64_t* out2);
int ise_index_shadow_row(ise_index_t* h, int64_t i, float* out3);
int ise_index_byte_row(ise_index_t* h, int64_t i, float* out2);

int ise_index_stage_query_debug(ise_index_t* h, const void* q_dev, int route, void* limbs, int64_t limbs_bytes,
                                float* out2, int32_t* info3);

int ise_refresh_env_knobs(void);

int ise_index_reserve_workspaces(ise_index_t* h, int64_t nq, int k);

int ise_index_reconstruct_host(ise_index_t* h, int64_t i0, int64_t n, float* out);

int ise_index_search_host(ise_index_t* h, const float* q, int64_t nq, int k,
                          float* D, int64_t* I);
int ise_index_host_stats(ise_index_t* h, uint64_t* out3);

typedef struct ise_range_result ise_range_result_t;
int ise_index_range_search_host(ise_index_t* h, const float* q, int64_t nq, float radius, ise_range_result_t** out);
int ise_range_result_get(const ise_range_result_t* r, int64_t* nq, const int64_t** lims, const float** D,
                         const int64_t** I);
int ise_range_result_destroy(ise_range_result_t* r);
int ise_index_range_stats(ise_index_t* h, uint64_t* out2);

int ise_index_remove_ids_host(ise_index_t* h, const int64_t* ids, int64_t n_ids, int64_t* n_removed);
int ise_index_remove_range(ise_index_t* h, int64_t i0, int64_t i1, int64_t* n_removed);
int ise_index_remove_stats(ise_index_t* h, uint64_t* out3);
int ise_index_remove_last_timing(ise_index_t* h, float* ms, uint64_t* bytes);
int ise_index_search_device(ise_index_t* h, const float* q_dev, int64_t nq, int k,
                            float* D_dev, int64_t* I_dev, void* stream);

typedef struct ise_selector ise_selector_t;
int ise_selector_create_range(ise_index_t* h, int64_t i0, int64_t i1, ise_selector_t** out);
int ise_selector_create_ids(ise_index_t* h, const int64_t* ids_host, int64_t n_ids, int invert, ise_selector_t** out);
int ise_selector_create_bitmap(ise_index_t* h, const uint32_t* words_host, int64_t n_words, ise_selector_t** out);
int ise_selector_info(const ise_selector_t* sel, int64_t* out5);
int ise_selector_destroy(ise_selector_t* sel);
int ise_index_search_sel_device(ise_index_t* h, const float* q_dev, int64_t nq, int k, const ise_selector_t* sel,
                                float* D_dev, int64_t* I_dev, void* stream);
int ise_index_search_sel_host(ise_index_t* h, const float* q, int64_t nq, int k, const ise_selector_t* sel, float* D,
                              int64_t* I);
int ise_index_range_search_sel_host(ise_index_t* h, const float* q, int64_t nq, float radius, const ise_selector_t* sel,
                                    ise_range_result_t** out);
int ise_index_sel_stats(ise_index_t* h, uint64_t* out3);

#define ISE_BINARY_MAX_BITS 8192
typedef struct ise_binary_index ise_binary_index_t;
typedef struct ise_binary_range_result ise_binary_range_result_t;
int ise_binary_index_create(ise_binary_index_t** out, int d_bits, int device);
int ise_binary_index_destroy(ise_binary_index_t* h);
int ise_binary_index_reset(ise_binary_index_t* h);
int ise_binary_index_info(const ise_binary_index_t* h, int* d_bits, int64_t* ntotal, int* device);
int ise_binary_index_add_host(ise_binary_index_t* h, const uint8_t* codes, int64_t n);
int ise_binary_index_add_device(ise_binary_index_t* h, const uint8_t* codes_dev, int64_t n, void* stream);
int ise_binary_index_reconstruct_host(ise_binary_index_t* h, int64_t i0, int64_t n, uint8_t* out);
int ise_binary_index_search_host(ise_binary_index_t* h, const uint8_t* q, int64_t nq, int k, int32_t* D, int64_t* I);
int ise_binary_index_search_device(ise_binary_index_t* h, const uint8_t* q_dev, int64_t nq, int k, int32_t* D_dev,
                                   int64_t* I_dev, void* stream);
int ise_binary_index_range_search_host(ise_binary_index_t* h, const uint8_t* q, int64_t nq, int32_t radius,
                                       ise_binary_range_result_t** out);
int ise_binary_range_result_get(const ise_binary_range_result_t* r, int64_t* nq, const int64_t** lims, const int32_t** D,
                                const int64_t** I);
int ise_binary_range_result_destroy(ise_binary_range_result_t* r);
int ise_binary_index_stats(ise_binary_index_t* h, uint64_t* out3);

int ise_index_search_keys_device(ise_index_t* h, const float* q_dev, int64_t nq, int k,
                                 uint32_t id_base, uint64_t* keys_dev, void* stream);

int ise_merge_keys_device(const uint64_t* keys_dev, int n_lists, int64_t nq, int k,
                          int metric, float* D_dev, int64_t* I_dev, int device, void* stream);

typedef struct ise_comm ise_comm_t;
int ise_comm_precheck(int device);
int ise_comm_unique_id(void* id128);
int ise_comm_create(ise_comm_t** out, const void* id128, int world, int rank, int device);
int ise_comm_allgather_keys(ise_comm_t* c, const uint64_t* send_dev, uint64_t* recv_dev,
                            int64_t count, void* stream);
int ise_comm_destroy(ise_comm_t* c);

int ise_index_assign_device(ise_index_t* h, const float* x_dev, int64_t n, float* D_dev,
                            int64_t* I_dev, void* stream);

int ise_normalize_rows_device(float* x_dev, int64_t n, int d, int device, void* stream);
int ise_normalize_rows_host(float* x, int64_t n, int d, int device);

int ise_bovw_histogram_device(const int64_t* labels_dev, const int64_t* offsets_dev,
                              int64_t n_images, int K, double* out_dev, int device, void* stream);

int ise_index_search_timed_device(ise_index_t* h, const float* q_dev, int64_t nq, int k,
                                  float* D_dev, int64_t* I_dev, void* stream, int iters,
                                  float* scan_ms_avg, float* merge_ms_avg);

#ifdef __cplusplus
}
#endif
#endif
```

Baseline: 162,600 queries/s.

## Add sampled prologue kernel to precompute query image and initial top-k bounds

Before the int8-shadow scan, a new prologue kernel stages the query shadow image once into a global buffer. It also scans a strided sample of tiles and computes a k-th-smallest lower-bound threshold per query. The main scan blocks then copy the prebuilt image instead of re-quantizing queries, and start with a tight tau bound, so more tiles can be pruned from the first iteration. This adds an extra kernel launch, a cross-block arrival counter, and extra buffers per work slot.

Measured after the change: 157,000 queries/s. 3.5% lower.

```diff
diff --git a/image-search-engine_amd/csrc/ise_knn.hip b/image-search-engine_amd/csrc/ise_knn.hip
--- a/image-search-engine_amd/csrc/ise_knn.hip
+++ b/image-search-engine_amd/csrc/ise_knn.hip
@@ -49,6 +49,7 @@
     double byte_rel = 0.0;
     double byte_rho = 1.0;
     unsigned long long half_batches = 0;
+    unsigned long long prologue_batches = 0;
     unsigned long long byte_batches = 0;
     unsigned long long* stats_dev = nullptr;
     unsigned long long mu_updates = 0;
@@ -61,6 +62,9 @@
         u64* xchg = nullptr;
         size_t xchg_elems = 0;
         uint32_t xchg_seq = 0;
+        unsigned char* pro_img = nullptr;
+        size_t pro_img_bytes = 0;
+        u64* pro_entries = nullptr;
         char* gemm = nullptr;
         size_t gemm_bytes = 0;
         u64* fl_state = nullptr;
@@ -270,6 +274,8 @@
         if (w.part) (void)hipFree(w.part);
         if (w.keys_tmp) (void)hipFree(w.keys_tmp);
         if (w.xchg) (void)hipFree(w.xchg);
+        if (w.pro_img) (void)hipFree(w.pro_img);
+        if (w.pro_entries) (void)hipFree(w.pro_entries);
         if (w.gemm) (void)hipFree(w.gemm);
         if (w.fl_state) (void)hipFree(w.fl_state);
         if (w.fl_list) (void)hipFree(w.fl_list);
@@ -707,6 +713,7 @@
     bool byte;
     bool short_;
     int short_bpc;
+    size_t pro_img_bytes;
 };
 
 static void launch_scan(const ise_index* h, const ScanPlan& pl, dim3 grid, hipStream_t st, const ScanParams& sp) {
@@ -737,6 +744,7 @@
     std::atomic<int> range_stage_cap{0};
     std::atomic<int> no_half{0};
     std::atomic<int> no_byte{0};
+    std::atomic<int> no_prologue{0};
     std::atomic<int> fail_byte_alloc{0};
     std::atomic<int> remove_slab_rows{0};
     void refresh() {
@@ -750,6 +758,7 @@
         range_stage_cap.store(num("ISE_RANGE_STAGE_CAP"));
         no_half.store(flag("ISE_NO_HALF_FILTER"));
         no_byte.store(flag("ISE_NO_BYTE_FILTER"));
+        no_prologue.store(flag("ISE_NO_PROLOGUE"));
         fail_byte_alloc.store(flag("ISE_FAIL_BYTE_ALLOC"));
         remove_slab_rows.store(num("ISE_REMOVE_SLAB_ROWS"));
     }
@@ -859,6 +868,8 @@
     pl->gemm_bytes = 0;
     pl->short_ = false;
     pl->short_bpc = 0;
+    pl->pro_img_bytes = (pl->byte && pl->T == 1 && pl->waves == 8 && pl->nqt == 1 && pl->kc <= pl->kpass && xchg_enabled())
+                            ? scan_image_bytes(qs_stride_byte(h)) : 0;
     static const bool short_t2 = [] { const char* e = getenv("ISE_SHORT_T2"); return !(e && e[0] == '0'); }();
     const int short_T = nq <= 16 ? 1 : 2;
     if (allow_short && !pl->byte && (nq <= 16 || (short_t2 && nq <= 64)) && pl->kc <= pl->kpass && h->n > 0 &&
@@ -892,6 +903,7 @@
                 pl->ch = std::min(chunk_steps(h), 4);
                 pl->half = false;
                 pl->byte = false;
+                pl->pro_img_bytes = 0;
             }
         }
     }
@@ -922,6 +934,21 @@
             w->xchg_seq = (uint32_t)strtoul(e, nullptr, 0);
         *changed = true;
     }
+    if (pl.pro_img_bytes > w->pro_img_bytes) {
+        if (w->pro_img) (void)hipFree(w->pro_img);
+        w->pro_img = nullptr;
+        w->pro_img_bytes = 0;
+        HIP_TRY(hipMalloc(&w->pro_img, pl.pro_img_bytes));
+        w->pro_img_bytes = pl.pro_img_bytes;
+        *changed = true;
+    }
+    if (pl.pro_img_bytes && !w->pro_entries) {
+        const size_t ne = (size_t)16 * PRO_SAMPLE;
+        HIP_TRY(hipMalloc(&w->pro_entries, (ne + 2) * sizeof(u64)));
+        HIP_TRY(hipMemset(w->pro_entries, 0xFF, ne * sizeof(u64)));
+        HIP_TRY(hipMemset(w->pro_entries + ne, 0, 2 * sizeof(u64)));
+        *changed = true;
+    }
     if (pl.kc > pl.kpass) {
         const size_t need2 = (size_t)nq * ((size_t)pl.kc + 2 + pl.kpass + XPASS_MAX);
         if (need2 > w->keys_tmp_elems) {
@@ -1004,6 +1031,7 @@
 static int next_xchg_seq(ise_index::WorkSlot* w, hipStream_t st, uint32_t* seq) {
     if (w->xchg_seq >= 0xFFFFFFF0u) {
         HIP_TRY(hipMemsetAsync(w->xchg, 0xFF, w->xchg_elems * sizeof(u64), st));
+        if (w->pro_entries) HIP_TRY(hipMemsetAsync(w->pro_entries, 0xFF, (size_t)16 * PRO_SAMPLE * sizeof(u64), st));
         w->xchg_seq = 0;
     }
     *seq = ++w->xchg_seq;
@@ -1319,6 +1347,17 @@
     if (pl.kc <= pl.kpass) {
         if ((rc = next_xchg_seq(w, st, &sp.xchg_seq))) return rc;
         if (tm && tm->on) HIP_TRY(hipEventRecord(tm->e0, st));
+        if (pl.pro_img_bytes && !gate && sp.xchg && w->pro_img && w->pro_entries && pl.pro_img_bytes <= w->pro_img_bytes &&
+            !knobs().no_prologue.load(std::memory_order_relaxed)) {
+            PrologueParams pp;
+            pp.image = w->pro_img;
+            pp.entries = w->pro_entries;
+            pp.arrive = reinterpret_cast<unsigned int*>(w->pro_entries + (size_t)16 * PRO_SAMPLE);
+            ise_launch_scan_prologue(pl.ch, pl.pro_img_bytes + 16, st, sp, pp);
+            HIP_TRY(hipGetLastError());
+            sp.image = w->pro_img;
+            h->prologue_batches++;
+        }
         launch_scan(h, pl, grid, st, sp);
         HIP_TRY(hipGetLastError());
         if (tm && tm->on) HIP_TRY(hipEventRecord(tm->e1, st));
@@ -2619,11 +2658,12 @@
     return ISE_OK;
 }
 
-extern "C" int ise_index_byte_stats(ise_index_t* h, uint64_t* out2) {
-    if (!h || !out2) return fail(ISE_E_INVALID, "NULL argument");
+extern "C" int ise_index_byte_stats(ise_index_t* h, uint64_t* out3) {
+    if (!h || !out3) return fail(ISE_E_INVALID, "NULL argument");
     std::lock_guard<std::mutex> lk(h->mu_);
-    out2[0] = h->byte_batches;
-    out2[1] = (h->xq8 && byte_rel_ok(h)) ? 1 : 0;
+    out3[0] = h->byte_batches;
+    out3[1] = (h->xq8 && byte_rel_ok(h)) ? 1 : 0;
+    out3[2] = h->prologue_batches;
     return ISE_OK;
 }
 
diff --git a/image-search-engine_amd/csrc/ise_scan.hpp b/image-search-engine_amd/csrc/ise_scan.hpp
--- a/image-search-engine_amd/csrc/ise_scan.hpp
+++ b/image-search-engine_amd/csrc/ise_scan.hpp
@@ -26,6 +26,38 @@
 #define CSTAMP(i) do {} while (0)
 #endif
 
+
+__device__ __forceinline__ const char* scan_chunk_ptr(const void* xb, int tile, int c, int g, int row_slots, int s0) {
+    return static_cast<const char*>(xb) + ((((size_t)tile * 16 + c) * row_slots + 4 * s0 + g) << 4);
+}
+__device__ __forceinline__ f32x4 scan_tile_f32x4(const void* m, int tile, int g) {
+    return *reinterpret_cast<const f32x4*>(static_cast<const float*>(m) + (size_t)tile * 16 + 4 * g);
+}
+__device__ __forceinline__ void byte_mfma_step(f32x4 a, f32x4 bhi, f32x4 blo, f32x4& acc0, f32x4& acc1) {
+    const i32x4 av = __builtin_bit_cast(i32x4, a);
+    acc0 = __builtin_bit_cast(f32x4, __builtin_amdgcn_mfma_i32_16x16x64_i8(av, __builtin_bit_cast(i32x4, bhi),
+                                                                           __builtin_bit_cast(i32x4, acc0), 0, 0, 0));
+    acc1 = __builtin_bit_cast(f32x4, __builtin_amdgcn_mfma_i32_16x16x64_i8(av, __builtin_bit_cast(i32x4, blo),
+                                                                           __builtin_bit_cast(i32x4, acc1), 0, 0, 0));
+}
+__device__ __forceinline__ f32x4 byte_limb_dot(f32x4 acc0, f32x4 acc1) {
+    const i32x4 ah = __builtin_bit_cast(i32x4, acc0), al = __builtin_bit_cast(i32x4, acc1);
+    f32x4 dot;
+#pragma unroll
+    for (int j = 0; j < 4; j++) dot[j] = fmaf(256.f, (float)ah[j], (float)al[j]);
+    return dot;
+}
+__device__ __forceinline__ float byte_score(float beta, float lo_shrink, float xn, float xr, float xe, int xsh, float dotj,
+                                            float ynj, float yej) {
+    const uint32_t m = __float_as_uint(yej);
+    const float cr = __uint_as_float(m << 16);
+    const float er = cr * (float)__builtin_bit_cast(_Float16, (unsigned short)(m >> 16));
+    return byte_lower_bound(beta, lo_shrink, xn, ynj, ldexpf(dotj * cr, -xsh), xr, sqrtf(ynj) + 0x1p-60f, er, xe);
+}
+__device__ __forceinline__ bool scan_key_ok(long long row, long long n, float s, bool query_ok) {
+    return (row < n) && (s < FLT_MAX) && query_ok;
+}
+
 template <int CH, int W, int T, bool BF16, bool SHIFT, int RM = ROWS_OWN>
 __global__ __launch_bounds__(W * 64, T == 1 ? W / 2 : (W / 4 > 0 ? W / 4 : 1)) void scan_kernel(const ScanParams p) {
     constexpr bool HALF = RM == ROWS_F16, BYTE = RM == ROWS_I8, SHADOW = HALF || BYTE;
@@ -36,6 +68,7 @@
     constexpr int BLOCK_THREADS = W * 64;
     constexpr bool XCHG = T >= 3 || (T == 2 && W == 8) || (RM == ROWS_I8 && T == 1 && W == 8);
     constexpr bool FFILT = XCHG && ISE_FINAL_FILTER;
+    constexpr bool PRO = RM == ROWS_I8 && T == 1 && W == 8 && XCHG;
     constexpr int NQ = 16 * T;
     constexpr int TPR = W >= 16 ? 32 : BLOCK_THREADS / 16;
     constexpr int KPLB = (W * 16 + 63) / 64;
@@ -69,19 +102,18 @@
     STAMP(0);
 
     auto load_chunk = [&](f32x4(&a)[CH], int tile, int s0) {
-        const char* base = static_cast<const char*>(p.xb) +
-                           ((((size_t)tile * 16 + c) * p.row_slots + 4 * s0 + g) << 4);
+        const char* base = scan_chunk_ptr(p.xb, tile, c, g, p.row_slots, s0);
         if (ABL(32)) base = static_cast<const char*>(p.xb) + (((size_t)c * p.row_slots + g) << 4);
         if (ABL(128)) return;
 #pragma unroll
         for (int s = 0; s < CH; s++) a[s] = *reinterpret_cast<const f32x4*>(base + 64 * s);
     };
     auto load_norms = [&](int tile) -> f32x4 {
-        return *reinterpret_cast<const f32x4*>(p.norms + (size_t)tile * 16 + 4 * g);
+        return scan_tile_f32x4(p.norms, tile, g);
     };
     auto load_meta = [&](const void* m, int tile) -> f32x4 {
         if constexpr (!SHADOW) return (f32x4){0.f, 0.f, 0.f, 0.f};
-        return *reinterpret_cast<const f32x4*>(static_cast<const float*>(m) + (size_t)tile * 16 + 4 * g);
+        return scan_tile_f32x4(m, tile, g);
     };
 
     constexpr int FPS = BF16 ? 2 : 1;
@@ -93,7 +125,8 @@
                        S4 <= TPR * QVS;
     f32x4 qv[T][QV];
     f32x4 muv[F32S ? QVS : 1];
-    const bool stager = tid < 16 * TPR;
+    const bool image = PRO && p.image != nullptr;
+    const bool stager = tid < 16 * TPR && !image;
     if (F32S && vec_q && stager) {
 #pragma unroll
         for (int i = 0; i < QVS; i++) {
@@ -132,6 +165,15 @@
             stage_request_row(smuv, p.mu, tid % TPR, TPR, p.d >> 2);
 #pragma unroll
             for (int tq = 0; tq < T; tq++) stage_request_row(sqv[tq], shadow_src(tq), tid % TPR, TPR, p.d >> 2);
+        }
+    }
+    constexpr int IMGV = 3;
+    f32x4 imgv[PRO ? IMGV : 1];
+    if constexpr (PRO) {
+        if (image) {
+#pragma unroll
+            for (int i = 0; i < IMGV; i++)
+                imgv[i] = reinterpret_cast<const f32x4*>(p.image)[min(tid + i * BLOCK_THREADS, (int)(scan_image_bytes(S) / 16) - 1)];
         }
     }
     __builtin_amdgcn_sched_barrier(0);
@@ -258,14 +300,29 @@
             if (t == 0) xn[cc] = sn;
         }
     }
+    if constexpr (PRO) {
+        if (image) {
+            const f32x4* src = reinterpret_cast<const f32x4*>(p.image);
+            f32x4* dst = reinterpret_cast<f32x4*>(qs);
+            const int n16 = (int)(scan_image_bytes(S) / 16);
+#pragma unroll
+            for (int i = 0; i < IMGV; i++)
+                if (tid + i * BLOCK_THREADS < n16) dst[tid + i * BLOCK_THREADS] = imgv[i];
+            for (int i = tid + IMGV * BLOCK_THREADS; i < n16; i += BLOCK_THREADS) dst[i] = src[i];
+        }
+    }
     for (int i = tid; i < NQ; i += BLOCK_THREADS) {
-        tauS[i] = TAU0;
+        if (!image) tauS[i] = TAU0;
         bwc[i] = 0;
         lockS[i] = 0;
     }
     __syncthreads();
     STAMP(1);
     CSTAMP(8);
+    bool bounded = false;
+    if constexpr (PRO) {
+        if (image) bounded = __ballot(tauS[c] == KEY_PAD) == 0;
+    }
 
     const float* qrow = qs + c * S + 4 * g;
     const bool use_floor = p.floor_keys != nullptr;
@@ -288,6 +345,13 @@
     }
     u64 xbound = KEY_PAD;
     bool booted = false;
+    if constexpr (PRO) {
+        if (bounded) {
+            tau[0] = tauS[c];
+            if (FFILT && lane < NQ / W) xbound = tauS[w + lane * W];
+            booted = true;
+        }
+    }
 
     auto merge_out = [&](int t, int cq) {
         const int qq = t * 16 + cq;
@@ -352,13 +416,8 @@
     auto score = [&](int t, float dotj, float ynj, float yej, float ysj) -> float {
         if constexpr (HALF) return half_lower_bound(p.beta, p.lo_shrink, xq_n[t] + ynj,
                                                     ldexpf(dotj, -((int)ysj + xq_sh[t])), yej + xq_e[t]);
-        if constexpr (BYTE) {
-            const uint32_t m = __float_as_uint(yej);
-            const float cr = __uint_as_float(m << 16);
-            const float er = cr * (float)__builtin_bit_cast(_Float16, (unsigned short)(m >> 16));
-            return byte_lower_bound(p.beta, p.lo_shrink, xq_n[t], ynj, ldexpf(dotj * cr, -xq_sh[t]), xq_r[t],
-                                    sqrtf(ynj) + 0x1p-60f, er, xq_e[t]);
-        }
+        if constexpr (BYTE)
+            return byte_score(p.beta, p.lo_shrink, xq_n[t], xq_r[t], xq_e[t], xq_sh[t], dotj, ynj, yej);
         if (l2) {
             const float tt = xq_n[t] + ynj;
             const float sc = tt - 2.f * dotj;
@@ -373,7 +432,7 @@
         for (int t = 0; t < T; t++)
 #pragma unroll
             for (int j = 0; j < 4; j++) {
-                bool ok = (row0 + j < p.n) && (sc[t][j] < FLT_MAX) && (t * 16 + c < nqt);
+                bool ok = scan_key_ok(row0 + j, p.n, sc[t][j], t * 16 + c < nqt);
                 const u64 kj = ((u64)ord_f32(sc[t][j]) << 32) | (uint32_t)((uint32_t)(row0 + j) + p.id_base);
                 if (use_floor) ok = ok && (kj > p.floor_keys[q0 + min(t * 16 + c, nqt - 1)]);
                 key[t][j] = ok ? kj : KEY_PAD;
@@ -382,18 +441,14 @@
 
     float tau_sc[T];
 #pragma unroll
-    for (int t = 0; t < T; t++) tau_sc[t] = FLT_MAX;
+    for (int t = 0; t < T; t++) tau_sc[t] = unord_f32((uint32_t)(tau[t] >> 32));
 
     auto epilogue = [&](int etile, f32x4 yn, f32x4 ye, f32x4 ys) {
         f32x4 sc[T];
 #pragma unroll
         for (int t = 0; t < T; t++) {
             f32x4 dot = acc0[t] + acc1[t];
-            if constexpr (BYTE) {
-                const i32x4 ah = __builtin_bit_cast(i32x4, acc0[t]), al = __builtin_bit_cast(i32x4, acc1[t]);
-#pragma unroll
-                for (int j = 0; j < 4; j++) dot[j] = fmaf(256.f, (float)ah[j], (float)al[j]);
-            }
+            if constexpr (BYTE) dot = byte_limb_dot(acc0[t], acc1[t]);
             acc0[t] = (f32x4){0.f, 0.f, 0.f, 0.f};
             acc1[t] = (f32x4){0.f, 0.f, 0.f, 0.f};
 #pragma unroll
@@ -432,7 +487,7 @@
                 for (int j = 0; j < 4; j++) {
                     if (hit[t][j]) {
                         const float s_ = sc[t][j];
-                        bool ok = (row0 + j < p.n) && (s_ < FLT_MAX) && (t * 16 + c < nqt);
+                        bool ok = scan_key_ok(row0 + j, p.n, s_, t * 16 + c < nqt);
                         const u64 kj = ((u64)ord_f32(s_) << 32) | (uint32_t)((uint32_t)(row0 + j) + p.id_base);
                         if (use_floor) ok = ok && (kj > p.floor_keys[q0 + min(t * 16 + c, nqt - 1)]);
                         const bool v = ok && kj < tau[t];
@@ -461,30 +516,11 @@
         for (int qq = w; qq < NQ; qq += W) {
             const u64* src = p.xchg + ((size_t)blockIdx.y * NQ + qq) * nb;
             auto slot_value = [&](int slot) -> uint32_t {
-                uint32_t best = 0xFFFFFFFFu;
-                for (int j = 0; j < G; j++) {
-                    const int i = slot * G + j;
-                    if (i < nb) {
-                        const u64 v = __hip_atomic_load(src + i, __ATOMIC_RELAXED, __HIP_MEMORY_SCOPE_AGENT);
-                        if ((uint32_t)(v >> 32) == p.xchg_seq) best = min(best, (uint32_t)v);
-                    }
-                }
-                return best;
+                return tagged_min<true>(src, slot * G, 1, G, nb, p.xchg_seq);
             };
             const uint32_t v0 = slot_value(lane), v1 = slot_value(lane + 64), v2 = slot_value(lane + 128),
                            v3 = slot_value(lane + 192);
-            uint32_t prefix = 0;
-            int rank = k;
-            for (int b = 31; b >= 0; b--) {
-                const uint32_t hm = b == 31 ? 0u : 0xFFFFFFFFu << (b + 1);
-                auto zero_here = [&](uint32_t v) { return ((v ^ prefix) & hm) == 0u && ((v >> b) & 1u) == 0u; };
-                const int c0 = __popcll(__ballot(zero_here(v0))) + __popcll(__ballot(zero_here(v1))) +
-                               __popcll(__ballot(zero_here(v2))) + __popcll(__ballot(zero_here(v3)));
-                if (rank > c0) {
-                    rank -= c0;
-                    prefix |= 1u << b;
-                }
-            }
+            const uint32_t prefix = wave_kth_u32(v0, v1, v2, v3, k);
             if (prefix != 0xFFFFFFFFu) {
                 const u64 bound = ((u64)prefix << 32) | 0xFFFFFFFFull;
                 if (FFILT && lane == (qq - w) / W) xbound = bound;
@@ -523,13 +559,7 @@
 #pragma unroll
             for (int t = 0; t < T; t++) {
                 if (BYTE) {
-                    const i32x4 av = __builtin_bit_cast(i32x4, a[s]);
-                    acc0[t] = __builtin_bit_cast(f32x4, __builtin_amdgcn_mfma_i32_16x16x64_i8(
-                                                            av, __builtin_bit_cast(i32x4, bcur[t]),
-                                                            __builtin_bit_cast(i32x4, acc0[t]), 0, 0, 0));
-                    acc1[t] = __builtin_bit_cast(f32x4, __builtin_amdgcn_mfma_i32_16x16x64_i8(
-                                                            av, __builtin_bit_cast(i32x4, bcur_lo[t]),
-                                                            __builtin_bit_cast(i32x4, acc1[t]), 0, 0, 0));
+                    byte_mfma_step(a[s], bcur[t], bcur_lo[t], acc0[t], acc1[t]);
                 } else if (HALF) {
                     const f16x8 av = __builtin_bit_cast(f16x8, a[s]);
                     acc0[t] = __builtin_amdgcn_mfma_f32_16x16x32_f16(av, __builtin_bit_cast(f16x8, bcur[t]), acc0[t], 0, 0, 0);
@@ -556,7 +586,7 @@
     if (has_work) {
         int tile = t0 + w, s0 = 0;
         int tiles_done = 0;
-        bool exchanged = !XCHG || p.xchg == nullptr || ABL(256);
+        bool exchanged = !XCHG || p.xchg == nullptr || ABL(256) || bounded;
         load_b(bcur, bcur_lo, 0);
         bool done = false;
         while (!done) {
@@ -573,6 +603,7 @@
                     if (ns0 >= nsteps) { ns0 = 0; ntile = tile + W; }
                     compute_chunk(A[j], s0, ns0);
                     if (ns0 == 0 && !ABL(8) && !(ABL(2048) && booted)) epilogue(tile, yn, ye, ys);
+                    if (ns0 == 0 && tiles_done == 0) STAMP(10);
                     if (ns0 == 0) tiles_done++;
                     done = ntile >= t1;
                     tile = ntile; s0 = ns0;
diff --git a/image-search-engine_amd/csrc/ise_scan_params.hpp b/image-search-engine_amd/csrc/ise_scan_params.hpp
--- a/image-search-engine_amd/csrc/ise_scan_params.hpp
+++ b/image-search-engine_amd/csrc/ise_scan_params.hpp
@@ -23,6 +23,7 @@
     int tiles_total, tiles_per_block;
     unsigned long long* xchg;
     uint32_t xchg_seq;
+    const unsigned char* image = nullptr;
     const unsigned int* gate;
     int ablate;
     unsigned long long* stamps;
@@ -41,6 +42,18 @@
                                (size_t)waves * CAP * 8 );
 }
 
+__host__ __device__ constexpr size_t scan_image_bytes(int S) { return (size_t)16 * ((size_t)S * 4 + 4 + 8 + 8); }
+
+#define PRO_BLOCKS 64
+#define PRO_TPW 8
+#define PRO_SAMPLE (PRO_BLOCKS * 8 * PRO_TPW)
+struct PrologueParams {
+    unsigned char* image;
+    unsigned long long* entries;
+    unsigned int* arrive;
+};
+void ise_launch_scan_prologue(int ch, size_t lds, hipStream_t st, const ScanParams& sp, const PrologueParams& pp);
+
 void ise_launch_scan_f32_shift(int ch, int waves, int T, dim3 grid, size_t lds, hipStream_t st, const ScanParams& sp);
 void ise_launch_scan_f32_plain(int ch, int waves, int T, dim3 grid, size_t lds, hipStream_t st, const ScanParams& sp);
 void ise_launch_scan_bf16(int ch, int waves, int T, dim3 grid, size_t lds, hipStream_t st, const ScanParams& sp);
diff --git a/image-search-engine_amd/csrc/ise_scan_prologue.hip b/image-search-engine_amd/csrc/ise_scan_prologue.hip
--- /dev/null
+++ b/image-search-engine_amd/csrc/ise_scan_prologue.hip
@@ -0,0 +1,10 @@
+#include "ise_scan_prologue.hpp"
+
+void ise_launch_scan_prologue(int ch, size_t lds, hipStream_t st, const ScanParams& sp, const PrologueParams& pp) {
+    const dim3 grid(PRO_BLOCKS), block(512);
+    switch (ch) {
+        case 4: hipLaunchKernelGGL(scan_prologue_kernel<4>, grid, block, lds, st, sp, pp); break;
+        case 2: hipLaunchKernelGGL(scan_prologue_kernel<2>, grid, block, lds, st, sp, pp); break;
+        default: hipLaunchKernelGGL(scan_prologue_kernel<1>, grid, block, lds, st, sp, pp); break;
+    }
+}
diff --git a/image-search-engine_amd/csrc/ise_scan_prologue.hpp b/image-search-engine_amd/csrc/ise_scan_prologue.hpp
--- /dev/null
+++ b/image-search-engine_amd/csrc/ise_scan_prologue.hpp
@@ -0,0 +1,143 @@
+#pragma once
+#include "ise_scan.hpp"
+
+template <int CH>
+__global__ __launch_bounds__(512, 4) void scan_prologue_kernel(const ScanParams p, const PrologueParams pp) {
+    constexpr int W = 8, NQ = 16, TPR = W * 64 / 16;
+    constexpr int R = 12 / CH;
+    static_assert((PRO_BLOCKS & (PRO_BLOCKS - 1)) == 0, "the arrival counter wraps");
+    extern __shared__ __align__(16) unsigned char smem[];
+    const int S = p.qs_stride;
+    float* qs = reinterpret_cast<float*>(smem);
+    float* xn = qs + NQ * S;
+    float* xe = xn + NQ;
+    int* xsh = reinterpret_cast<int*>(xe + NQ);
+    int* lastS = reinterpret_cast<int*>(smem + scan_image_bytes(S));
+
+    const int tid = threadIdx.x, lane = tid & 63, w = __builtin_amdgcn_readfirstlane(tid >> 6);
+    const int c = lane & 15, g = lane >> 4;
+    const int nqt = min(NQ, p.nq);
+    const int k = p.k;
+    const int nsteps = p.row_slots >> 2;
+
+    {
+        const int cc = tid / TPR, t = tid % TPR;
+        const int PS = p.row_slots * 16;
+        const bool rowok = cc < nqt;
+        const float* src = p.q + (size_t)(rowok ? cc : 0) * p.d;
+        unsigned char* hi = reinterpret_cast<unsigned char*>(qs + cc * S);
+        unsigned char* lo = hi + 16 * p.row_slots;
+        if (shadow_vec_ok(p.d, PS, p.q, TPR)) {
+            f32x4 sqv[SHADOW_QV], smuv[SHADOW_QV];
+            stage_request_row(smuv, p.mu, t, TPR, p.d >> 2);
+            stage_request_row(sqv, src, t, TPR, p.d >> 2);
+            float amax, mark;
+            stage_shadow_vec_scale<TPR>(sqv, smuv, src, p.mu, p.d >> 2, rowok, t, PS >> 2, false, amax, mark);
+            stage_shadow_vec_limbs<true, TPR>(sqv, smuv, src, p.mu, p.d >> 2, rowok, t, PS >> 2, amax, mark, hi, lo,
+                                              xn + cc, xe + cc, xsh + cc);
+        } else {
+            stage_shadow_scalar<true, TPR>(src, p.mu, p.d, PS, rowok, t, hi, lo, xn + cc, xe + cc, xsh + cc);
+        }
+    }
+    __syncthreads();
+    if (blockIdx.x == 0) {
+        const f32x4* src = reinterpret_cast<const f32x4*>(smem);
+        f32x4* dst = reinterpret_cast<f32x4*>(pp.image);
+        for (int i = tid; i < (int)((scan_image_bytes(S) - NQ * 8) / 16); i += W * 64) dst[i] = src[i];
+    }
+
+    const int j0 = (blockIdx.x * W + w) * PRO_TPW;
+    const bool dense = p.tiles_total >= PRO_SAMPLE;
+    auto tile_of = [&](int j) -> int { return dense ? (int)((long long)j * p.tiles_total / PRO_SAMPLE) : j; };
+    const int ntl = dense ? PRO_TPW : max(0, min(PRO_TPW, p.tiles_total - j0));
+    const float xq_n = xn[c], xq_e = xe[c], xq_r = sqrtf(xq_n) + 0x1p-60f;
+    const int xq_sh = xsh[c];
+    const float* qrow = qs + c * S + 4 * g;
+    if (ntl > 0) {
+        f32x4 A[R][CH];
+        auto load_chunk = [&](f32x4(&a)[CH], int tile, int s0) {
+            const char* base = scan_chunk_ptr(p.xb, tile, c, g, p.row_slots, s0);
+#pragma unroll
+            for (int s = 0; s < CH; s++) a[s] = *reinterpret_cast<const f32x4*>(base + 64 * s);
+        };
+        int li = 0, ls0 = 0;
+        auto advance_load = [&]() {
+            int ns = ls0 + CH, ni = li;
+            if (ns >= nsteps) { ns = 0; ni = li + 1; }
+            if (ni < ntl) { li = ni; ls0 = ns; }
+        };
+#pragma unroll
+        for (int j = 0; j < R - 1; j++) {
+            load_chunk(A[j], tile_of(j0 + li), ls0);
+            advance_load();
+        }
+        f32x4 acc0 = {0.f, 0.f, 0.f, 0.f}, acc1 = {0.f, 0.f, 0.f, 0.f};
+        int i = 0, s0 = 0;
+        bool done = false;
+        while (!done) {
+#pragma unroll
+            for (int j = 0; j < R; j++) {
+                if (!done) {
+                    const int tile = tile_of(j0 + i);
+                    const f32x4 yn = scan_tile_f32x4(p.norms, tile, g);
+                    const f32x4 ye = scan_tile_f32x4(p.bmeta, tile, g);
+                    load_chunk(A[(j + R - 1) % R], tile_of(j0 + li), ls0);
+                    advance_load();
+                    __builtin_amdgcn_sched_barrier(0);
+#pragma unroll
+                    for (int s = 0; s < CH; s++) {
+                        const f32x4 bhi = *reinterpret_cast<const f32x4*>(qrow + 16 * (s0 + s));
+                        const f32x4 blo = *reinterpret_cast<const f32x4*>(qrow + 4 * p.row_slots + 16 * (s0 + s));
+                        byte_mfma_step(A[j][s], bhi, blo, acc0, acc1);
+                    }
+                    s0 += CH;
+                    if (s0 >= nsteps) {
+                        const f32x4 dot = byte_limb_dot(acc0, acc1);
+                        acc0 = (f32x4){0.f, 0.f, 0.f, 0.f};
+                        acc1 = (f32x4){0.f, 0.f, 0.f, 0.f};
+                        uint32_t best = 0xFFFFFFFFu;
+#pragma unroll
+                        for (int r = 0; r < 4; r++) {
+                            const float sc = byte_score(p.beta, p.lo_shrink, xq_n, xq_r, xq_e, xq_sh, dot[r], yn[r], ye[r]);
+                            if (scan_key_ok((long long)tile * 16 + 4 * g + r, p.n, sc, c < nqt)) best = min(best, ord_f32(sc));
+                        }
+                        best = min(best, (uint32_t)__shfl_xor((int)best, 16));
+                        best = min(best, (uint32_t)__shfl_xor((int)best, 32));
+                        if (g == 0)
+                            __hip_atomic_store(pp.entries + (size_t)c * PRO_SAMPLE + j0 + i, ((u64)p.xchg_seq << 32) | best,
+                                               __ATOMIC_RELAXED, __HIP_MEMORY_SCOPE_AGENT);
+                        s0 = 0;
+                        i++;
+                        done = i >= ntl;
+                    }
+                }
+            }
+        }
+    }
+
+    asm volatile("s_waitcnt vmcnt(0)" ::: "memory");
+    __syncthreads();
+    if (tid == 0) {
+        __builtin_amdgcn_fence(__ATOMIC_RELEASE, "agent");
+        asm volatile("s_waitcnt vmcnt(0)" ::: "memory");
+        const unsigned prev = __hip_atomic_fetch_add(pp.arrive, 1u, __ATOMIC_RELAXED, __HIP_MEMORY_SCOPE_AGENT);
+        const int last = ((prev + 1u) & (unsigned)(PRO_BLOCKS - 1)) == 0u ? 1 : 0;
+        *lastS = last;
+        if (last) {
+            __builtin_amdgcn_fence(__ATOMIC_ACQUIRE, "agent");
+            asm volatile("s_waitcnt vmcnt(0)" ::: "memory");
+        }
+    }
+    __syncthreads();
+    if (!*lastS) return;
+    u64* bound = reinterpret_cast<u64*>(pp.image + scan_image_bytes(S) - NQ * 8);
+    for (int qq = w; qq < NQ; qq += W) {
+        const u64* src = pp.entries + (size_t)qq * PRO_SAMPLE;
+        uint32_t v[4];
+#pragma unroll
+        for (int e = 0; e < 4; e++) v[e] = tagged_min<false>(src, lane + 64 * e, 256, PRO_SAMPLE / 256, PRO_SAMPLE, p.xchg_seq);
+        const uint32_t prefix = wave_kth_u32(v[0], v[1], v[2], v[3], k);
+        if (lane == 0)
+            bound[qq] = qq >= nqt ? 0ull : (prefix != 0xFFFFFFFFu ? ((u64)prefix << 32) | 0xFFFFFFFFull : KEY_PAD);
+    }
+}
diff --git a/image-search-engine_amd/csrc/ise_select.hpp b/image-search-engine_amd/csrc/ise_select.hpp
--- a/image-search-engine_amd/csrc/ise_select.hpp
+++ b/image-search-engine_amd/csrc/ise_select.hpp
@@ -147,6 +147,35 @@
 }
 
 
+template <bool ATOMIC>
+__device__ __forceinline__ uint32_t tagged_min(const u64* src, int first, int step, int count, int n, uint32_t seq) {
+    uint32_t best = 0xFFFFFFFFu;
+    for (int j = 0; j < count; j++) {
+        const int i = first + j * step;
+        if (i < n) {
+            const u64 v = ATOMIC ? __hip_atomic_load(src + i, __ATOMIC_RELAXED, __HIP_MEMORY_SCOPE_AGENT) : src[i];
+            if ((uint32_t)(v >> 32) == seq) best = min(best, (uint32_t)v);
+        }
+    }
+    return best;
+}
+
+__device__ __forceinline__ uint32_t wave_kth_u32(uint32_t v0, uint32_t v1, uint32_t v2, uint32_t v3, int k) {
+    uint32_t prefix = 0;
+    int rank = k;
+    for (int b = 31; b >= 0; b--) {
+        const uint32_t hm = b == 31 ? 0u : 0xFFFFFFFFu << (b + 1);
+        auto zero_here = [&](uint32_t v) { return ((v ^ prefix) & hm) == 0u && ((v >> b) & 1u) == 0u; };
+        const int c0 = __popcll(__ballot(zero_here(v0))) + __popcll(__ballot(zero_here(v1))) +
+                       __popcll(__ballot(zero_here(v2))) + __popcll(__ballot(zero_here(v3)));
+        if (rank > c0) {
+            rank -= c0;
+            prefix |= 1u << b;
+        }
+    }
+    return prefix;
+}
+
 template <int KPL>
 __device__ __forceinline__ void block_topk_part(const u64* list, int n, int base, int per, int k, u64* dst) {
     const int lane = threadIdx.x & 63;
diff --git a/image-search-engine_amd/faiss_compat.py b/image-search-engine_amd/faiss_compat.py
--- a/image-search-engine_amd/faiss_compat.py
+++ b/image-search-engine_amd/faiss_compat.py
@@ -240,9 +240,9 @@
         return {"half_batches": int(out[0])}
 
     def byte_stats(self) -> dict:
-        out = (ctypes.c_uint64 * 2)()
+        out = (ctypes.c_uint64 * 3)()
         _n.check(_n.lib.ise_index_byte_stats(self._h, out))
-        return {"byte_batches": int(out[0]), "byte_route": bool(out[1])}
+        return {"byte_batches": int(out[0]), "byte_route": bool(out[1]), "prologue_batches": int(out[2])}
 
     def byte_row(self, i: int) -> tuple:
         out = (ctypes.c_float * 2)()
diff --git a/include/ise_knn.h b/include/ise_knn.h
--- a/include/ise_knn.h
+++ b/include/ise_knn.h
@@ -45,7 +45,7 @@
 int ise_index_short_stats(ise_index_t* h, uint64_t* out1);
 
 int ise_index_half_stats(ise_index_t* h, uint64_t* out1);
-int ise_index_byte_stats(ise_index_t* h, uint64_t* out2);
+int ise_index_byte_stats(ise_index_t* h, uint64_t* out3);
 int ise_index_shadow_row(ise_index_t* h, int64_t i, float* out3);
 int ise_index_byte_row(ise_index_t* h, int64_t i, float* out2);
 
```
